# HKU-BAL/MegaGTA

Hardware: AMD Instinct MI355X
Metric: HMM-scored node expansions/sec + SdBG-build Gk-mer/s, k=45, 100Mx150bp (higher is better)
Workload: dtype u32

## Files before the change

### include/megagta_hip.h

```cpp
#ifndef MEGAGTA_HIP_H_
#define MEGAGTA_HIP_H_
#include <stdint.h>
#ifdef __cplusplus
extern "C" {
#endif

#define MGTA_OK 0
#define MGTA_EINVAL (-1)
#define MGTA_EHIP (-2)
#define MGTA_ENOMEM (-3)
#define MGTA_EUNSUPPORTED (-4)
#define MGTA_ESINK (-5)
#define MGTA_EOVERFLOW (-6)
#define MGTA_EINTERNAL (-7)

#define MGTA_NUM_BUCKETS 65536

typedef struct mgta_ctx mgta_ctx;
typedef struct mgta_reads mgta_reads;
typedef struct mgta_sdbg mgta_sdbg;
typedef struct mgta_hmm mgta_hmm;

const char *mgta_last_error(void);
const char *mgta_version(void);

mgta_ctx *mgta_ctx_create(int device_id);
void mgta_ctx_destroy(mgta_ctx *);
int mgta_ctx_set_mem_limit(mgta_ctx *, uint64_t bytes);
int mgta_ctx_device_memory(mgta_ctx *, uint64_t *free_bytes, uint64_t *total_bytes);
int mgta_ctx_keep_stream(mgta_ctx *, int on);
typedef struct mgta_stream mgta_stream;
int mgta_sdbg_stream_detach(mgta_ctx *, mgta_stream **out);
int mgta_stream_sizes(const mgta_stream *, uint64_t *n_recs, uint64_t *n_tip_words);
int mgta_stream_download(mgta_stream *, uint16_t *recs, uint32_t *tips);
void mgta_stream_free(mgta_stream *);
int mgta_ctx_release_scratch(mgta_ctx *);
int mgta_ctx_set_full_lsd(mgta_ctx *, int on);
int mgta_sort_plan(uint64_t n_items, int words_per_key, uint32_t bucket_begin, uint32_t bucket_end, int *n_passes, int *skip_bits);
int mgta_sort_plan_wide(uint64_t n_items, int words_per_key, uint32_t bucket_begin, uint32_t bucket_end, int *n_passes, int *skip_bits,
                        int *widths );
int mgta_ctx_set_search_cost_rate(mgta_ctx *, int expansions_per_seed);
int mgta_ctx_set_search_cost_curve(mgta_ctx *, int expansions_per_seed, uint64_t knee_expansions, int expansions_per_seed_beyond);
int mgta_ctx_set_search_arena(mgta_ctx *, int log2_base_nodes, uint64_t pool_bytes);
int mgta_ctx_set_search_page_limit(mgta_ctx *, int pages);
int mgta_ctx_keep_multiplicity(mgta_ctx *, int on);

int mgta_reads_pack_text(mgta_ctx *, const char *text, uint64_t n_bytes, const uint64_t *offsets , uint64_t n_reads,
                         uint32_t *bin_words, uint64_t capacity_words, uint64_t *n_words_out);


typedef int (*mgta_edge_sink)(void *user, int32_t bucket_begin, int32_t bucket_end,
                              const int64_t *bucket_counts ,
                              const uint16_t *recs, int64_t n_recs, const uint16_t *large, int64_t n_large,
                              const uint32_t *tips, int64_t n_tip_words);

typedef struct mgta_build_stats {
    int32_t k, words_per_key, words_per_tip, n_passes;
    int64_t n_reads, n_kmers;
    int64_t n_items;
    int64_t n_edges, n_tips, n_large;
    int64_t n_sort_launches;
    double ms_total;
    double ms_count, ms_gen, ms_sort, ms_emit, ms_d2h;
    double ms_sort_scatter;
    double ms_local_sort;
    int64_t n_big_segments;
    int64_t n_lsd_tiles;
    uint64_t bytes_peak;
    double ms_stage1;
    int64_t n_fused_passes;
    int64_t n_wide_passes;
    int64_t n_split_levels;
} mgta_build_stats;

int mgta_reads_upload(mgta_ctx *, const uint32_t *packed_seq, uint64_t n_words, const uint64_t *start_idx,
                      uint64_t n_reads, mgta_reads **out);
int mgta_reads_adopt_device(mgta_ctx *, const uint32_t *d_packed_seq, uint64_t n_words,
                            const uint64_t *d_start_idx, uint64_t n_reads, mgta_reads **out);
void mgta_reads_free(mgta_reads *);

int mgta_sdbg_build_resident(mgta_ctx *, const mgta_reads *, uint64_t n_short_reads, int k, int min_count,
                             int need_mercy, int32_t bucket_begin, int32_t bucket_end ,
                             mgta_edge_sink sink, void *user, mgta_build_stats *stats);
int mgta_sdbg_last_counting(mgta_ctx *, int64_t *hist );
int mgta_sdbg_export_records_device(mgta_ctx *, void *d_dst, uint64_t capacity_bytes, uint64_t *n_records);
int mgta_sdbg_build(mgta_ctx *, const uint32_t *packed_seq, uint64_t n_words, const uint64_t *start_idx,
                    uint64_t n_reads, uint64_t n_short_reads, int k, int min_count, int need_mercy,
                    mgta_edge_sink sink, void *user, mgta_build_stats *stats);

int mgta_sdbg_load(mgta_ctx *, int k, const uint16_t *recs, int64_t size, const int64_t *bucket_items,
                   const uint32_t *tips, int64_t n_tip_words, int words_per_tip, mgta_sdbg **out);
int mgta_sdbg_load_resident(mgta_ctx *, mgta_sdbg **out);
int mgta_sdbg_load_large(mgta_ctx *, int k, const uint16_t *recs, int64_t size, const int64_t *bucket_items, const uint32_t *tips,
                         int64_t n_tip_words, int words_per_tip, const uint16_t *large, int64_t n_large, mgta_sdbg **out);
int mgta_sdbg_load_files(mgta_ctx *, const char *prefix, mgta_sdbg **out);
void mgta_sdbg_free(mgta_sdbg *);
int64_t mgta_sdbg_size(const mgta_sdbg *);
int mgta_sdbg_k(const mgta_sdbg *);
int mgta_sdbg_outgoing(mgta_sdbg *, const int64_t *edges, int64_t n, int64_t *out4, int8_t *outdeg);
int mgta_sdbg_invalid_bits(mgta_sdbg *, uint64_t *words);
int mgta_sdbg_index_edges(mgta_sdbg *, const uint8_t *seqs , int64_t n, int64_t *edge_ids);

int mgta_sdbg_edge_multiplicity(mgta_sdbg *, const int64_t *edge_ids, int64_t n, uint16_t *mult);

typedef struct mgta_contig_cov {
    uint64_t sum;
    uint32_t len, n_windows;
    uint32_t n_covered;
    uint32_t min, max, median;
} mgta_contig_cov;
typedef struct mgta_coverage_stats {
    int64_t n_contigs, n_windows;
    int64_t n_walked;
    int64_t n_index_searches;
    int64_t n_batches;
    int64_t groups_per_cu;
    double ms_kernel;
    double ms_walk;
} mgta_coverage_stats;
int mgta_ctx_set_coverage_batch(mgta_ctx *, uint64_t windows);
int mgta_contig_coverage(mgta_sdbg *, const char *seqs, const uint64_t *offsets , int64_t n, mgta_contig_cov *per_contig,
                         uint16_t *per_window , int64_t *abundance , mgta_coverage_stats *stats );

typedef struct mgta_contig_share {
    uint64_t mass;
    uint32_t len, n_windows;
    uint32_t n_covered;
    uint32_t n_unique;
    uint32_t max_share;
    uint32_t reserved_;
} mgta_contig_share;
typedef struct mgta_share_stats {
    int64_t n_contigs, n_windows;
    int64_t n_walked, n_index_searches;
    int64_t n_batches;
    int64_t n_covered;
    int64_t n_distinct_edges;
    uint64_t total_mult;
    uint64_t total_mass;
    uint64_t table_slots;
    uint64_t table_bytes;
    uint64_t window_bytes;
    double ms_walk;
    double ms_count;
    double ms_share;
    double ms_total;
} mgta_share_stats;
int mgta_ctx_set_share_hash_bits(mgta_ctx *, int bits);
int mgta_contig_share_coverage(mgta_sdbg *, const char *seqs, const uint64_t *offsets , int64_t n, mgta_contig_share *per_contig,
                               uint32_t *per_window_share , uint16_t *per_window , mgta_share_stats *stats );

typedef struct mgta_match_stats {
    int64_t n_contigs, n_contig_windows;
    int64_t n_marked_edges;
    int64_t n_reads, n_read_windows;
    int64_t n_walked, n_index_searches;
    int64_t n_matched_reads;
    int64_t groups_per_cu;
    double ms_mark, ms_walk;
} mgta_match_stats;
int mgta_reads_match_contigs(mgta_sdbg *, const mgta_reads *reads, int reads_reversed, uint64_t n_short_reads,
                             const char *seqs, const uint64_t *offsets , int64_t n,
                             uint64_t *match_bits ,
                             uint32_t *hit_windows , mgta_match_stats *stats );

typedef struct mgta_sample_cov_stats {
    int64_t n_contigs, n_windows;
    int64_t n_walked, n_index_searches;
    int64_t n_batches;
    int64_t n_covered;
    int64_t n_keys;
    int64_t n_libs;
    int64_t n_reads, n_read_windows;
    int64_t n_read_walked, n_read_index_searches;
    int64_t n_hit_windows;
    int64_t groups_per_cu;
    uint64_t total_mass;
    uint64_t table_slots;
    uint64_t table_bytes;
    uint64_t window_bytes;
    uint64_t count_bytes;
    double ms_mark;
    double ms_scan;
    double ms_mass;
    double ms_total;
} mgta_sample_cov_stats;
int mgta_contig_sample_coverage(mgta_sdbg *, const mgta_reads *reads, int reads_reversed, const uint64_t *lib_end , int n_libs,
                                const char *seqs, const uint64_t *offsets , int64_t n, uint64_t *mass ,
                                mgta_contig_share *per_contig , uint64_t *per_window_count ,
                                uint32_t *per_window_share , uint64_t *lib_hit_windows ,
                                mgta_sample_cov_stats *stats );

typedef struct mgta_pileup_params { int32_t min_anchors, min_overlap, max_mismatch_permille; } mgta_pileup_params;
typedef struct mgta_contig_pileup { uint32_t len, n_covered, min_depth, max_depth; uint64_t n_placed, n_unique, depth_sum, mismatch_sum; } mgta_contig_pileup;
typedef struct mgta_read_place { int32_t score, contig, diag, orient; uint32_t n_placed, n_mismatch; } mgta_read_place;
typedef struct mgta_pileup_stats {
    int64_t n_contigs, n_contig_letters, n_contig_windows;
    int64_t n_keys;
    int64_t n_occurrences;
    int64_t n_reads, n_read_windows;
    int64_t n_hit_windows;
    int64_t n_read_walked, n_read_index_searches;
    int64_t n_reads_with_candidate, n_candidates;
    int64_t n_verified;
    int64_t n_reads_placed, n_reads_multi, n_placements;
    int64_t n_bases_piled;
    int64_t groups_per_cu;
    uint64_t peak_bytes;
    double ms_keys, ms_index, ms_scan, ms_records, ms_total;
} mgta_pileup_stats;
int mgta_reads_pileup(mgta_sdbg *, const mgta_reads *reads, int reads_reversed, uint64_t n_short_reads, const char *seqs,
                      const uint64_t *offsets , int64_t n, const mgta_pileup_params *params ,
                      uint32_t *counts , uint32_t *uniq ,
                      mgta_contig_pileup *per_contig , mgta_read_place *per_read ,
                      mgta_pileup_stats *stats );
int mgta_ctx_set_pileup_chunk(mgta_ctx *, uint32_t reads);

typedef struct mgta_derep_stats {
    int64_t n_seqs, n_letters;
    int64_t n_first;
    int64_t n_duplicates, n_contained, n_kept;
    int64_t n_windows;
    int64_t anchor_len;
    int64_t n_compares;
    double ms_dups, ms_table, ms_verify;
} mgta_derep_stats;
int mgta_seqs_derep(mgta_ctx *, const char *seqs, const uint64_t *offsets , int64_t n,
                    uint8_t *status, int64_t *rep, uint32_t *copies, mgta_derep_stats *stats );
int mgta_ctx_set_derep_hash_bits(mgta_ctx *, int bits);

typedef struct mgta_align_rec {
    double score;
    int32_t status;
    int32_t model_from, model_to;
    int32_t n_match, n_insert, n_delete;
} mgta_align_rec;
typedef struct mgta_align_stats {
// ... 202 lines not shown
```

### megagta_amd/_lib.py

```python
from __future__ import annotations

import ctypes as C
import os

_HERE = os.path.dirname(os.path.abspath(__file__))
LIB_PATH = os.environ.get("MEGAGTA_HIP_LIB") or os.path.join(_HERE, "libmegagta_hip.so")


class MegaGtaError(RuntimeError):
    pass


class DenovoStats(C.Structure):
    _fields_ = [("n_tips", C.c_int64), ("n_bubbles", C.c_int64), ("n_bubble_candidates", C.c_int64), ("n_bubble_rounds", C.c_int64),
                ("n_paths", C.c_int64), ("n_unitig_sweeps", C.c_int64), ("n_contigs", C.c_int64), ("total_len", C.c_int64),
                ("ms_tips", C.c_float), ("ms_bubbles", C.c_float), ("ms_unitigs", C.c_float)]

    def as_dict(self):
        return {n: getattr(self, n) for n, _ in self._fields_}


class BuildStats(C.Structure):
    _fields_ = [("k", C.c_int32), ("words_per_key", C.c_int32), ("words_per_tip", C.c_int32), ("n_passes", C.c_int32),
                ("n_reads", C.c_int64), ("n_kmers", C.c_int64), ("n_items", C.c_int64), ("n_edges", C.c_int64),
# ... 57 lines not shown
                ("table_slots", C.c_uint64), ("table_bytes", C.c_uint64), ("window_bytes", C.c_uint64), ("ms_walk", C.c_double), ("ms_count", C.c_double),
                ("ms_share", C.c_double), ("ms_total", C.c_double)]

    def as_dict(self):
        return {n: getattr(self, n) for n, _ in self._fields_}


class MatchStats(C.Structure):
    _fields_ = [("n_contigs", C.c_int64), ("n_contig_windows", C.c_int64), ("n_marked_edges", C.c_int64), ("n_reads", C.c_int64),
                ("n_read_windows", C.c_int64), ("n_walked", C.c_int64), ("n_index_searches", C.c_int64), ("n_matched_reads", C.c_int64),
                ("groups_per_cu", C.c_int64), ("ms_mark", C.c_double), ("ms_walk", C.c_double)]

    def as_dict(self):
        return {n: getattr(self, n) for n, _ in self._fields_}


class SampleCovStats(C.Structure):
    _fields_ = [("n_contigs", C.c_int64), ("n_windows", C.c_int64), ("n_walked", C.c_int64), ("n_index_searches", C.c_int64), ("n_batches", C.c_int64),
                ("n_covered", C.c_int64), ("n_keys", C.c_int64), ("n_libs", C.c_int64), ("n_reads", C.c_int64), ("n_read_windows", C.c_int64),
                ("n_read_walked", C.c_int64), ("n_read_index_searches", C.c_int64), ("n_hit_windows", C.c_int64), ("groups_per_cu", C.c_int64),
                ("total_mass", C.c_uint64), ("table_slots", C.c_uint64), ("table_bytes", C.c_uint64), ("window_bytes", C.c_uint64),
                ("count_bytes", C.c_uint64), ("ms_mark", C.c_double), ("ms_scan", C.c_double), ("ms_mass", C.c_double), ("ms_total", C.c_double)]

    def as_dict(self):
        return {n: getattr(self, n) for n, _ in self._fields_}


class DerepStats(C.Structure):
    _fields_ = [("n_seqs", C.c_int64), ("n_letters", C.c_int64), ("n_first", C.c_int64), ("n_duplicates", C.c_int64), ("n_contained", C.c_int64),
                ("n_kept", C.c_int64), ("n_windows", C.c_int64), ("anchor_len", C.c_int64), ("n_compares", C.c_int64), ("ms_dups", C.c_double),
                ("ms_table", C.c_double), ("ms_verify", C.c_double)]

    def as_dict(self):
        return {n: getattr(self, n) for n, _ in self._fields_}


class AlignRec(C.Structure):
    _fields_ = [("score", C.c_double), ("status", C.c_int32), ("model_from", C.c_int32), ("model_to", C.c_int32), ("n_match", C.c_int32),
                ("n_insert", C.c_int32), ("n_delete", C.c_int32)]


class AlignStats(C.Structure):
    _fields_ = [("n_seqs", C.c_int64), ("n_aligned", C.c_int64), ("n_unaligned", C.c_int64), ("n_cells", C.c_int64), ("n_batches", C.c_int64),
                ("blocks_per_cu", C.c_int64), ("waves_per_block", C.c_int64), ("grid_blocks", C.c_int64), ("lds_bytes", C.c_int64),
                ("msc_in_lds", C.c_int64), ("ms_fill", C.c_double), ("ms_trace", C.c_double)]

    def as_dict(self):
        return {n: getattr(self, n) for n, _ in self._fields_}


class PostRec(C.Structure):
    _fields_ = [("fwd", C.c_double), ("bwd", C.c_double), ("status", C.c_int32), ("pad", C.c_int32)]


class PostStats(C.Structure):
    _fields_ = [("n_seqs", C.c_int64), ("n_scored", C.c_int64), ("n_unaligned", C.c_int64), ("n_cells", C.c_int64), ("n_batches", C.c_int64),
                ("workgroups", C.c_int64), ("waves_per_block", C.c_int64), ("blocks_per_cu", C.c_int64), ("lds_bytes", C.c_int64),
                ("msc_in_lds", C.c_int64), ("peak_bytes", C.c_int64), ("ms_forward", C.c_double), ("ms_backward", C.c_double)]

    def as_dict(self):
        return {n: getattr(self, n) for n, _ in self._fields_}


class RowPair(C.Structure):
    _fields_ = [("i", C.c_int32), ("j", C.c_int32), ("n_diff", C.c_uint16), ("n_overlap", C.c_uint16)]


class ClusterStats(C.Structure):
    _fields_ = [("n_rows", C.c_int64), ("n_unaligned", C.c_int64), ("n_pairs_kept", C.c_int64), ("n_clusters", C.c_int64), ("n_singletons", C.c_int64),
                ("largest_cluster", C.c_int64), ("n_components", C.c_int64), ("n_tiles", C.c_int64), ("n_link_pops", C.c_int64),
                ("blocks_per_cu", C.c_int64), ("grid_blocks", C.c_int64), ("lds_bytes", C.c_int64), ("peak_bytes", C.c_int64),
                ("ms_pairs", C.c_double), ("ms_link", C.c_double)]

    def as_dict(self):
        return {n: getattr(self, n) for n, _ in self._fields_}


class TreeStats(C.Structure):
    _fields_ = [("n_rows", C.c_int64), ("n_pairs", C.c_int64), ("n_merges", C.c_int64), ("n_rounds", C.c_int64), ("n_entries_visited", C.c_int64),
                ("n_lists_rewritten", C.c_int64), ("n_cut_fallbacks", C.c_int64), ("n_unaligned", C.c_int64), ("n_clusters", C.c_int64),
                ("n_singletons", C.c_int64), ("largest_cluster", C.c_int64), ("peak_bytes", C.c_int64), ("ms_pairs", C.c_double), ("ms_build", C.c_double),
                ("ms_rounds", C.c_double), ("ms_cut", C.c_double)]

    def as_dict(self):
        return {n: getattr(self, n) for n, _ in self._fields_}


class NearestRec(C.Structure):
    _fields_ = [("status", C.c_int32), ("ref", C.c_int32), ("score", C.c_int32), ("ref_from", C.c_int32), ("ref_to", C.c_int32), ("n_match", C.c_int32),
                ("n_ident", C.c_int32), ("n_insert", C.c_int32), ("n_delete", C.c_int32)]


class NearestStats(C.Structure):
    _fields_ = [("n_seqs", C.c_int64), ("n_refs", C.c_int64), ("n_pairs", C.c_int64), ("n_unaligned", C.c_int64), ("n_cells", C.c_int64),
                ("n_trace_cells", C.c_int64), ("n_batches", C.c_int64), ("n_segments", C.c_int64), ("blocks_per_cu", C.c_int64),
                ("waves_per_block", C.c_int64), ("grid_blocks", C.c_int64), ("lds_bytes", C.c_int64), ("peak_bytes", C.c_int64),
                ("ms_score", C.c_double), ("ms_trace", C.c_double)]

    def as_dict(self):
        return {n: getattr(self, n) for n, _ in self._fields_}


class ChimeraRec(C.Structure):
    _fields_ = [("status", C.c_int32), ("ref", C.c_int32), ("score", C.c_int32), ("brk", C.c_int32), ("left_ref", C.c_int32), ("left_score", C.c_int32),
                ("right_ref", C.c_int32), ("right_score", C.c_int32), ("two", C.c_int32), ("one", C.c_int32), ("gain", C.c_int32)]


class ChimeraStats(C.Structure):
    _fields_ = [("n_seqs", C.c_int64), ("n_refs", C.c_int64), ("n_clean", C.c_int64), ("n_chimeric", C.c_int64), ("n_unchecked", C.c_int64),
                ("n_cells", C.c_int64), ("n_parent_cells", C.c_int64), ("n_items", C.c_int64), ("n_parent_items", C.c_int64), ("n_segments", C.c_int64),
                ("n_groups", C.c_int64), ("grid_blocks", C.c_int64), ("waves_per_block", C.c_int64), ("blocks_per_cu", C.c_int64), ("lds_bytes", C.c_int64),
                ("bound_bytes", C.c_int64), ("peak_bytes", C.c_int64), ("ms_top", C.c_double), ("ms_parents", C.c_double)]

    def as_dict(self):
        return {n: getattr(self, n) for n, _ in self._fields_}


class PileupParams(C.Structure):
    _fields_ = [("min_anchors", C.c_int32), ("min_overlap", C.c_int32), ("max_mismatch_permille", C.c_int32)]


class PileupStats(C.Structure):
    _fields_ = [("n_contigs", C.c_int64), ("n_contig_letters", C.c_int64), ("n_contig_windows", C.c_int64), ("n_keys", C.c_int64), ("n_occurrences", C.c_int64),
                ("n_reads", C.c_int64), ("n_read_windows", C.c_int64), ("n_hit_windows", C.c_int64), ("n_read_walked", C.c_int64),
                ("n_read_index_searches", C.c_int64), ("n_reads_with_candidate", C.c_int64), ("n_candidates", C.c_int64), ("n_verified", C.c_int64),
                ("n_reads_placed", C.c_int64), ("n_reads_multi", C.c_int64), ("n_placements", C.c_int64), ("n_bases_piled", C.c_int64),
                ("groups_per_cu", C.c_int64), ("peak_bytes", C.c_uint64), ("ms_keys", C.c_double), ("ms_index", C.c_double), ("ms_scan", C.c_double),
                ("ms_records", C.c_double), ("ms_total", C.c_double)]

    def as_dict(self):
        return {n: getattr(self, n) for n, _ in self._fields_}


EDGE_SINK = C.CFUNCTYPE(C.c_int, C.c_void_p, C.c_int32, C.c_int32, C.POINTER(C.c_int64), C.POINTER(C.c_uint16), C.c_int64,
                        C.POINTER(C.c_uint16), C.c_int64, C.POINTER(C.c_uint32), C.c_int64)
CONTIG_SINK = C.CFUNCTYPE(C.c_int, C.c_void_p, C.c_int64, C.c_void_p, C.c_int64, C.c_void_p, C.c_int64,
                          C.POINTER(AstarSide), C.POINTER(AstarSide))

SYMBOLS = {
    "mgta_last_error": (C.c_char_p, []),
    "mgta_version": (C.c_char_p, []),
    "mgta_ctx_create": (C.c_void_p, [C.c_int]),
    "mgta_ctx_destroy": (None, [C.c_void_p]),
    "mgta_ctx_set_mem_limit": (C.c_int, [C.c_void_p, C.c_uint64]),
    "mgta_ctx_set_full_lsd": (C.c_int, [C.c_void_p, C.c_int]),
    "mgta_sort_plan": (C.c_int, [C.c_uint64, C.c_int, C.c_uint32, C.c_uint32, C.POINTER(C.c_int), C.POINTER(C.c_int)]),
    "mgta_sort_plan_wide": (C.c_int, [C.c_uint64, C.c_int, C.c_uint32, C.c_uint32, C.POINTER(C.c_int), C.POINTER(C.c_int), C.POINTER(C.c_int)]),
    "mgta_reads_upload": (C.c_int, [C.c_void_p, C.c_void_p, C.c_uint64, C.c_void_p, C.c_uint64, C.POINTER(C.c_void_p)]),
    "mgta_reads_adopt_device": (C.c_int, [C.c_void_p, C.c_void_p, C.c_uint64, C.c_void_p, C.c_uint64, C.POINTER(C.c_void_p)]),
    "mgta_reads_free": (None, [C.c_void_p]),
    "mgta_sdbg_build_resident": (C.c_int, [C.c_void_p, C.c_void_p, C.c_uint64, C.c_int, C.c_int, C.c_int, C.c_int32, C.c_int32,
                                          EDGE_SINK, C.c_void_p, C.POINTER(BuildStats)]),
    "mgta_sdbg_last_counting": (C.c_int, [C.c_void_p, C.c_void_p]),
    "mgta_sdbg_export_records_device": (C.c_int, [C.c_void_p, C.c_void_p, C.c_uint64, C.POINTER(C.c_uint64)]),
    "mgta_sdbg_build": (C.c_int, [C.c_void_p, C.c_void_p, C.c_uint64, C.c_void_p, C.c_uint64, C.c_uint64, C.c_int, C.c_int,
                                 C.c_int, EDGE_SINK, C.c_void_p, C.POINTER(BuildStats)]),
    "mgta_findstart": (C.c_int, [C.c_void_p, C.c_void_p, C.c_int, C.c_int, C.c_void_p, C.c_int64, C.c_void_p, C.c_int64, C.c_void_p, C.c_void_p]),
    "mgta_sdbg_load_resident": (C.c_int, [C.c_void_p, C.c_void_p]),
    "mgta_sdbg_load_files": (C.c_int, [C.c_void_p, C.c_char_p, C.c_void_p]),
    "mgta_sdbg_invalid_bits": (C.c_int, [C.c_void_p, C.c_void_p]),
    "mgta_ctx_set_search_cost_rate": (C.c_int, [C.c_void_p, C.c_int]),
    "mgta_ctx_set_search_cost_curve": (C.c_int, [C.c_void_p, C.c_int, C.c_uint64, C.c_int]),
    "mgta_ctx_set_search_arena": (C.c_int, [C.c_void_p, C.c_int, C.c_uint64]),
    "mgta_ctx_set_search_page_limit": (C.c_int, [C.c_void_p, C.c_int]),
    "mgta_ctx_device_memory": (C.c_int, [C.c_void_p, C.POINTER(C.c_uint64), C.POINTER(C.c_uint64)]),
    "mgta_ctx_keep_stream": (C.c_int, [C.c_void_p, C.c_int]),
    "mgta_sdbg_stream_detach": (C.c_int, [C.c_void_p, C.POINTER(C.c_void_p)]),
    "mgta_stream_sizes": (C.c_int, [C.c_void_p, C.POINTER(C.c_uint64), C.POINTER(C.c_uint64)]),
    "mgta_stream_download": (C.c_int, [C.c_void_p, C.c_void_p, C.c_void_p]),
    "mgta_stream_free": (None, [C.c_void_p]),
    "mgta_sdbg_k": (C.c_int, [C.c_void_p]),
    "mgta_ctx_set_search_share": (C.c_int, [C.c_void_p, C.c_int, C.c_int]),
    "mgta_astar_batch_on": (C.c_int, [C.c_void_p, C.c_void_p, C.c_void_p, C.c_void_p, C.c_char_p, C.c_void_p, C.c_int64, C.c_int, C.c_double,
                                     C.c_int, CONTIG_SINK, C.c_void_p, C.POINTER(AstarStats)]),
    "mgta_astar_batch_packed": (C.c_int, [C.c_void_p, C.c_void_p, C.c_void_p, C.c_char_p, C.c_void_p, C.c_int64, C.c_int, C.c_double, C.c_int,
                                         C.POINTER(C.c_void_p), C.c_void_p, C.c_void_p, C.POINTER(AstarStats)]),
    "mgta_reads_pack_text": (C.c_int, [C.c_void_p, C.c_char_p, C.c_uint64, C.c_void_p, C.c_uint64, C.c_void_p, C.c_uint64, C.POINTER(C.c_uint64)]),
    "mgta_ctx_release_scratch": (C.c_int, [C.c_void_p]),
    "mgta_denovo": (C.c_int, [C.c_void_p, C.c_int, C.c_int, C.c_int, C.c_void_p, C.c_void_p, C.c_void_p]),
    "mgta_host_free": (None, [C.c_void_p]),
    "mgta_sdbg_load": (C.c_int, [C.c_void_p, C.c_int, C.c_void_p, C.c_int64, C.c_void_p, C.c_void_p, C.c_int64, C.c_int,
                                C.POINTER(C.c_void_p)]),
    "mgta_ctx_keep_multiplicity": (C.c_int, [C.c_void_p, C.c_int]),
    "mgta_ctx_set_coverage_batch": (C.c_int, [C.c_void_p, C.c_uint64]),
    "mgta_sdbg_load_large": (C.c_int, [C.c_void_p, C.c_int, C.c_void_p, C.c_int64, C.c_void_p, C.c_void_p, C.c_int64, C.c_int, C.c_void_p, C.c_int64,
                                      C.POINTER(C.c_void_p)]),
    "mgta_sdbg_edge_multiplicity": (C.c_int, [C.c_void_p, C.c_void_p, C.c_int64, C.c_void_p]),
    "mgta_contig_coverage": (C.c_int, [C.c_void_p, C.c_char_p, C.c_void_p, C.c_int64, C.c_void_p, C.c_void_p, C.c_void_p, C.c_void_p]),
    "mgta_contig_share_coverage": (C.c_int, [C.c_void_p, C.c_char_p, C.c_void_p, C.c_int64, C.c_void_p, C.c_void_p, C.c_void_p, C.c_void_p]),
    "mgta_ctx_set_share_hash_bits": (C.c_int, [C.c_void_p, C.c_int]),
    "mgta_reads_match_contigs": (C.c_int, [C.c_void_p, C.c_void_p, C.c_int, C.c_uint64, C.c_char_p, C.c_void_p, C.c_int64, C.c_void_p, C.c_void_p,
                                          C.c_void_p]),
    "mgta_contig_sample_coverage": (C.c_int, [C.c_void_p, C.c_void_p, C.c_int, C.c_void_p, C.c_int, C.c_char_p, C.c_void_p, C.c_int64, C.c_void_p, C.c_void_p,
                                             C.c_void_p, C.c_void_p, C.c_void_p, C.c_void_p]),
    "mgta_reads_pileup": (C.c_int, [C.c_void_p, C.c_void_p, C.c_int, C.c_uint64, C.c_char_p, C.c_void_p, C.c_int64, C.c_void_p, C.c_void_p, C.c_void_p, C.c_void_p,
                                   C.c_void_p, C.c_void_p]),
    "mgta_ctx_set_pileup_chunk": (C.c_int, [C.c_void_p, C.c_uint32]),
    "mgta_seqs_derep": (C.c_int, [C.c_void_p, C.c_char_p, C.c_void_p, C.c_int64, C.c_void_p, C.c_void_p, C.c_void_p, C.c_void_p]),
    "mgta_ctx_set_derep_hash_bits": (C.c_int, [C.c_void_p, C.c_int]),
    "mgta_seqs_align": (C.c_int, [C.c_void_p, C.c_void_p, C.c_char_p, C.c_void_p, C.c_int64, C.c_void_p, C.c_void_p, C.c_void_p, C.c_void_p, C.c_void_p]),
    "mgta_ctx_set_align_batch": (C.c_int, [C.c_void_p, C.c_int64]),
    "mgta_seqs_posterior": (C.c_int, [C.c_void_p, C.c_void_p, C.c_char_p, C.c_void_p, C.c_int64, C.c_void_p, C.c_void_p, C.c_void_p, C.c_void_p, C.c_void_p,
                                      C.c_void_p]),
    "mgta_ctx_set_posterior_batch": (C.c_int, [C.c_void_p, C.c_int64]),
    "mgta_rows_pairs": (C.c_int, [C.c_void_p, C.c_void_p, C.c_int64, C.c_int64, C.c_int64, C.c_double, C.c_void_p, C.c_int64, C.c_void_p, C.c_void_p]),
    "mgta_rows_cluster": (C.c_int, [C.c_void_p, C.c_void_p, C.c_void_p, C.c_int64, C.c_int64, C.c_int64, C.c_double, C.c_void_p, C.c_void_p, C.c_void_p,
                                    C.c_void_p, C.c_void_p]),
    "mgta_pairs_link": (C.c_int, [C.c_void_p, C.c_int64, C.c_void_p, C.c_void_p, C.c_int64, C.c_void_p, C.c_void_p, C.c_void_p, C.c_void_p, C.c_void_p]),
    "mgta_ctx_set_cluster_tile": (C.c_int, [C.c_void_p, C.c_int64]),
    "mgta_pairs_tree": (C.c_int, [C.c_void_p, C.c_void_p, C.c_int64, C.c_void_p, C.c_int64, C.c_void_p, C.c_int64, C.c_void_p, C.c_void_p]),
    "mgta_tree_cut": (C.c_int, [C.c_void_p, C.c_int64, C.c_void_p, C.c_int64, C.c_void_p, C.c_void_p, C.c_int64, C.c_double, C.c_void_p, C.c_void_p, C.c_void_p,
                                C.c_void_p, C.c_void_p]),
    "mgta_rows_clusters": (C.c_int, [C.c_void_p, C.c_void_p, C.c_void_p, C.c_int64, C.c_int64, C.c_int64, C.c_void_p, C.c_int64, C.c_void_p, C.c_void_p,
                                     C.c_void_p, C.c_void_p, C.c_void_p, C.c_void_p, C.c_void_p]),
    "mgta_seqs_nearest": (C.c_int, [C.c_void_p, C.c_char_p, C.c_void_p, C.c_int64, C.c_char_p, C.c_void_p, C.c_int64, C.c_void_p, C.c_int32, C.c_int32,
                                    C.c_void_p, C.c_void_p, C.c_void_p, C.c_void_p, C.c_void_p]),
    "mgta_ctx_set_nearest_batch": (C.c_int, [C.c_void_p, C.c_int64]),
    "mgta_seqs_chimera": (C.c_int, [C.c_void_p, C.c_char_p, C.c_void_p, C.c_int64, C.c_char_p, C.c_void_p, C.c_int64, C.c_void_p, C.c_int32, C.c_int32,
                                    C.c_int32, C.c_int32, C.c_void_p, C.c_void_p, C.c_void_p]),
    "mgta_ctx_set_chimera_segment": (C.c_int, [C.c_void_p, C.c_int64]),
    "mgta_ctx_set_chimera_groups": (C.c_int, [C.c_void_p, C.c_int64]),
    "mgta_sdbg_free": (None, [C.c_void_p]),
    "mgta_sdbg_size": (C.c_int64, [C.c_void_p]),
    "mgta_sdbg_outgoing": (C.c_int, [C.c_void_p, C.c_void_p, C.c_int64, C.c_void_p, C.c_void_p]),
    "mgta_sdbg_index_edges": (C.c_int, [C.c_void_p, C.c_void_p, C.c_int64, C.c_void_p]),
    "mgta_hmm_load": (C.c_int, [C.c_void_p, C.c_int, C.c_int, C.c_void_p, C.c_void_p, C.c_void_p, C.c_void_p, C.c_void_p,
                               C.POINTER(C.c_void_p)]),
    "mgta_hmm_free": (None, [C.c_void_p]),
    "mgta_probe_random_lines": (C.c_int, [C.c_void_p, C.c_uint64, C.POINTER(LineProbe), C.c_int]),
    "mgta_astar_batch": (C.c_int, [C.c_void_p, C.c_void_p, C.c_void_p, C.c_char_p, C.c_void_p, C.c_int64, C.c_int, C.c_double,
                                  C.c_int, CONTIG_SINK, C.c_void_p, C.POINTER(AstarStats)]),
}

_LIB = None


def load():
    global _LIB
    if _LIB is not None:
        return _LIB
    if not os.path.exists(LIB_PATH):
        raise MegaGtaError(f"{LIB_PATH} is missing: build it with `python -c 'import __graft_entry__ as g; g.build()'` "
                           "(make -C megagta_amd/csrc). There is no CPU fallback.")
    L = C.CDLL(LIB_PATH)
    for name, (res, args) in SYMBOLS.items():
        fn = getattr(L, name)
        fn.restype, fn.argtypes = res, args
    _LIB = L
    return L


def check(rc: int, what: str):
    if rc != 0:
        raise MegaGtaError(f"{what} failed ({rc}): {load().mgta_last_error().decode()}")
```

### megagta_amd/api.py

```python
from __future__ import annotations

import ctypes as C
import hashlib
import os
from dataclasses import dataclass, field

import numpy as np

from . import _lib
from .chimera import REC as _chimera_rec
from ._lib import MegaGtaError, check

NUM_BUCKETS = 65536


@dataclass
class EdgeStream:
    k: int
    words_per_tip: int
    bucket_items: np.ndarray
    records: np.ndarray
    large: np.ndarray
    tips: np.ndarray
    bucket_large: np.ndarray = None
# ... 170 lines not shown
                  "mgta_rows_pairs")
            if got.value != cnt.value:
                raise MegaGtaError(f"mgta_rows_pairs counted {cnt.value} pairs, then {got.value}")
        return dict(pairs=pairs[:cnt.value], stats=st.as_dict())

    def cluster(self, rows, lens, min_overlap: int, cutoff: float) -> dict:
        r = self._rows(rows)
        n, M = r.shape
        ln = np.ascontiguousarray(lens, dtype=np.int64)
        if ln.shape != (n,):
            raise ValueError("lens must hold one length per row")
        cl, rep = np.zeros(max(1, n), dtype=np.int32), np.zeros(max(1, n), dtype=np.int64)
        rd, ro = np.zeros(max(1, n), dtype=np.uint16), np.zeros(max(1, n), dtype=np.uint16)
        st = _lib.ClusterStats()
        check(self._L.mgta_rows_cluster(self.h, r.ctypes.data, ln.ctypes.data, n, M, int(min_overlap), float(cutoff), cl.ctypes.data, rep.ctypes.data,
                                        rd.ctypes.data, ro.ctypes.data, C.byref(st)), "mgta_rows_cluster")
        return dict(cluster=cl[:n], rep=rep[:n], rep_diff=rd[:n], rep_overlap=ro[:n], stats=st.as_dict())

    def pairs_tree(self, pairs, n_residues) -> dict:
        p = _pair_array(pairs)
        nr = np.ascontiguousarray(n_residues, dtype=np.int32)
        if nr.ndim != 1:
            raise ValueError("n_residues must hold one value per row")
        n = nr.size
        merges = np.zeros(max(1, n), dtype=TREE_MERGE)
        cnt, st = C.c_int64(0), _lib.TreeStats()
        check(self._L.mgta_pairs_tree(self.h, p.ctypes.data if p.size else None, p.size, nr.ctypes.data, n, merges.ctypes.data, n, C.byref(cnt), C.byref(st)),
              "mgta_pairs_tree")
        return dict(merges=merges[:cnt.value], stats=st.as_dict())

    def clusters(self, rows, lens, min_overlap: int, cutoffs) -> dict:
        r = self._rows(rows)
        n, M = r.shape
        ln = np.ascontiguousarray(lens, dtype=np.int64)
        if ln.shape != (n,):
            raise ValueError("lens must hold one length per row")
        cut = np.ascontiguousarray(cutoffs, dtype=np.float64)
        if cut.ndim != 1:
            raise ValueError("cutoffs must be a list of numbers")
        k = cut.size
        cl, rep = np.zeros((k, n), dtype=np.int32), np.zeros((k, n), dtype=np.int64)
        rd, ro = np.zeros((k, n), dtype=np.uint16), np.zeros((k, n), dtype=np.uint16)
        merges = np.zeros(max(1, n), dtype=TREE_MERGE)
        cnt, st = C.c_int64(0), _lib.TreeStats()
        check(self._L.mgta_rows_clusters(self.h, r.ctypes.data, ln.ctypes.data, n, M, int(min_overlap), cut.ctypes.data if k else None, k, cl.ctypes.data,
                                         rep.ctypes.data, rd.ctypes.data, ro.ctypes.data, merges.ctypes.data, C.byref(cnt), C.byref(st)), "mgta_rows_clusters")
        return dict(cluster=cl, rep=rep, rep_diff=rd, rep_overlap=ro, merges=merges[:cnt.value], stats=st.as_dict())

    def set_nearest_batch(self, cells: int = 0):
        check(self._L.mgta_ctx_set_nearest_batch(self.h, int(cells)), "mgta_ctx_set_nearest_batch")

    def nearest(self, seqs, refs, sub, gap_open: int, gap_extend: int, scores: bool = False, paths: bool = False) -> dict:
        raw = [s if isinstance(s, (bytes, bytearray)) else str(s).encode("latin-1") for s in seqs]
        rraw = [s if isinstance(s, (bytes, bytearray)) else str(s).encode("latin-1") for s in refs]
        n, n_ref = len(raw), len(rraw)
        table = np.ascontiguousarray(sub, dtype=np.int8)
        if table.shape != (27, 27):
            raise ValueError("sub must be int8[27, 27]")
        offsets, roffsets = np.zeros(n + 1, dtype=np.uint64), np.zeros(n_ref + 1, dtype=np.uint64)
        if n:
            np.cumsum([len(s) for s in raw], out=offsets[1:])
        if n_ref:
            np.cumsum([len(s) for s in rraw], out=roffsets[1:])
        recs = np.zeros(max(1, n), dtype=NEAREST_REC)
        sc = np.zeros((n, n_ref), dtype=np.int32) if scores else None
        p = np.zeros(int(offsets[n]) + n * 4096 + 1, dtype=np.uint8) if paths else None
        plen = np.zeros(max(1, n), dtype=np.int32) if paths else None
        st = _lib.NearestStats()
        check(self._L.mgta_seqs_nearest(self.h, b"".join(raw), offsets.ctypes.data, n, b"".join(rraw), roffsets.ctypes.data, n_ref, table.ctypes.data,
                                        int(gap_open), int(gap_extend), recs.ctypes.data, sc.ctypes.data if scores and sc.size else None,
                                        p.ctypes.data if paths else None, plen.ctypes.data if paths else None, C.byref(st)), "mgta_seqs_nearest")
        out = dict(recs=recs[:n], stats=st.as_dict())
        if scores:
            out["scores"] = sc
        if paths:
            out["paths"] = [p[int(offsets[i]) + i * 4096:int(offsets[i]) + i * 4096 + int(plen[i])].tobytes().decode() for i in range(n)]
        return out

    def set_chimera_segment(self, columns: int = 0):
        check(self._L.mgta_ctx_set_chimera_segment(self.h, int(columns)), "mgta_ctx_set_chimera_segment")

    def set_chimera_groups(self, groups: int = 0):
        check(self._L.mgta_ctx_set_chimera_groups(self.h, int(groups)), "mgta_ctx_set_chimera_groups")

    def chimera(self, seqs, refs, sub, gap_open: int, gap_extend: int, min_seg: int, min_gain: int, tops: bool = False) -> dict:
        raw = [s if isinstance(s, (bytes, bytearray)) else str(s).encode("latin-1") for s in seqs]
        rraw = [s if isinstance(s, (bytes, bytearray)) else str(s).encode("latin-1") for s in refs]
        n, n_ref = len(raw), len(rraw)
        table = np.ascontiguousarray(sub, dtype=np.int8)
        if table.shape != (27, 27):
            raise ValueError("sub must be int8[27, 27]")
        offsets, roffsets = np.zeros(n + 1, dtype=np.uint64), np.zeros(n_ref + 1, dtype=np.uint64)
        if n:
            np.cumsum([len(s) for s in raw], out=offsets[1:])
        if n_ref:
            np.cumsum([len(s) for s in rraw], out=roffsets[1:])
        recs = np.zeros(max(1, n), dtype=CHIMERA_REC)
        tp = np.zeros((int(offsets[n]) + 1, 8), dtype=np.int32) if tops else None
        st = _lib.ChimeraStats()
        check(self._L.mgta_seqs_chimera(self.h, b"".join(raw), offsets.ctypes.data, n, b"".join(rraw), roffsets.ctypes.data, n_ref, table.ctypes.data,
                                        int(gap_open), int(gap_extend), int(min_seg), int(min_gain), recs.ctypes.data, tp.ctypes.data if tops else None,
                                        C.byref(st)), "mgta_seqs_chimera")
        out = dict(recs=recs[:n], stats=st.as_dict())
        if tops:
            out["tops"] = [tp[int(offsets[i]):int(offsets[i + 1])] for i in range(n)]
        return out

    def release_scratch(self):
        check(self._L.mgta_ctx_release_scratch(self.h), "mgta_ctx_release_scratch")

    def set_search_arena(self, log2_base_nodes: int = 0, pool_bytes: int = 0):
        check(self._L.mgta_ctx_set_search_arena(self.h, int(log2_base_nodes), int(pool_bytes)), "mgta_ctx_set_search_arena")

    def set_search_page_limit(self, pages: int = 0):
        check(self._L.mgta_ctx_set_search_page_limit(self.h, int(pages)), "mgta_ctx_set_search_page_limit")

    def upload_reads(self, packed: np.ndarray, start_idx: np.ndarray) -> "Reads":
        packed = np.ascontiguousarray(packed, dtype=np.uint32)
        start_idx = np.ascontiguousarray(start_idx, dtype=np.uint64)
        out = C.c_void_p()
        check(self._L.mgta_reads_upload(self.h, packed.ctypes.data, packed.size, start_idx.ctypes.data, start_idx.size - 1,
                                        C.byref(out)), "mgta_reads_upload")
        return Reads(self, out, start_idx.size - 1)

    def adopt_reads(self, d_packed_ptr: int, n_words: int, d_start_ptr: int, n_reads: int, keepalive=None) -> "Reads":
        out = C.c_void_p()
        check(self._L.mgta_reads_adopt_device(self.h, d_packed_ptr, n_words, d_start_ptr, n_reads, C.byref(out)),
              "mgta_reads_adopt_device")
        r = Reads(self, out, n_reads)
        r._keep = keepalive
        return r

    def build_sdbg(self, reads: "Reads", k: int, min_count: int = 1, need_mercy: bool = False, collect: bool = True,
                   n_short_reads: int | None = None, bucket_range: tuple[int, int] = (0, NUM_BUCKETS)) -> EdgeStream:
        wpt = (2 * k + 31) // 32
        recs, large, tips = [], [], []
        counts = np.zeros((NUM_BUCKETS, 3), dtype=np.int64)

        def sink(user, b0, b1, bc, r, nr, lg, nl, tp, ntw):
            nb = b1 - b0
            counts[b0:b1] = np.ctypeslib.as_array(bc, shape=(nb * 3,)).reshape(nb, 3)
            recs.append(np.ctypeslib.as_array(r, shape=(nr,)).copy() if nr and r else np.zeros(0, np.uint16))
            large.append(np.ctypeslib.as_array(lg, shape=(nl,)).copy() if nl else np.zeros(0, np.uint16))
            tips.append(np.ctypeslib.as_array(tp, shape=(ntw,)).copy() if ntw and tp else np.zeros(0, np.uint32))
            return 0

        cb = _lib.EDGE_SINK(sink) if collect else C.cast(None, _lib.EDGE_SINK)
        st = _lib.BuildStats()
        ns = reads.n_reads if n_short_reads is None else n_short_reads
        check(self._L.mgta_sdbg_build_resident(self.h, reads.h, ns, k, min_count, int(need_mercy), bucket_range[0], bucket_range[1],
                                               cb, None, C.byref(st)),
              "mgta_sdbg_build_resident")
        cat = lambda xs, dt: np.concatenate(xs) if xs else np.zeros(0, dt)
        return EdgeStream(k=k, words_per_tip=wpt, bucket_items=counts[:, 0].copy(), records=cat(recs, np.uint16),
                          large=cat(large, np.uint16), tips=cat(tips, np.uint32), bucket_large=counts[:, 1].copy(),
                          bucket_tips=counts[:, 2].copy(), stats=st.as_dict())


def export_records_to_torch(ctx: "Context"):
    import torch
    n = C.c_uint64()
    check(ctx._L.mgta_sdbg_export_records_device(ctx.h, None, 0, C.byref(n)), "mgta_sdbg_export_records_device")
    t = torch.empty(max(1, n.value * 2), dtype=torch.uint8, device="cuda")
    check(ctx._L.mgta_sdbg_export_records_device(ctx.h, t.data_ptr(), t.numel(), C.byref(n)), "mgta_sdbg_export_records_device")
    return t[: n.value * 2]


SHARE_DTYPE = np.dtype([("mass", "<u8"), ("len", "<u4"), ("n_windows", "<u4"), ("n_covered", "<u4"), ("n_unique", "<u4"), ("max_share", "<u4"),
                        ("reserved_", "<u4")])
COV_DTYPE = np.dtype([("sum", "<u8"), ("len", "<u4"), ("n_windows", "<u4"), ("n_covered", "<u4"), ("min", "<u4"), ("max", "<u4"), ("median", "<u4")])


class _multiplicity:

    def __init__(self, ctx: "Context", on: bool):
        self.ctx, self.was = ctx, getattr(ctx, "_keep_multiplicity", False)
        self.on = bool(on) or self.was

    def __enter__(self):
        if self.on != self.was:
            self.ctx.keep_multiplicity(self.on)
        return self

    def __exit__(self, *exc):
        if self.on != self.was:
            self.ctx.keep_multiplicity(self.was)
        return False


class Graph:

    def __init__(self, ctx: Context, stream: "EdgeStream | None", k: int = 0, keep_multiplicity: bool = False):
        if stream is None:
            self.ctx, self.k = ctx, k
            out = C.c_void_p()
            with _multiplicity(ctx, keep_multiplicity) as sw:
                self.keep_multiplicity = sw.on
                check(ctx._L.mgta_sdbg_load_resident(ctx.h, C.byref(out)), "mgta_sdbg_load_resident")
            self.h = out
            self.size = ctx._L.mgta_sdbg_size(self.h)
            self.k = ctx._L.mgta_sdbg_k(self.h)
            return
        self.ctx, self.k = ctx, stream.k
        recs = np.ascontiguousarray(stream.records, dtype=np.uint16)
        bi = np.ascontiguousarray(stream.bucket_items, dtype=np.int64)
        tips = np.ascontiguousarray(stream.tips, dtype=np.uint32)
        out = C.c_void_p()
        with _multiplicity(ctx, keep_multiplicity) as sw:
            self.keep_multiplicity = sw.on
            if sw.on:
                large = np.ascontiguousarray(stream.large, dtype=np.uint16)
                check(ctx._L.mgta_sdbg_load_large(ctx.h, stream.k, recs.ctypes.data, recs.size, bi.ctypes.data, tips.ctypes.data, tips.size,
                                                  stream.words_per_tip, large.ctypes.data, large.size, C.byref(out)), "mgta_sdbg_load_large")
            else:
                check(ctx._L.mgta_sdbg_load(ctx.h, stream.k, recs.ctypes.data, recs.size, bi.ctypes.data, tips.ctypes.data, tips.size,
                                            stream.words_per_tip, C.byref(out)), "mgta_sdbg_load")
        self.h = out
        self.size = ctx._L.mgta_sdbg_size(self.h)

    @classmethod
    def from_files(cls, ctx: Context, prefix: str, keep_multiplicity: bool = False) -> "Graph":
        self = cls.__new__(cls)
        self.ctx = ctx
        out = C.c_void_p()
        with _multiplicity(ctx, keep_multiplicity) as sw:
            self.keep_multiplicity = sw.on
            check(ctx._L.mgta_sdbg_load_files(ctx.h, os.fsencode(prefix), C.byref(out)), "mgta_sdbg_load_files")
        self.h = out
        self.size = ctx._L.mgta_sdbg_size(self.h)
        self.k = ctx._L.mgta_sdbg_k(self.h)
        return self

    def outgoing(self, edges) -> tuple[np.ndarray, np.ndarray]:
        e = np.ascontiguousarray(edges, dtype=np.int64)
        out = np.empty((e.size, 4), dtype=np.int64)
        deg = np.empty(e.size, dtype=np.int8)
        check(self.ctx._L.mgta_sdbg_outgoing(self.h, e.ctypes.data, e.size, out.ctypes.data, deg.ctypes.data), "mgta_sdbg_outgoing")
        return deg, out

    def index_edges(self, kmers: list[str]) -> np.ndarray:
        m = {"A": 1, "C": 2, "G": 3, "T": 4, "N": 3}
        seqs = np.array([[m.get(c, 0) for c in s.upper()[: self.k + 1]] for s in kmers], dtype=np.uint8).reshape(len(kmers), self.k + 1)
        ids = np.empty(len(kmers), dtype=np.int64)
        check(self.ctx._L.mgta_sdbg_index_edges(self.h, seqs.ctypes.data, len(kmers), ids.ctypes.data), "mgta_sdbg_index_edges")
        return ids

    def invalid_bits(self) -> np.ndarray:
        out = np.zeros((self.size + 63) // 64, dtype=np.uint64)
        check(self.ctx._L.mgta_sdbg_invalid_bits(self.h, out.ctypes.data), "mgta_sdbg_invalid_bits")
        return out

    def edge_multiplicity(self, ids) -> np.ndarray:
        e = np.ascontiguousarray(ids, dtype=np.int64)
        out = np.empty(e.size, dtype=np.uint16)
        check(self.ctx._L.mgta_sdbg_edge_multiplicity(self.h, e.ctypes.data, e.size, out.ctypes.data), "mgta_sdbg_edge_multiplicity")
        return out

    def contig_coverage(self, seqs, per_window: bool = False, abundance: bool = True) -> dict:
        raw = [s if isinstance(s, (bytes, bytearray)) else str(s).encode() for s in seqs]
        n = len(raw)
        offsets = np.zeros(n + 1, dtype=np.uint64)
        if n:
            np.cumsum([len(s) for s in raw], out=offsets[1:])
        buf = b"".join(raw)
        cov = np.zeros(n, dtype=COV_DTYPE)
        nw = np.maximum(0, np.diff(offsets.astype(np.int64)) - self.ctx._L.mgta_sdbg_k(self.h))
        woff = np.zeros(n + 1, dtype=np.int64)
        np.cumsum(nw, out=woff[1:])
        pw = np.zeros(int(woff[-1]), dtype=np.uint16) if per_window else None
        ab = np.zeros(65536, dtype=np.int64) if abundance else None
        st = _lib.CoverageStats()
        check(self.ctx._L.mgta_contig_coverage(self.h, buf, offsets.ctypes.data, n, cov.ctypes.data if n else None,
                                               pw.ctypes.data if per_window and pw.size else None, ab.ctypes.data if abundance else None,
                                               C.byref(st)), "mgta_contig_coverage")
        out = dict(contigs=cov, abundance=ab, stats=st.as_dict())
        if per_window:
            out["per_window"], out["window_offsets"] = pw, woff
        return out

    def contig_share_coverage(self, seqs, per_window: bool = False) -> dict:
        raw = [s if isinstance(s, (bytes, bytearray)) else str(s).encode() for s in seqs]
        n = len(raw)
        offsets = np.zeros(n + 1, dtype=np.uint64)
        if n:
            np.cumsum([len(s) for s in raw], out=offsets[1:])
        rec = np.zeros(n, dtype=SHARE_DTYPE)
        nw = np.maximum(0, np.diff(offsets.astype(np.int64)) - self.ctx._L.mgta_sdbg_k(self.h))
        woff = np.zeros(n + 1, dtype=np.int64)
        np.cumsum(nw, out=woff[1:])
        pws = np.zeros(int(woff[-1]), dtype=np.uint32) if per_window else None
        pw = np.zeros(int(woff[-1]), dtype=np.uint16) if per_window else None
        st = _lib.ShareStats()
        check(self.ctx._L.mgta_contig_share_coverage(self.h, b"".join(raw), offsets.ctypes.data, n, rec.ctypes.data if n else None,
                                                     pws.ctypes.data if per_window and pws.size else None, pw.ctypes.data if per_window and pw.size else None,
                                                     C.byref(st)), "mgta_contig_share_coverage")
        out = dict(contigs=rec, stats=st.as_dict(), per_window_share=pws, per_window=pw)
        if per_window:
            out["window_offsets"] = woff
        return out

    def match_reads(self, reads: "Reads", seqs, n_short_reads: int | None = None, counts: bool = False, reads_reversed: bool = True) -> dict:
        raw = [s if isinstance(s, (bytes, bytearray)) else str(s).encode() for s in seqs]
        n = len(raw)
        offsets = np.zeros(n + 1, dtype=np.uint64)
        if n:
            np.cumsum([len(s) for s in raw], out=offsets[1:])
        ns = reads.n_reads if n_short_reads is None else int(n_short_reads)
        words = np.zeros(max(1, (ns + 63) // 64), dtype=np.uint64)
        hits = np.zeros(ns, dtype=np.uint32) if counts else None
# ... 335 lines not shown
```

### megagta_amd/csrc/common.hpp

```cpp
#pragma once
#include <hip/hip_runtime.h>

#include <cstdarg>
#include <cstdint>
#include <cstdio>
#include <cstring>
#include <exception>
#include <new>
#include <string>
#include <vector>

#include "../../include/megagta_hip.h"

namespace mgta {

void set_error(const char *fmt, ...);

struct HipError {
    int code;
};

#define MGTA_HIP_CHECK(expr)                                                                        \
    do {                                                                                            \
        hipError_t e_ = (expr);                                                                     \
        if (e_ != hipSuccess) {                                                                     \
            ::mgta::set_error("%s failed: %s (%s:%d)", #expr, hipGetErrorString(e_), __FILE__, __LINE__); \
            throw ::mgta::HipError{e_ == hipErrorOutOfMemory ? MGTA_ENOMEM : MGTA_EHIP};           \
        }                                                                                           \
    } while (0)

struct DevBuf {
    void *p = nullptr;
    size_t bytes = 0;
    uint64_t *live = nullptr, *peak = nullptr;
    DevBuf() = default;
    DevBuf(const DevBuf &) = delete;
    DevBuf &operator=(const DevBuf &) = delete;
    DevBuf(DevBuf &&o) noexcept { *this = std::move(o); }
    DevBuf &operator=(DevBuf &&o) noexcept {
        if (this != &o) { release(); p = o.p; bytes = o.bytes; live = o.live; peak = o.peak; o.p = nullptr; o.bytes = 0; }
        return *this;
    }
    ~DevBuf() { release(); }
    void alloc(size_t n, uint64_t *live_ = nullptr, uint64_t *peak_ = nullptr) {
        release();
        if (n == 0) n = 16;
        MGTA_HIP_CHECK(hipMalloc(&p, n));
        bytes = n; live = live_; peak = peak_;
        if (live) { *live += n; if (peak && *live > *peak) *peak = *live; }
    }
    void release() {
        if (p) { (void)hipFree(p); if (live) *live -= bytes; }
        p = nullptr; bytes = 0;
    }
    template <class T> T *as() const { return reinterpret_cast<T *>(p); }
};

template <class F> int guarded(const char *who, F &&f) {
    try { return f(); }
    catch (const HipError &e) { return e.code; }
    catch (const std::bad_alloc &) { set_error("%s: out of host memory", who); return MGTA_ENOMEM; }
    catch (const std::exception &e) { set_error("%s: %s", who, e.what()); return MGTA_EHIP; }
}

struct Timer {
    hipEvent_t a = nullptr, b = nullptr;
    hipStream_t st;
    explicit Timer(hipStream_t s) : st(s) { MGTA_HIP_CHECK(hipEventCreate(&a)); MGTA_HIP_CHECK(hipEventCreate(&b)); }
    Timer(Timer &&o) noexcept : a(o.a), b(o.b), st(o.st) { o.a = o.b = nullptr; }
    ~Timer() { if (a) (void)hipEventDestroy(a); if (b) (void)hipEventDestroy(b); }
    void start() { MGTA_HIP_CHECK(hipEventRecord(a, st)); }
    void end() { MGTA_HIP_CHECK(hipEventRecord(b, st)); }
    float ms() const { float t = 0; MGTA_HIP_CHECK(hipEventElapsedTime(&t, a, b)); return t; }
    double stop() {
        MGTA_HIP_CHECK(hipGetLastError());
        end();
        MGTA_HIP_CHECK(hipEventSynchronize(b));
        MGTA_HIP_CHECK(hipGetLastError());
        return ms();
    }
};

enum Slot { S_BLOCK_COUNT, S_BLOCK_BASE, S_SCAN_TMP, S_SMALL, S_KEYS_A, S_KEYS_B, S_HIST, S_TILE_HEADS, S_TILE_BASE, S_CNT, S_BASE,
            S_FIRST, S_OUT_REC, S_OUT_LARGE, S_OUT_TIPS, S_PLAN, S_BIG, S_LSD, S_MULTI_COUNT, S_POS2ID, S_SOLID, S_MERCY, S_EDGE_COUNT, S_SIDE, S_FUSED_HIST,
            S_DIGIT_TOTALS ,
            S_SPLIT , S_NUM };

}

namespace mgta {
struct AstarArenas {
    DevBuf pool, meta;
};
}

struct mgta_ctx {
    int refs = 1;
    int device = 0;
    hipStream_t stream = nullptr;
    uint64_t mem_limit = 0;
    int force_full_lsd = 0;
    int lsd_skip_left = 0;
    int split_levels = 0;
    int astar_log_b0 = 0;
    uint64_t astar_pool_bytes = 0;
    int search_page_limit = 0;
    int search_share_num = 1, search_share_den = 1;
    int search_cost_rate = 0;
    uint64_t search_cost_knee = 0;
    int search_cost_rate2 = 0;
    int force_lsd_tiles = 0;
    uint64_t live_bytes = 0, peak_bytes = 0;
    int num_cus = 256;
    hipDeviceProp_t prop;
    std::vector<mgta::DevBuf> pool;
    mgta::AstarArenas astar;
    std::vector<int64_t> edge_counting;
    const void *last_rec = nullptr;
    uint64_t last_n_rec = 0;
    uint32_t last_bucket_lo = 0, last_bucket_hi = 0;
    const void *last_tips = nullptr;
    const void *last_first = nullptr;
    uint64_t last_n_tips = 0;
    int last_k = 0, last_words_per_tip = 0;
    int keep_stream = 0;
    bool acc_valid = false;
    mgta::DevBuf acc_rec, acc_tips;
    uint64_t acc_n_rec = 0, acc_n_tips = 0;
    std::vector<int64_t> acc_items;
    int keep_multiplicity = 0;
    uint64_t coverage_batch_windows = 0;
    uint64_t align_batch_cells = 0;
    uint64_t posterior_batch_cells = 0;
    uint64_t nearest_batch_cells = 0;
    uint64_t chimera_segment_cols = 0;
    uint64_t chimera_groups = 0;
    uint64_t cluster_tile_rows = 0;
    int derep_hash_bits = 64;
    int share_hash_bits = 64;
    uint32_t pileup_chunk = 0;
    const void *last_large = nullptr;
    uint64_t last_n_large = 0;
    mgta::DevBuf acc_large;
    uint64_t acc_n_large = 0;
    bool acc_has_large = false;
};

namespace mgta {
inline void ctx_retain(mgta_ctx *c) { __atomic_add_fetch(&c->refs, 1, __ATOMIC_RELAXED); }
void ctx_release(mgta_ctx *c);
inline void forget_last_build(mgta_ctx *c) {
    c->last_rec = nullptr; c->last_tips = nullptr; c->last_first = nullptr; c->last_n_rec = 0; c->last_n_tips = 0; c->last_k = 0;
    c->last_large = nullptr; c->last_n_large = 0;
}
}

struct mgta_hmm {
    mgta_ctx *ctx = nullptr;
    int M = 0, A = 0;
    mgta::DevBuf tab;
    int8_t col[2][64];
    mgta::DevBuf d_col;
    int8_t alpha[128];
    mgta::DevBuf d_alpha;
    size_t n_doubles = 0;
};

struct mgta_reads {
    mgta_ctx *ctx = nullptr;
    const uint32_t *d_packed = nullptr;
    const uint64_t *d_start = nullptr;
    uint64_t n_words = 0, n_reads = 0;
    mgta::DevBuf own_packed, own_start;
};
```

### megagta_amd/csrc/sdbg_build.hip

```cpp
#include <algorithm>
#include <cmath>
#include <cstdlib>
#include <memory>
#include <type_traits>

#include "common.hpp"
#include "device_utils.hpp"
#include "scan.hpp"
#include "segment_split.hpp"

namespace mgta {

constexpr int kDollar = 4;

template <int W>
struct Key {
    uint32_t w[W];
};

template <int W>
__device__ __forceinline__ void shl_bits(uint32_t (&x)[W], int s) {
    if (s == 0) return;
    if (s == 32) {
#pragma unroll
// ... 987 lines not shown
            ss.toff[tid] = (uint32_t)place;
            ss.gtile[tid] = ex + my_off - place;
            if (tid == kVals - 1) ss.toff[kVals] = (uint32_t)(place + c);
        }
        __syncthreads();
        if (tile_base >= n) return;
        const uint64_t cnt = (n - tile_base) < (uint64_t)kBlockTile ? (n - tile_base) : (uint64_t)kBlockTile;
        scatter_subtiles<W, BIASED, true, STABLE, BITS, NEXT_BITS>(sh, in + tile_base, out, cnt, d, &ss, d_next);
        __syncthreads();
        const int lane = lane_id(), wv = wave_id();
        for (int v = wv * (kVals / kSortWaves); v < (wv + 1) * (kVals / kSortWaves); ++v) {
            const uint32_t from = ss.toff[v], len = ss.toff[v + 1] - from;
            SideEntry<NEXT_BITS> *to = side + ss.gtile[v] + from;
            for (uint32_t i = lane; i < len; i += 64) to[i] = ss.bytes[from + i];
        }
    } else {
        __syncthreads();
        if (tile_base >= n) return;
        const uint64_t cnt = (n - tile_base) < (uint64_t)kBlockTile ? (n - tile_base) : (uint64_t)kBlockTile;
        scatter_subtiles<W, BIASED, false, STABLE, BITS>(sh, in + tile_base, out, cnt, d);
    }
}

constexpr uint64_t kSegInOther = 1ull << 63;
struct SegList {
    uint64_t *first, *end;
    uint32_t *count;
    uint32_t cap;
};
struct SplitLists {
    SegList small, mid, next;
    uint32_t *n_split;
};

template <int W>
__global__ __launch_bounds__(kSortThreads) void segment_split_kernel(Key<W> *buf0, Key<W> *buf1, const uint64_t *seg_first, const uint64_t *seg_end,
                                                                      Digit d, uint32_t local_tile, uint32_t lds_cap, SplitLists out) {
    __shared__ ScatterShared<W> sh;
    __shared__ uint64_t s64[kSortThreads / 64 + 1];
    __shared__ uint32_t s_cnt[256];
    __shared__ uint32_t e_meta[256];
    __shared__ uint32_t s_one;
    const int tid = threadIdx.x, lane = lane_id(), wv = wave_id();
    const uint64_t f = wave_uniform(seg_first[blockIdx.x]), s0 = f & ~kSegInOther, cnt = wave_uniform(seg_end[blockIdx.x]) - s0;
    if (cnt <= (uint64_t)lds_cap) return;
    const bool in_other = (f & kSegInOther) != 0;
    const Key<W> *x = (in_other ? buf1 : buf0) + s0;
    Key<W> *y = (in_other ? buf0 : buf1) + s0;
    if (tid < 256) s_cnt[tid] = 0;
    if (tid == 0) { s_one = 0; atomicAdd(out.n_split, 1u); }
    __syncthreads();
    for (uint64_t base = (uint64_t)wv * 64; base < cnt; base += kSortThreads) {
        const uint64_t i = base + (uint64_t)lane;
        const bool valid = i < cnt;
        const uint32_t dg = valid ? get_digit<W>(x[i], d) : 0u;
        const uint32_t dg0 = wave_uniform(dg);
        const uint64_t vm = __ballot(valid);
        if (__ballot(valid && dg == dg0) == vm) {
            if (lane == 0) atomicAdd(&s_cnt[dg0], (uint32_t)__popcll(vm));
        } else if (valid)
            atomicAdd(&s_cnt[dg], 1u);
    }
    __syncthreads();
    const uint64_t c = tid < 256 ? s_cnt[tid] : 0;
    if (c == cnt) s_one = 1;
    const uint64_t ex = block_excl_scan64<kSortThreads>(c, s64, nullptr);
    if (tid < 256) sh.gbase[tid] = ex;
    __syncthreads();
    auto append = [&](const SegList &l, uint32_t q, uint64_t first, uint64_t end) {
        if (q < l.cap) { l.first[q] = first; l.end[q] = end; }
    };
    if (s_one) {
        if (tid == 0) append(out.next, atomicAdd(out.next.count, 1u), f, s0 + cnt);
        return;
    }
    scatter_subtiles<W>(sh, x, y, cnt, d);
    __syncthreads();
    if (wv != 0) return;
    uint64_t *const e_first = sh.gbase, *const e_end = sh.gdelta;
    uint32_t cv[4], n_cls[kSplitClasses] = {0, 0, 0}, n_ent = 0;
#pragma unroll
    for (int q = 0; q < 4; ++q) cv[q] = s_cnt[q * 64 + lane];
    SplitPacker pk(s0, local_tile, lds_cap);
    auto emit = [&](uint32_t cls, uint64_t first, uint64_t end) {
        const uint32_t idx = cls == kSplitSmall ? n_cls[0]++ : (cls == kSplitMid ? n_cls[1]++ : n_cls[2]++);
        if (lane == 0) { e_first[n_ent] = first; e_end[n_ent] = end; e_meta[n_ent] = cls | (idx << 2); }
        ++n_ent;
    };
#pragma unroll
    for (int q = 0; q < 4; ++q)
        for (int i = 0; i < 64; ++i) pk.step((uint32_t)__builtin_amdgcn_readlane((int)cv[q], i), emit);
    pk.finish(emit);
    uint32_t base[kSplitClasses] = {0, 0, 0};
    if (lane == 0) {
        if (n_cls[0]) base[0] = atomicAdd(out.small.count, n_cls[0]);
        if (n_cls[1]) base[1] = atomicAdd(out.mid.count, n_cls[1]);
        if (n_cls[2]) base[2] = atomicAdd(out.next.count, n_cls[2]);
    }
#pragma unroll
    for (int q = 0; q < kSplitClasses; ++q) base[q] = wave_uniform(base[q]);
    wave_lds_fence();
    const uint64_t where = in_other ? 0ull : kSegInOther;
    for (uint32_t e = lane; e < n_ent; e += 64) {
        const uint32_t cls = e_meta[e] & 3u, idx = e_meta[e] >> 2;
        const uint64_t first = e_first[e] | where, end = e_end[e];
        if (cls == kSplitSmall) append(out.small, base[0] + idx, first, end);
        else if (cls == kSplitMid) append(out.mid, base[1] + idx, first, end);
        else append(out.next, base[2] + idx, first, end);
    }
}

template <int W>
__global__ __launch_bounds__(kSortThreads) void segment_copy_kernel(Key<W> *res, const Key<W> *other, const uint64_t *seg_first, const uint64_t *seg_end) {
    const uint64_t f = seg_first[blockIdx.x], s0 = f & ~kSegInOther, cnt = seg_end[blockIdx.x] - s0;
    if (!(f & kSegInOther)) return;
    for (uint64_t i = threadIdx.x; i < cnt; i += kSortThreads) res[s0 + i] = other[s0 + i];
}

template <int W> struct LocalCfg {
    static constexpr int kTile = W <= 4 ? 4096 : 2048;
    static constexpr int kIpt = kTile / kSortThreads;
    static constexpr int kChunk = kTile / kSortWaves;
};

template <int W> struct BigCfg {
    static constexpr int kTile = W <= 4 ? 8192 : (W <= 8 ? 4096 : 0);
};

template <int W, int TILE = LocalCfg<W>::kTile>
struct LocalShared {
    Key<W> keys[TILE];
    uint16_t seg[TILE];
    uint16_t whist[kSortWaves][256];
    uint32_t start[256];
    uint32_t scratch[kSortThreads / 64 + 1];
    uint32_t wheads[kSortWaves + 1];
};

template <int W>
struct CompareShared {
    static constexpr int kRoom = (80 * 1024 - 1024 - LocalCfg<W>::kTile * 4 * W) / 2;
    static constexpr int kBins = kRoom >= 2048 ? (kRoom / 2048 * 2048 < 16384 ? kRoom / 2048 * 2048 : 16384) : 16384;
    static_assert(kBins >= LocalCfg<W>::kTile || kBins == 16384, "a bin per segment at least");
    Key<W> keys[LocalCfg<W>::kTile];
    uint32_t hist[kBins / 2];
    uint32_t scratch[kSortThreads / 64 + 1];
    uint32_t flags[2];
    uint64_t masks[LocalCfg<W>::kTile / 64];
};

template <int W>
__device__ __forceinline__ uint32_t key_prefix(const Key<W> &key, int T) { return T == 0 ? 0u : (key.w[0] >> (32 - T)); }

struct LocalPlan {
    const Digit *low_plan;
    int n_low;
    int T;
    Digit upper;
    uint32_t mask_last2;
    uint32_t mask_last;
    uint32_t stride;
    uint64_t *lsd_list;
    uint32_t *lsd_count;
    uint32_t lsd_cap;
    int debug;
};

constexpr uint32_t kMaxAvgRun = 40;
constexpr uint32_t kMaxRun = 256;

template <int W, int FIRST, bool MASKED>
__device__ __forceinline__ bool key_less(const Key<W> &a, const Key<W> &b, uint32_t m2, uint32_t m1) {
    bool lt = false;
    auto word = [&](const Key<W> &k, int j) {
        uint32_t x = k.w[j];
        if (MASKED && j == W - 1) x &= m1;
        if (MASKED && j == W - 2) x &= m2;
        return x;
    };
#pragma unroll
    for (int j = W - 1; j >= FIRST; j -= 2) {
        if (j - 1 >= FIRST) {
            const uint64_t x = ((uint64_t)word(a, j - 1) << 32) | word(a, j), y = ((uint64_t)word(b, j - 1) << 32) | word(b, j);
            lt = x < y || (x == y && lt);
        } else {
            const uint32_t x = word(a, j), y = word(b, j);
            lt = x < y || (x == y && lt);
        }
    }
    return lt;
}

template <int W>
__device__ __forceinline__ int tile_load(LocalShared<W> &sh, const Key<W> *keys, uint64_t first, uint32_t nt, int T, Key<W> (&key)[LocalCfg<W>::kIpt],
                                         uint32_t (&seg)[LocalCfg<W>::kIpt]) {
    constexpr int kIpt = LocalCfg<W>::kIpt, kChunk = LocalCfg<W>::kChunk;
    const int lane = lane_id(), wv = wave_id();
    const uint64_t le_mask = lanemask_lt() | (1ull << lane);
    uint32_t running = 0;
#pragma unroll
    for (int it = 0; it < kIpt; ++it) {
        uint32_t j = (uint32_t)wv * kChunk + (uint32_t)it * 64 + (uint32_t)lane;
        bool valid = j < nt, head = false;
        if (valid) {
            key[it] = keys[first + j];
            head = j == 0 || key_prefix<W>(key[it], T) != key_prefix<W>(keys[first + j - 1], T);
        }
        uint64_t bal = __ballot(head);
        seg[it] = running + (uint32_t)__popcll(bal & le_mask);
        running += (uint32_t)__popcll(bal);
    }
    if (lane == 0) sh.wheads[wv] = running;
    __syncthreads();
    uint32_t before = 0, nseg = 0;
    for (int w = 0; w < kSortWaves; ++w) { uint32_t c = sh.wheads[w]; if (w < wv) before += c; nseg += c; }
    before = wave_uniform(before);
    nseg = wave_uniform(nseg);
#pragma unroll
    for (int it = 0; it < kIpt; ++it) seg[it] = seg[it] + before - 1;
    return nseg <= 1 ? 0 : (nseg <= 256 ? 1 : 2);
}

template <int W, int TILE = LocalCfg<W>::kTile>
__device__ __forceinline__ void tile_zero_counts(LocalShared<W, TILE> &sh) {
    uint16_t *whist = sh.whist[wave_id()];
    for (int i = lane_id(); i < 256; i += 64) whist[i] = 0;
}

template <int W, int TILE = LocalCfg<W>::kTile>
__device__ __forceinline__ void lds_pass(LocalShared<W, TILE> &sh, Key<W> (&key)[TILE / kSortThreads], uint32_t (&seg)[TILE / kSortThreads], uint32_t nt,
                                         Digit d, bool by_seg, int seg_shift, bool reload, uint32_t off = 0) {
    constexpr int kIpt = TILE / kSortThreads, kChunk = TILE / kSortWaves;
    const int tid = threadIdx.x, lane = lane_id(), wv = wave_id();
    uint16_t *whist = sh.whist[wv];
    uint32_t dr[kIpt], cnt[kIpt];
    if (by_seg) {
#pragma unroll
        for (int it = 0; it < kIpt; ++it) dr[it] = (seg[it] >> seg_shift) & 255u;
    } else {
        get_digits<W, kIpt>(key, d, dr);
    }
#pragma unroll
    for (int it = 0; it < kIpt; ++it) {
        uint32_t j = (uint32_t)wv * kChunk + (uint32_t)it * 64 + (uint32_t)lane;
        bool valid = j - off < nt;
        uint32_t dg = valid ? dr[it] : 0u, rank;
        wave_match(dg, by_seg ? 8 : d.bits, valid, rank, cnt[it]);
        dr[it] = dg | (rank << 8) | ((uint32_t)valid << 31);
    }
#pragma unroll
    for (int it = 0; it < kIpt; ++it) {
        if (dr[it] >> 31) {
            const uint32_t dg = dr[it] & 255u, rank = (dr[it] >> 8) & 0xFFu, prev = whist[dg];
            if (rank == cnt[it] - 1) whist[dg] = (uint16_t)(prev + cnt[it]);
            dr[it] += prev << 8;
        }
        wave_lds_fence();
    }
    __syncthreads();
    uint32_t tot = 0, inc = 0;
    if (wv < 4) {
#pragma unroll
        for (int w = 0; w < kSortWaves; ++w) tot += sh.whist[w][tid];
        inc = wave_incl_scan(tot);
        if (lane == 63) sh.scratch[wv] = inc;
    }
    __syncthreads();
    if (wv < 4) {
        uint32_t running = inc - tot;
        for (int w = 0; w < wv; ++w) running += sh.scratch[w];
#pragma unroll
        for (int w = 0; w < kSortWaves; ++w) { uint32_t c = sh.whist[w][tid]; sh.whist[w][tid] = (uint16_t)running; running += c; }
    }
    __syncthreads();
#pragma unroll
    for (int it = 0; it < kIpt; ++it) {
        if (dr[it] >> 31) {
            uint32_t pos = whist[dr[it] & 255u] + ((dr[it] >> 8) & 0x7FFFFFu);
            sh.keys[pos] = key[it];
            sh.seg[pos] = (uint16_t)seg[it];
        }
    }
    __syncthreads();
    tile_zero_counts<W, TILE>(sh);
    if (reload) {
#pragma unroll
        for (int it = 0; it < kIpt; ++it) {
            uint32_t j = (uint32_t)wv * kChunk + (uint32_t)it * 64 + (uint32_t)lane;
            if (j < nt) { key[it] = sh.keys[j]; seg[it] = sh.seg[j]; }
        }
    }
}

template <int W, int PW>
__device__ __forceinline__ uint64_t key_top(const Key<W> &k) {
    return PW == 1 ? (uint64_t)k.w[0] : (((uint64_t)k.w[0] << 32) | (uint64_t)k.w[W > 1 ? 1 : 0]);
}

template <int W, int FIRST, bool MASKED, int PW>
__device__ __forceinline__ bool finish_by_comparison(CompareShared<W> &sh, Key<W> *keys, uint64_t first, uint32_t nt, int run_bits, uint32_t m2,
                                                     uint32_t m1, bool skip_compare) {
    const int run_shift = 32 * PW - run_bits;
    constexpr int kIpt = LocalCfg<W>::kIpt, kWindows = LocalCfg<W>::kTile / 64;
    const int lane = lane_id(), wv = wave_id();
    const uint64_t le_mask = lanemask_lt() | (1ull << lane);
    uint32_t heads = 0;
#pragma unroll
    for (int it = 0; it < kIpt; ++it) {
        const uint32_t win = (uint32_t)it * kSortWaves + (uint32_t)wv, j = win * 64 + (uint32_t)lane;
        const bool head = j < nt && (j == 0 || ((key_top<W, PW>(sh.keys[j - 1]) ^ key_top<W, PW>(sh.keys[j])) >> run_shift) != 0);
        const uint64_t hm = __ballot(head);
        if (lane == 0) sh.masks[win] = hm;
        heads += (uint32_t)__popcll(hm);
    }
    if (lane == 0 && heads) atomicAdd(&sh.flags[0], heads);
    __syncthreads();
    if (nt > wave_uniform(sh.flags[0]) * kMaxAvgRun) return false;
    uint32_t run[kIpt];
    bool over = false;
#pragma unroll
    for (int it = 0; it < kIpt; ++it) {
        const uint32_t win = (uint32_t)it * kSortWaves + (uint32_t)wv, j = win * 64 + (uint32_t)lane;
        run[it] = 0;
        if (j < nt) {
            const uint64_t hm = sh.masks[win];
            uint64_t m = hm & le_mask;
            uint32_t w = win;
            while (m == 0 && win - w <= kMaxRun / 64) m = sh.masks[--w];
            const uint32_t rs = m ? w * 64 + 63u - (uint32_t)__clzll((long long)m) : j;
            over = over || m == 0;
            m = hm & ~le_mask;
            w = win;
            while (m == 0 && w + 1 < (uint32_t)kWindows && w - win <= kMaxRun / 64) m = sh.masks[++w];
            const uint32_t re = m ? w * 64 + (uint32_t)__ffsll((long long)m) - 1u : nt;
            over = over || re - rs > kMaxRun;
            run[it] = rs | ((re - rs) << 16);
        }
    }
    if (__ballot(over) && lane == 0) sh.flags[1] = 1;
    __syncthreads();
    if (wave_uniform(sh.flags[1])) return false;
#pragma unroll
    for (int it = 0; it < kIpt; ++it) {
        const uint32_t j = ((uint32_t)it * kSortWaves + (uint32_t)wv) * 64 + (uint32_t)lane;
        if (j < nt) {
            const Key<W> mine = sh.keys[j];
            const uint32_t rs = run[it] & 0xFFFFu, re = rs + (run[it] >> 16);
            uint32_t r = j - rs;
            if (!skip_compare) {
                r = 0;
#pragma unroll 2
                for (uint32_t t = rs; t < j; ++t) r += key_less<W, FIRST, MASKED>(mine, sh.keys[t], m2, m1) ? 0u : 1u;
#pragma unroll 2
                for (uint32_t t = j + 1; t < re; ++t) r += key_less<W, FIRST, MASKED>(sh.keys[t], mine, m2, m1) ? 1u : 0u;
            }
            keys[first + rs + r] = mine;
        }
    }
    return true;
}

template <int W, bool WANT_KEYS>
__global__ __launch_bounds__(kSortThreads, 8) void local_sort_kernel(Key<W> *keys, uint64_t n, LocalPlan lp, uint64_t *big, uint32_t *big_count,
                                                                     uint32_t big_cap) {
    constexpr int kTile = LocalCfg<W>::kTile, kIpt = LocalCfg<W>::kIpt, kChunk = LocalCfg<W>::kChunk, kWindows = kTile / 64;
    constexpr uint32_t NONE = ~0u;
    static_assert(kWindows <= 64, "tile bounds are read off one 64-bit head mask per lane");
    const uint32_t kLocalStride = lp.stride;
    __shared__ CompareShared<W> sh;
    const int tid = threadIdx.x, lane = lane_id(), wv = wave_id(), T = lp.T;
    const uint64_t lo = (uint64_t)blockIdx.x * kLocalStride;
    const uint32_t loaded = (uint32_t)(n - lo < (uint64_t)kTile ? n - lo : (uint64_t)kTile);
    constexpr bool want_keys = WANT_KEYS;
    if (tid == 0) { sh.flags[0] = 0; sh.flags[1] = 0; }
    Key<W> key[kIpt];
    uint32_t seg[kIpt];
    uint32_t carry = 0;
#pragma unroll
    for (int it = 0; it < kIpt; ++it) {
        const uint32_t j = (uint32_t)wv * kChunk + (uint32_t)it * 64 + (uint32_t)lane;
        const bool inw = j < loaded;
        uint32_t p = 0;
        if (inw) {
            if (want_keys) key[it] = keys[lo + j];
            else key[it].w[0] = keys[lo + j].w[0];
            p = key_prefix<W>(key[it], T);
        }
        uint32_t pp = __shfl_up(p, 1, 64);
        if (lane == 0) pp = it == 0 ? ((inw && lo + j > 0) ? key_prefix<W>(keys[lo + j - 1], T) : 0u) : carry;
        carry = __shfl(p, 63, 64);
        const uint64_t hm = __ballot(inw && (lo + j == 0 || p != pp));
        if (lane == 0) sh.masks[wv * kIpt + it] = hm;
    }
    __syncthreads();
    const uint64_t hmask = lane < kWindows ? sh.masks[lane] : 0ull;
    const bool in_stride = (uint32_t)lane < kLocalStride / 64;
    const uint32_t first_off = wave_uniform(wave_min(in_stride && hmask ? (uint32_t)lane * 64 + (uint32_t)__ffsll((long long)hmask) - 1u : NONE));
    if (first_off == NONE) return;
    uint32_t end_off = wave_uniform(wave_min(!in_stride && hmask ? (uint32_t)lane * 64 + (uint32_t)__ffsll((long long)hmask) - 1u : NONE));
    if (end_off == NONE) {
        if (lo + loaded == n) end_off = loaded;
        else {
            end_off = wave_uniform(wave_max(in_stride && hmask ? (uint32_t)lane * 64 + 63u - (uint32_t)__clzll((long long)hmask) : 0u));
            if (tid == 0) {
                uint32_t q = atomicAdd(big_count, 1u);
                if (q < big_cap) big[q] = lo + end_off;
            }
        }
    }
    const uint32_t nt = end_off - first_off;
    if (nt == 0) return;
    const uint64_t first = lo + first_off;
    auto leave_to_lsd = [&]() {
        if (tid == 0) {
            uint32_t q = atomicAdd(lp.lsd_count, 1u);
            if (q < lp.lsd_cap) { lp.lsd_list[2 * q] = first; lp.lsd_list[2 * q + 1] = lo + end_off; }
        }
    };
    if (!want_keys) { leave_to_lsd(); return; }
    uint32_t nseg;
    {
        uint64_t in_tile = hmask;
        const uint32_t w0 = (uint32_t)lane * 64;
        if (w0 + 64 <= first_off || w0 >= end_off) in_tile = 0;
        else {
            if (first_off > w0) in_tile &= ~0ull << (first_off - w0);
            if (end_off < w0 + 64) in_tile &= ~0ull >> (w0 + 64 - end_off);
        }
        const uint32_t c = (uint32_t)__popcll(in_tile), inc = wave_incl_scan(c);
        nseg = wave_uniform((uint32_t)__shfl(inc, 63, 64));
        const uint64_t le_mask = lanemask_lt() | (1ull << lane);
#pragma unroll
        for (int it = 0; it < kIpt; ++it) {
            const int m = wv * kIpt + it;
            const uint32_t before = (uint32_t)__shfl(inc - c, m, 64);
            const uint64_t mm = (uint64_t)__shfl((unsigned long long)in_tile, m, 64);
            seg[it] = before + (uint32_t)__popcll(mm & le_mask) - 1u;
        }
    }
    if (lp.debug & 2) return;
    constexpr int kBins = CompareShared<W>::kBins, kWordsPerThread = kBins / 2 / kSortThreads;
    int ub = 31 - __clz((int)((uint32_t)kBins / nseg));
    if (ub > lp.upper.bits) ub = lp.upper.bits;
    const uint32_t n_words = ((nseg << ub) + 1u) >> 1;
    for (uint32_t i = tid; i < n_words; i += kSortThreads) sh.hist[i] = 0;
    __syncthreads();
    const int run_bits = T + ub;
    uint32_t br[kIpt];
#pragma unroll
    for (int it = 0; it < kIpt; ++it) {
        const uint32_t j = (uint32_t)wv * kChunk + (uint32_t)it * 64 + (uint32_t)lane;
        br[it] = ~0u;
        if (j - first_off < nt) {
            const uint32_t dg = ub ? (uint32_t)((key_top<W, 2>(key[it]) << T) >> (64 - ub)) : 0u;
            const uint32_t bin = (seg[it] << ub) | dg, sh16 = (bin & 1u) * 16u;
            const uint32_t old = atomicAdd(&sh.hist[bin >> 1], 1u << sh16);
            br[it] = bin | (((old >> sh16) & 0xFFFFu) << 16);
        }
    }
    __syncthreads();
    {
        uint32_t wds[kWordsPerThread], run = 0;
#pragma unroll
        for (int i = 0; i < kWordsPerThread; ++i) {
            const uint32_t wi = (uint32_t)tid * kWordsPerThread + i;
            const uint32_t x = wi < n_words ? sh.hist[wi] : 0u;
            wds[i] = run | ((run + (x & 0xFFFFu)) << 16);
            run += (x & 0xFFFFu) + (x >> 16);
        }
        const uint32_t base = block_excl_scan<kSortThreads>(run, sh.scratch, nullptr);
#pragma unroll
        for (int i = 0; i < kWordsPerThread; ++i) {
            const uint32_t wi = (uint32_t)tid * kWordsPerThread + i;
            if (wi < n_words) sh.hist[wi] = wds[i] + base * 0x00010001u;
        }
    }
    __syncthreads();
#pragma unroll
    for (int it = 0; it < kIpt; ++it) {
        if (br[it] != ~0u) {
            const uint32_t bin = br[it] & 0xFFFFu;
            const uint32_t pos = ((sh.hist[bin >> 1] >> ((bin & 1u) * 16u)) & 0xFFFFu) + (br[it] >> 16);
#pragma unroll
            for (int w = 0; w < W; ++w) sh.keys[pos].w[w] = key[it].w[w];
        }
    }
    __syncthreads();
    if (lp.debug & 4) return;
    const bool skip = (lp.debug & 1) != 0;
    const bool masked = (lp.mask_last2 & lp.mask_last) != ~0u;
    bool done;
    if (run_bits > 32 && W > 1)
        done = masked ? finish_by_comparison<W, (W > 1 ? 1 : 0), true, 2>(sh, keys, first, nt, run_bits, lp.mask_last2, lp.mask_last, skip)
                      : finish_by_comparison<W, (W > 1 ? 1 : 0), false, 2>(sh, keys, first, nt, run_bits, lp.mask_last2, lp.mask_last, skip);
    else if (run_bits == 32 && W > 1)
        done = masked ? finish_by_comparison<W, (W > 1 ? 1 : 0), true, 1>(sh, keys, first, nt, run_bits, lp.mask_last2, lp.mask_last, skip)
                      : finish_by_comparison<W, (W > 1 ? 1 : 0), false, 1>(sh, keys, first, nt, run_bits, lp.mask_last2, lp.mask_last, skip);
    else
        done = masked ? finish_by_comparison<W, 0, true, 1>(sh, keys, first, nt, run_bits, lp.mask_last2, lp.mask_last, skip)
                      : finish_by_comparison<W, 0, false, 1>(sh, keys, first, nt, run_bits, lp.mask_last2, lp.mask_last, skip);
    if (!done) leave_to_lsd();
}

template <int W>
__global__ __launch_bounds__(kSortThreads, 8) void local_lsd_kernel(Key<W> *keys, const Key<W> *other, const uint64_t *start, const uint64_t *end,
                                                                    int stride, LocalPlan lp) {
    constexpr int kIpt = LocalCfg<W>::kIpt;
    __shared__ LocalShared<W> sh;
    const int tid = threadIdx.x;
    const uint64_t f = wave_uniform(start[(uint64_t)blockIdx.x * stride]), first = f & ~kSegInOther;
    const uint64_t cnt = wave_uniform(end[(uint64_t)blockIdx.x * stride]) - first;
    if (cnt > (uint64_t)LocalCfg<W>::kTile || cnt == 0) return;
    const uint32_t nt = (uint32_t)cnt;
    const Key<W> *in = (f & kSegInOther) ? other : keys;
    Key<W> key[kIpt];
    uint32_t seg[kIpt];
    const int n_seg_pass = tile_load<W>(sh, in, first, nt, lp.T, key, seg);
    const int n_pass = lp.n_low + n_seg_pass;
    tile_zero_counts<W>(sh);
    for (int pass = 0; pass < n_pass; ++pass) {
        const bool by_seg = pass >= lp.n_low;
        Digit d;
        d.pos = 0; d.bits = 8; d.bias = 0;
        if (!by_seg) d = lp.low_plan[pass];
        lds_pass<W>(sh, key, seg, nt, d, by_seg, by_seg ? 8 * (pass - lp.n_low) : 0, pass + 1 < n_pass);
    }
#pragma unroll
    for (int it = 0; it < kIpt; ++it) {
        uint32_t j = (uint32_t)it * kSortThreads + (uint32_t)tid;
        if (j < nt) keys[first + j] = sh.keys[j];
    }
}

template <int W>
__global__ __launch_bounds__(kSortThreads) void segment_lds_kernel(Key<W> *keys, const Key<W> *other, const uint64_t *start, const uint64_t *end,
                                                                    LocalPlan lp) {
    constexpr int TILE = BigCfg<W>::kTile > 0 ? BigCfg<W>::kTile : LocalCfg<W>::kTile, kIpt = TILE / kSortThreads, kChunk = TILE / kSortWaves;
    __shared__ LocalShared<W, TILE> sh;
    const int tid = threadIdx.x, lane = lane_id(), wv = wave_id();
    const uint64_t f = wave_uniform(start[blockIdx.x]), first = f & ~kSegInOther, cnt = wave_uniform(end[blockIdx.x]) - first;
    if (cnt <= (uint64_t)LocalCfg<W>::kTile || cnt > (uint64_t)BigCfg<W>::kTile) return;
    const uint32_t nt = (uint32_t)cnt;
    const Key<W> *in = (f & kSegInOther) ? other : keys;
    Key<W> key[kIpt];
    uint32_t seg[kIpt];
#pragma unroll
    for (int it = 0; it < kIpt; ++it) {
        const uint32_t j = (uint32_t)wv * kChunk + (uint32_t)it * 64 + (uint32_t)lane;
        seg[it] = 0;
        if (j < nt) key[it] = in[first + j];
    }
    tile_zero_counts<W, TILE>(sh);
    for (int pass = 0; pass < lp.n_low; ++pass) lds_pass<W, TILE>(sh, key, seg, nt, lp.low_plan[pass], false, 0, pass + 1 < lp.n_low);
#pragma unroll
    for (int it = 0; it < kIpt; ++it) {
        const uint32_t j = (uint32_t)it * kSortThreads + (uint32_t)tid;
        if (j < nt) keys[first + j] = sh.keys[j];
    }
}

template <int W>
__global__ __launch_bounds__(256) void segment_end_kernel(const Key<W> *keys, uint64_t n, int T, const uint64_t *big, uint64_t *big_end) {
    __shared__ unsigned long long s_end;
    const uint64_t start = big[blockIdx.x];
    const uint32_t pre = key_prefix<W>(keys[start], T);
    if (threadIdx.x == 0) s_end = ~0ull;
    __syncthreads();
    for (uint64_t base = start + 1; base < n; base += 256 * 16) {
        unsigned long long found = ~0ull;
        for (int i = 0; i < 16; ++i) {
            uint64_t idx = base + (uint64_t)i * 256 + threadIdx.x;
            if (idx < n && key_prefix<W>(keys[idx], T) != pre && (unsigned long long)idx < found) found = idx;
        }
        if (found != ~0ull) atomicMin(&s_end, found);
        __syncthreads();
        if (s_end != ~0ull) break;
    }
    __syncthreads();
    if (threadIdx.x == 0) big_end[blockIdx.x] = s_end == ~0ull ? n : s_end;
}

constexpr int kEmitThreads = 256;
constexpr int kEmitPerThread = 16;
constexpr int kEmitTile = kEmitThreads * kEmitPerThread;

template <int W>
__device__ __forceinline__ bool keys_equal(const Key<W> &x, const Key<W> &y) {
    bool eq = true;
#pragma unroll
    for (int j = 0; j < W; ++j) eq = eq && (x.w[j] == y.w[j]);
    return eq;
}
template <int W>
__device__ __forceinline__ bool same_km1(const Key<W> &x, const Key<W> &y, int k) {
    int full = (k - 1) >> 4, rem = (k - 1) & 15;
    bool eq = true;
#pragma unroll
    for (int j = 0; j < W; ++j) {
        if (j < full) eq = eq && (x.w[j] == y.w[j]);
        else if (j == full && rem > 0) eq = eq && ((x.w[j] >> (16 - rem) * 2) == (y.w[j] >> (16 - rem) * 2));
    }
    return eq;
}
template <int W>
__device__ __forceinline__ int key_a(const Key<W> &x, int k) {
    if ((x.w[W - 1] >> 3) & 1u) {
        int wi = (k - 1) >> 4, ci = (k - 1) & 15;
        uint32_t word = 0;
#pragma unroll
        for (int j = 0; j < W; ++j) if (j == wi) word = x.w[j];
        return (word >> (15 - ci) * 2) & 3;
    }
    return kDollar;
}
template <int W>
__device__ __forceinline__ int key_b(const Key<W> &x) { return x.w[W - 1] & 7u; }

constexpr int kRunBaseStepLog = 10;
struct RunStarts {
    uint32_t *lo;
    uint64_t *base;
};
__device__ __forceinline__ uint64_t run_full_start(const RunStarts &r, uint64_t s) {
    const uint64_t b = r.base[s >> kRunBaseStepLog];
    return b + (uint32_t)(r.lo[s] - (uint32_t)b);
}
__device__ __forceinline__ uint64_t run_length(const RunStarts &r, uint64_t s, uint64_t m, uint64_t n_items) {
    return s + 1 < m ? (uint64_t)(uint32_t)(r.lo[s + 1] - r.lo[s]) : n_items - run_full_start(r, s);
}

struct EmitChain {
    unsigned long long *state;
    uint32_t *ticket;
    uint32_t *error;
    unsigned long long *total;
};

template <int W, bool TICKET>
__global__ __launch_bounds__(kEmitThreads) void emit_compact_kernel(const Key<W> *keys, uint64_t n, int k, EmitChain chain, uint32_t n_tiles,
                                                                     RunStarts sub_start, uint8_t *sub_info) {
    __shared__ uint32_t s_cnt[kEmitPerThread * (kEmitThreads / 64)];
    __shared__ uint32_t s_scr[kEmitThreads / 64 + 1];
    __shared__ uint32_t s_tile;
    __shared__ unsigned long long s_base;
    const uint32_t tile = TICKET ? chain_ticket(chain.ticket, &s_tile) : blockIdx.x;
    uint64_t base = (uint64_t)tile * kEmitTile;
    const int lane = lane_id(), wv = wave_id();
    uint32_t headbits = 0;
    uint32_t rank_in_wave[kEmitPerThread];
    uint8_t info[kEmitPerThread];
#pragma unroll
    for (int it = 0; it < kEmitPerThread; ++it) {
        uint64_t idx = base + (uint64_t)it * kEmitThreads + threadIdx.x;
        bool head = false;
        info[it] = 0;
        if (idx < n) {
            Key<W> cur = keys[idx];
            bool ghead = true, bhead = true;
            if (idx == 0) head = true;
            else {
                Key<W> prv = keys[idx - 1];
                head = !keys_equal<W>(cur, prv);
                ghead = !same_km1<W>(cur, prv, k);
                bhead = (cur.w[0] >> 16) != (prv.w[0] >> 16);
            }
            info[it] = (uint8_t)(key_a<W>(cur, k) | (key_b<W>(cur) << 3) | ((int)ghead << 6) | ((int)bhead << 7));
        }
        uint64_t bal = __ballot(head);
        rank_in_wave[it] = (uint32_t)__popcll(bal & lanemask_lt());
        headbits |= (uint32_t)head << it;
        if (lane == 0) s_cnt[it * (kEmitThreads / 64) + wv] = (uint32_t)__popcll(bal);
    }
    __syncthreads();
    uint32_t v = threadIdx.x < kEmitPerThread * (kEmitThreads / 64) ? s_cnt[threadIdx.x] : 0, tile_total = 0;
    uint32_t ex = block_excl_scan<kEmitThreads>(v, s_scr, &tile_total);
    __syncthreads();
    if (threadIdx.x < kEmitPerThread * (kEmitThreads / 64)) s_cnt[threadIdx.x] = ex;
    if (wv == 0) {
        const uint64_t before = chain_exclusive(chain.state, tile, tile_total, chain.error);
        if (lane == 0) {
            s_base = before;
            if (tile + 1 == n_tiles) *chain.total = before + tile_total;
        }
    }
    __syncthreads();
    uint64_t tb = s_base;
#pragma unroll
    for (int it = 0; it < kEmitPerThread; ++it) {
        if ((headbits >> it) & 1u) {
            uint64_t idx = base + (uint64_t)it * kEmitThreads + threadIdx.x;
            uint64_t s = tb + s_cnt[it * (kEmitThreads / 64) + wv] + rank_in_wave[it];
            sub_start.lo[s] = (uint32_t)idx;
            if ((s & ((1u << kRunBaseStepLog) - 1)) == 0) sub_start.base[s >> kRunBaseStepLog] = idx;
            sub_info[s] = info[it];
        }
    }
}

constexpr int kDecideThreads = 256;
constexpr int kDecidePerThread = 4;
constexpr int kDecideTile = kDecideThreads * kDecidePerThread;
constexpr int kDecideHalo = 32;

__device__ __forceinline__ bool run_suppressed(int a, int b, int has_a, int has_b) {
    return (a == kDollar && ((has_b >> b) & 1)) || (b == kDollar && ((has_a >> a) & 1));
}

__global__ __launch_bounds__(kDecideThreads) void emit_decide_kernel(RunStarts sub_start, const uint8_t *sub_info, uint64_t m,
                                                                      uint64_t n_items, uint16_t *rec, uint32_t *cnt_e,
                                                                      uint32_t *cnt_l, uint32_t *cnt_t) {
    __shared__ uint32_t s_e[kDecideThreads / 64], s_l[kDecideThreads / 64], s_t[kDecideThreads / 64];
    __shared__ uint8_t s_info[kDecideTile + 2 * kDecideHalo];
    const uint64_t t0 = (uint64_t)blockIdx.x * kDecideTile;
    const uint64_t w_lo = t0 >= (uint64_t)kDecideHalo ? t0 - kDecideHalo : 0;
    const uint64_t w_hi = t0 + kDecideTile + kDecideHalo < m ? t0 + kDecideTile + kDecideHalo : m;
    for (uint64_t x = w_lo + threadIdx.x; x < w_hi; x += kDecideThreads) s_info[x - w_lo] = sub_info[x];
    __syncthreads();
    auto info_at = [&](uint64_t x) -> int { return (x >= w_lo && x < w_hi) ? (int)s_info[x - w_lo] : (int)sub_info[x]; };
    uint32_t ne = 0, nl = 0, nt = 0;
    for (int q = 0; q < kDecidePerThread; ++q) {
        uint64_t s = t0 + (uint64_t)q * kDecideThreads + threadIdx.x;
        if (s >= m) break;
        int inf = info_at(s);
        int a = inf & 7, b = (inf >> 3) & 7;
        int has_a = 0, has_b = 0;
        auto collect = [&](int xi) {
            const int xa = xi & 7, xb = (xi >> 3) & 7;
            if (xa != kDollar && xb != kDollar) { has_a |= 1 << xa; has_b |= 1 << xb; }
        };
        collect(inf);
        bool front_b_solid = false, front_b_dollar = false;
        uint64_t gs = s;
        for (int gi = inf; !(gi & 64);) {
            --gs; gi = info_at(gs); collect(gi);
            if (((gi >> 3) & 7) == b) { if ((gi & 7) != kDollar) front_b_solid = true; else front_b_dollar = true; }
        }
        uint64_t ge = s + 1;
        while (ge < m) {
            const int xi = info_at(ge);
            if (xi & 64) break;
            collect(xi);
            ++ge;
        }
        uint16_t r = 0xFFFF;
        if (!run_suppressed(a, b, has_a, has_b)) {
            const bool seen_b = front_b_solid || (front_b_dollar && !((has_b >> b) & 1));
            int w = (b == kDollar) ? 0 : (seen_b ? b + 5 : b + 1);
            int last = 0;
            if (a != kDollar) {
                bool later = false;
                for (uint64_t x = s + 1; x < ge; ++x) {
                    int xi = info_at(x), xa = xi & 7, xb = (xi >> 3) & 7;
                    if (xa == a && (xb != kDollar || !((has_a >> a) & 1))) later = true;
                }
                last = later ? 0 : 1;
            }
            uint64_t run = run_length(sub_start, s, m, n_items);
            uint32_t count = run > 65535 ? 65535u : (uint32_t)run;
            int tip = a == kDollar;
            r = (uint16_t)(w | (last << 4) | (tip << 5) | ((count > 255 ? 255u : count) << 8));
            ne++;
            nl += count > 254;
            nt += tip;
        }
        rec[s] = r;
    }
    ne = wave_sum(ne); nl = wave_sum(nl); nt = wave_sum(nt);
    if (lane_id() == 0) { s_e[wave_id()] = ne; s_l[wave_id()] = nl; s_t[wave_id()] = nt; }
    __syncthreads();
    if (threadIdx.x == 0) {
        uint32_t e = 0, l = 0, t = 0;
        for (int w = 0; w < kDecideThreads / 64; ++w) { e += s_e[w]; l += s_l[w]; t += s_t[w]; }
        cnt_e[blockIdx.x] = e; cnt_l[blockIdx.x] = l; cnt_t[blockIdx.x] = t;
    }
}

template <int W>
__global__ __launch_bounds__(kDecideThreads) void emit_write_kernel(const Key<W> *keys, RunStarts sub_start, const uint8_t *sub_info, const uint16_t *rec,
                                                                     uint64_t m, uint64_t n_items, const uint64_t *base_e,
                                                                     const uint64_t *base_l, const uint64_t *base_t, int words_per_tip,
                                                                     uint32_t b_lo, uint16_t *out_rec, uint16_t *out_large,
                                                                     uint32_t *out_tips, int64_t *bucket_first ) {
    __shared__ uint64_t s_scr[kDecideThreads / 64 + 1];
    uint64_t s0 = (uint64_t)blockIdx.x * kDecideTile + (uint64_t)threadIdx.x * kDecidePerThread;
    uint16_t r[kDecidePerThread];
    uint64_t packed = 0;
    uint32_t cnts[kDecidePerThread];
    for (int q = 0; q < kDecidePerThread; ++q) {
        uint64_t s = s0 + q;
        r[q] = 0xFFFF; cnts[q] = 0;
        if (s < m) {
            r[q] = rec[s];
            if (r[q] != 0xFFFF) {
                uint64_t run = run_length(sub_start, s, m, n_items);
                cnts[q] = run > 65535 ? 65535u : (uint32_t)run;
                packed += 1ull + ((uint64_t)(cnts[q] > 254) << 20) + ((uint64_t)((r[q] >> 5) & 1) << 40);
            }
        }
    }
    uint64_t ex = block_excl_scan64<kDecideThreads>(packed, s_scr, nullptr);
    uint64_t ie = base_e[blockIdx.x] + (ex & 0xFFFFF), il = base_l[blockIdx.x] + ((ex >> 20) & 0xFFFFF),
             it = base_t[blockIdx.x] + (ex >> 40);
    for (int q = 0; q < kDecidePerThread; ++q) {
        uint64_t s = s0 + q;
        if (s >= m) break;
        const bool is_tip = r[q] != 0xFFFF && ((r[q] >> 5) & 1);
        const bool bucket_head = (sub_info[s] & 128) != 0;
        const uint64_t first_item = (is_tip || bucket_head) ? run_full_start(sub_start, s) : 0;
        if (bucket_head) {
            uint32_t bucket = keys[first_item].w[0] >> 16;
            int64_t *bf = bucket_first + (uint64_t)(bucket - b_lo) * 3;
            bf[0] = (int64_t)ie; bf[1] = (int64_t)il; bf[2] = (int64_t)it;
        }
        if (r[q] != 0xFFFF) {
            out_rec[ie++] = r[q];
            if (cnts[q] > 254) out_large[il++] = (uint16_t)cnts[q];
            if ((r[q] >> 5) & 1) {
                for (int j = 0; j < words_per_tip; ++j) out_tips[it * words_per_tip + j] = keys[first_item].w[j];
                it++;
            }
        }
    }
}

}
#include "sdbg_solid.hpp"
namespace mgta {

static std::vector<Digit> low_digit_plan(int k, int W, int T) {
    std::vector<Digit> plan;
    int pad = 32 * W - 2 * k - 4, top = 32 * W - T;
    if (top > 0) plan.push_back(Digit{0, std::min(4, top)});
    for (int pos = 4 + pad; pos < top; pos += 8) plan.push_back(Digit{pos, std::min(8, top - pos)});
    return plan;
}

template <class T>
static T *pool_get(mgta_ctx *ctx, int slot, uint64_t bytes) {
    if ((int)ctx->pool.size() < S_NUM) ctx->pool.resize(S_NUM);
    DevBuf &b = ctx->pool[slot];
    if (b.bytes < bytes || !b.p) {
        b.release();
        b.alloc(bytes + bytes / 8, &ctx->live_bytes, &ctx->peak_bytes);
    }
    return b.as<T>();
}
static uint64_t pool_bytes(const mgta_ctx *ctx) {
    uint64_t t = 0;
    for (const DevBuf &b : ctx->pool) t += b.bytes;
    return t;
}

struct SortModes {
    int bias = 1, side = 1, fused = 1, wide = 1;
    static SortModes from_env() {
        const char *bias = getenv("MGTA_SORT_BIAS"), *side = getenv("MGTA_SORT_SIDE"), *fused = getenv("MGTA_SORT_FUSED"), *wide = getenv("MGTA_SORT_WIDE");
        return SortModes{bias ? atoi(bias) : 1, side ? atoi(side) : 1, fused ? atoi(fused) : 1, wide ? atoi(wide) : 1};
    }
};

static double avg_segment_len(uint64_t n_items, int p, double prefix_frac) { return (double)n_items / std::max(1.0, std::pow(256.0, p) * prefix_frac); }
static double avg_segment_len_bits(uint64_t n_items, int bits, double prefix_frac) { return (double)n_items / std::max(1.0, std::pow(2.0, bits) * prefix_frac); }
constexpr int kMaxTop = 4;
struct TopPlan {
    int P = 0, skip = 0;
    uint32_t bias = 0;
    double frac = 1.0;
    int width[kMaxTop] = {8, 8, 8, 8};
    int key_bits() const { int t = 0; for (int i = 0; i < P; ++i) t += width[i]; return t; }
    int T() const { return key_bits() + skip; }
    int n_wide() const { int c = 0; for (int i = 0; i < P; ++i) c += width[i] > 8; return c; }
    int max_width() const { int m = 8; for (int i = 0; i < P; ++i) m = std::max(m, width[i]); return m; }
    bool same_digits(const TopPlan &o) const {
        bool same = P == o.P && skip == o.skip && bias == o.bias;
        for (int i = 0; same && i < P; ++i) same = width[i] == o.width[i];
        return same;
    }
    Digit pass_digit(int W, int i) const {
        int below = skip;
        for (int j = 0; j <= i; ++j) below += width[j];
        return Digit{32 * W - below, width[i], bias};
    }
    double avg_segment(uint64_t n_items) const { return avg_segment_len_bits(n_items, key_bits(), frac); }
};
static TopPlan choose_top_plan(const mgta_ctx *ctx, uint64_t n_items, int max_top, double prefix_frac, uint32_t b_lo = 0, uint32_t b_hi = 0,
                               int mode = 0) {
    TopPlan plain;
    plain.frac = prefix_frac;
    if (ctx && ctx->force_full_lsd) return plain;
    while (plain.P < max_top && avg_segment_len(n_items, plain.P, prefix_frac) > (plain.P >= 3 ? 700.0 : 256.0)) ++plain.P;
    if (mode == 0 || b_hi <= b_lo || (b_lo == 0 && b_hi >= (uint32_t)MGTA_NUM_BUCKETS)) return plain;
    const uint32_t span = ((b_hi - b_lo) << 16) - 1u;
    const int skip_full = __builtin_clz(span | 1u);
    for (int P = 1; P <= max_top; ++P) {
        const int skip = std::min(skip_full, 32 - 8 * P);
        if (skip <= 0 || 8 * P + skip < 16) continue;
        const double frac = std::min(1.0, prefix_frac * std::pow(2.0, skip));
        const double limit = mode >= 2 ? (P >= 3 ? 700.0 : 256.0) : (P >= 3 ? 400.0 : 256.0);
        if (P < max_top && avg_segment_len(n_items, P, frac) > limit) continue;
        if (P < plain.P || (mode >= 2 && P <= plain.P)) return TopPlan{P, skip, b_lo << 16, frac};
        break;
    }
    return plain;
}

static TopPlan widen_top_plan(const TopPlan &base, uint64_t n_items, int max_top, double prefix_frac, uint32_t b_lo, uint32_t b_hi, int bias_mode,
                              int wide) {
    const int max_bits = 8 * std::min(max_top, kMaxTop);
    if (wide <= 0 || base.P < 2) return base;
    if (wide >= 2) {
        TopPlan tp = base;
        for (int i = 0; i < tp.P - 1 && tp.key_bits() < max_bits; ++i) tp.width[i] = 9;
        if (tp.key_bits() + tp.skip > max_bits) {
            tp.skip = max_bits - tp.key_bits();
            if (tp.skip < 0 || (tp.skip > 0 && tp.T() < 16)) return base;
            if (tp.skip == 0) tp.bias = 0;
            tp.frac = std::min(1.0, prefix_frac * std::pow(2.0, tp.skip));
        }
        return tp;
    }
    if (base.P < 3) return base;
    TopPlan tp;
    tp.P = base.P - 1;
    for (int i = 0; i < tp.P - 1; ++i) tp.width[i] = 9;
    const bool sub_range = bias_mode != 0 && b_hi > b_lo && !(b_lo == 0 && b_hi >= (uint32_t)MGTA_NUM_BUCKETS);
    const int skip_full = sub_range ? __builtin_clz((((b_hi - b_lo) << 16) - 1u) | 1u) : 0;
    tp.skip = std::max(0, std::min(skip_full, max_bits - tp.key_bits()));
    if (tp.skip > 0 && tp.T() < 16) tp.skip = 0;
    tp.bias = tp.skip > 0 ? b_lo << 16 : 0u;
    tp.frac = std::min(1.0, prefix_frac * std::pow(2.0, tp.skip));
    if (tp.key_bits() > max_bits || tp.avg_segment(n_items) > 256.0) return base;
    return tp;
}

template <int WT>
struct SortJob {
    Key<WT> *a = nullptr, *b = nullptr;
    uint64_t n = 0;
    TopPlan top;
    std::vector<Digit> low;
    uint32_t mask_last2 = ~0u, mask_last = ~0u;
    int side_mode = 1;
    bool census_done = false;
    bool side_done = false;
    bool first_pass_done = false;
    bool uses_side() const { return side_mode > 0 && top.P >= 2 && kSideFits<WT>; }
    uint64_t side_bytes() const { return n * (top.max_width() > 8 ? 2u : 1u) + 64; }
    uint64_t hist_bytes() const { return std::max<uint64_t>(1, (n + kBlockTile - 1) / kBlockTile) * ((uint64_t)8 << top.max_width()); }
};
static uint64_t *digit_totals(mgta_ctx *ctx) { return pool_get<uint64_t>(ctx, S_DIGIT_TOTALS, 1024 * 8); }
struct SortLog {
    mgta_build_stats *S = nullptr;
    std::vector<Timer> scatter;
};

template <int WT, int BITS, int NEXT_BITS>
static bool global_pass(mgta_ctx *ctx, const SortJob<WT> &job, SortLog *log, const Key<WT> *src, Key<WT> *dst, Digit dg, Digit dn, bool first,
                        bool side_valid, bool write_side, void *d_side, uint64_t *d_hist, uint64_t *d_totals) {
    hipStream_t stream = ctx->stream;
    const uint64_t n = job.n, tiles = (n + kBlockTile - 1) / kBlockTile;
    constexpr uint64_t kVals = 1ull << BITS;
    const dim3 grid((unsigned)tiles), block(kSortThreads);
    if (!(first && job.census_done)) {
        if (side_valid) {
            hipLaunchKernelGGL((radix_census_side_kernel<BITS>), grid, block, 0, stream, static_cast<const SideEntry<BITS> *>(d_side), n, tiles, d_hist);
            if (job.side_mode >= 2) {
                std::vector<uint64_t> h_side(tiles * kVals), h_keys(tiles * kVals);
                MGTA_HIP_CHECK(hipStreamSynchronize(stream));
                MGTA_HIP_CHECK(hipMemcpy(h_side.data(), d_hist, tiles * kVals * 8, hipMemcpyDeviceToHost));
                hipLaunchKernelGGL((radix_census_kernel<WT, BITS>), grid, block, 0, stream, src, n, dg, tiles, d_hist);
                MGTA_HIP_CHECK(hipStreamSynchronize(stream));
                MGTA_HIP_CHECK(hipMemcpy(h_keys.data(), d_hist, tiles * kVals * 8, hipMemcpyDeviceToHost));
                if (h_side != h_keys) { set_error("internal: side-digit census differs from the census of the keys"); return false; }
            }
        } else
            hipLaunchKernelGGL((radix_census_kernel<WT, BITS>), grid, block, 0, stream, src, n, dg, tiles, d_hist);
    }
    hipLaunchKernelGGL(radix_rowscan_kernel, dim3((unsigned)kVals), dim3(1024), 0, stream, d_hist, tiles, d_totals);
    if (log) log->scatter.emplace_back(stream).start();
    auto launch = [&](auto biased, auto side, auto stable) {
        constexpr bool kSide = decltype(side)::value;
        hipLaunchKernelGGL((radix_scatter_kernel<WT, decltype(biased)::value, kSide, decltype(stable)::value, BITS, kSide ? NEXT_BITS : 8>), grid, block, 0, stream,
                           src, dst, n, dg, tiles, d_hist, d_totals, kSide ? static_cast<SideEntry<kSide ? NEXT_BITS : 8> *>(d_side) : nullptr, dn);
    };
    auto pick_stable = [&](auto biased, auto side) {
        if constexpr (BITS == 8) {
            if (first) { launch(biased, side, std::false_type{}); return; }
        }
        launch(biased, side, std::true_type{});
    };
    auto pick_side = [&](auto biased) {
        if constexpr (kScatterFits<WT, BITS, NEXT_BITS>) {
            if (write_side) { pick_stable(biased, std::true_type{}); return; }
        }
        pick_stable(biased, std::false_type{});
    };
    dg.bias ? pick_side(std::true_type{}) : pick_side(std::false_type{});
    if (log) {
        log->scatter.back().end();
        log->S->n_sort_launches++;
        if (BITS > 8) log->S->n_wide_passes++;
    }
    return true;
}

template <int WT>
static Key<WT> *global_passes(mgta_ctx *ctx, const SortJob<WT> &job, SortLog *log) {
    uint64_t *d_hist = pool_get<uint64_t>(ctx, S_HIST, job.hist_bytes());
    uint64_t *d_totals = digit_totals(ctx);
    void *d_side = job.uses_side() ? pool_get<uint8_t>(ctx, S_SIDE, job.side_bytes()) : nullptr;
    bool side_valid = job.side_done && d_side;
    Key<WT> *src = job.a, *dst = job.b;
    for (int i = job.top.P - 1 - (job.first_pass_done ? 1 : 0); i >= 0; --i) {
        const bool first = i == job.top.P - 1;
        const Digit dg = job.top.pass_digit(WT, i), dn = i > 0 ? job.top.pass_digit(WT, i - 1) : Digit{0, 0, 0};
        const bool write_side = d_side && i > 0;
        const int bits = dg.bits, next = i > 0 ? dn.bits : 8;
        bool ok = false, known = true;
        auto run = [&](auto b, auto nb) {
            ok = global_pass<WT, decltype(b)::value, decltype(nb)::value>(ctx, job, log, src, dst, dg, dn, first, side_valid, write_side, d_side, d_hist, d_totals);
        };
        using std::integral_constant;
        if (bits == 8 && next == 8) run(integral_constant<int, 8>{}, integral_constant<int, 8>{});
        else if constexpr (kWideFits<WT>) {
            if (bits == 8 && next == 9) run(integral_constant<int, 8>{}, integral_constant<int, 9>{});
            else if (bits == 9 && (next == 9 || i == 0)) run(integral_constant<int, 9>{}, integral_constant<int, 9>{});
            else known = false;
        } else
            known = false;
        if (!known) { set_error("internal: no scatter kernel for a %d-bit digit before a %d-bit one at %d key words", bits, next, WT); return nullptr; }
        if (!ok) return nullptr;
        side_valid = write_side;
        std::swap(src, dst);
    }
    return src;
}

template <int WT> constexpr uint32_t kLdsCap = BigCfg<WT>::kTile > 0 ? BigCfg<WT>::kTile : LocalCfg<WT>::kTile;
template <int WT>
static uint64_t split_list_bytes(uint64_t n_items) { return split_list_caps(n_items, LocalCfg<WT>::kTile, kLdsCap<WT>).bytes(); }

template <int WT>
static int split_oversized(mgta_ctx *ctx, const SortJob<WT> &job, Key<WT> *src, Key<WT> *dst, const uint64_t *seg_first, const uint64_t *seg_end,
                           uint32_t n_seg, const LocalPlan &lp) {
    hipStream_t stream = ctx->stream;
    const SplitCaps caps = split_list_caps(job.n, LocalCfg<WT>::kTile, kLdsCap<WT>);
    if (caps.n_small > 0xFFFFFFFFull) { set_error("too many keys for the lists of the oversized segments"); return -1; }
    uint64_t *d_lists = pool_get<uint64_t>(ctx, S_SPLIT, caps.bytes());
    uint64_t *at = d_lists;
    auto take = [&](uint64_t entries) { SegList l{at, at + entries, nullptr, (uint32_t)entries}; at += 2 * entries; return l; };
    SegList small = take(caps.n_small), mid = take(caps.n_mid), next[2] = {take(caps.n_next), take(caps.n_next)};
    uint32_t *d_counts = reinterpret_cast<uint32_t *>(at);
    small.count = d_counts; mid.count = d_counts + 1; next[0].count = next[1].count = d_counts + 2;
    int levels = 0;
    const int n_low = (int)job.low.size();
    for (int level = 0; level < n_low && n_seg > 0; ++level) {
        MGTA_HIP_CHECK(hipMemsetAsync(d_counts, 0, 16, stream));
        const SplitLists out{small, mid, next[level & 1], d_counts + 3};
        hipLaunchKernelGGL((segment_split_kernel<WT>), dim3(n_seg), dim3(kSortThreads), 0, stream, src, dst, seg_first, seg_end, job.low[n_low - 1 - level],
                           (uint32_t)LocalCfg<WT>::kTile, kLdsCap<WT>, out);
        uint32_t h[4] = {0, 0, 0, 0};
        MGTA_HIP_CHECK(hipMemcpyAsync(h, d_counts, 16, hipMemcpyDeviceToHost, stream));
        MGTA_HIP_CHECK(hipStreamSynchronize(stream));
        if (h[0] > small.cap || h[1] > mid.cap || h[2] > out.next.cap) {
            set_error("internal: list overflow of the oversized segments at level %d (%u / %u / %u entries)", level, h[0], h[1], h[2]);
            return -1;
        }
        if (h[3] > 0) ++levels;
        if (h[0] > 0) hipLaunchKernelGGL((local_lsd_kernel<WT>), dim3(h[0]), dim3(kSortThreads), 0, stream, src, dst, small.first, small.end, 1, lp);
        if (h[1] > 0) hipLaunchKernelGGL((segment_lds_kernel<WT>), dim3(h[1]), dim3(kSortThreads), 0, stream, src, dst, mid.first, mid.end, lp);
        seg_first = out.next.first; seg_end = out.next.end; n_seg = h[2];
    }
    if (n_seg > 0) hipLaunchKernelGGL((segment_copy_kernel<WT>), dim3(n_seg), dim3(kSortThreads), 0, stream, src, dst, seg_first, seg_end);
    return levels;
}

template <int WT>
static Key<WT> *lds_finish(mgta_ctx *ctx, const SortJob<WT> &job, Key<WT> *src, Key<WT> *dst, SortLog *log) {
    hipStream_t stream = ctx->stream;
    const uint64_t n_items = job.n;
    const int T = job.top.T();
    const std::vector<Digit> &low = job.low;
    if (low.size() > 64) { set_error("too many sort digits"); return nullptr; }
    Digit *d_plan = pool_get<Digit>(ctx, S_PLAN, 64 * sizeof(Digit));
    MGTA_HIP_CHECK(hipMemcpyAsync(d_plan, low.data(), low.size() * sizeof(Digit), hipMemcpyHostToDevice, stream));
    const double avg_seg = job.top.avg_segment(n_items);
    uint32_t margin = (uint32_t)std::min<double>(LocalCfg<WT>::kTile / 2, std::max<double>(LocalCfg<WT>::kTile / 8, 2.5 * avg_seg));
    margin = (margin + 63u) & ~63u;
    const uint32_t stride = (uint32_t)LocalCfg<WT>::kTile - margin;
    const uint64_t l_blocks = (n_items + stride - 1) / stride;
    if (l_blocks > 0x7FFFFFFFull) { set_error("too many sort tiles"); return nullptr; }
    const uint32_t big_cap = (uint32_t)l_blocks + 1;
    uint64_t *d_big = pool_get<uint64_t>(ctx, S_BIG, (2 * (uint64_t)big_cap + 2) * 8);
    uint32_t *d_big_count = reinterpret_cast<uint32_t *>(d_big + 2 * (uint64_t)big_cap);
    MGTA_HIP_CHECK(hipMemsetAsync(d_big_count, 0, 8, stream));
    uint64_t *d_lsd = pool_get<uint64_t>(ctx, S_LSD, 2 * l_blocks * 8);
    Timer t(stream);
    t.start();
    const bool skip_a = ctx->lsd_skip_left > 0;
    if (skip_a) --ctx->lsd_skip_left;
    const int ub = ((ctx->force_lsd_tiles & 1) || skip_a) ? 0 : std::max(0, std::min(8, (WT > 1 ? 40 : 32) - T));
    LocalPlan lp;
    lp.low_plan = d_plan; lp.n_low = (int)low.size(); lp.T = T;
    lp.upper = Digit{32 * WT - T - ub, ub};
    lp.mask_last2 = job.mask_last2; lp.mask_last = job.mask_last; lp.stride = stride;
    lp.lsd_list = d_lsd; lp.lsd_count = d_big_count + 1; lp.lsd_cap = (uint32_t)l_blocks;
    lp.debug = ctx->force_lsd_tiles >> 1;
    if (ub > 0)
        hipLaunchKernelGGL((local_sort_kernel<WT, true>), dim3((unsigned)l_blocks), dim3(kSortThreads), 0, stream, src, n_items, lp, d_big, d_big_count,
                           big_cap);
    else
        hipLaunchKernelGGL((local_sort_kernel<WT, false>), dim3((unsigned)l_blocks), dim3(kSortThreads), 0, stream, src, n_items, lp, d_big, d_big_count,
                           big_cap);
    t.end();
    uint32_t n_big = 0, n_lsd_tiles = 0;
    MGTA_HIP_CHECK(hipMemcpyAsync(&n_lsd_tiles, d_big_count + 1, 4, hipMemcpyDeviceToHost, stream));
    MGTA_HIP_CHECK(hipMemcpyAsync(&n_big, d_big_count, 4, hipMemcpyDeviceToHost, stream));
    MGTA_HIP_CHECK(hipStreamSynchronize(stream));
    const float ms_local = t.ms();
    if (n_big > big_cap) { set_error("more than %u oversized key segments in one pass", big_cap); return nullptr; }
    if (n_lsd_tiles > lp.lsd_cap) { set_error("internal: tile list overflow"); return nullptr; }
    if (ub > 0 && l_blocks >= 64 && 2 * (uint64_t)n_lsd_tiles > l_blocks) ctx->lsd_skip_left = 7;
    t.start();
    if (n_lsd_tiles > 0 && !(lp.debug & 2))
        hipLaunchKernelGGL((local_lsd_kernel<WT>), dim3(n_lsd_tiles), dim3(kSortThreads), 0, stream, src, dst, d_lsd, d_lsd + 1, 2, lp);
    if (n_big > 0) {
        hipLaunchKernelGGL((segment_end_kernel<WT>), dim3(n_big), dim3(256), 0, stream, src, n_items, T, d_big, d_big + big_cap);
        hipLaunchKernelGGL((local_lsd_kernel<WT>), dim3(n_big), dim3(kSortThreads), 0, stream, src, dst, d_big, d_big + big_cap, 1, lp);
        const bool use_big = BigCfg<WT>::kTile > 0 && !low.empty();
        if (use_big) hipLaunchKernelGGL((segment_lds_kernel<WT>), dim3(n_big), dim3(kSortThreads), 0, stream, src, dst, d_big, d_big + big_cap, lp);
        if (!low.empty()) {
            const int levels = split_oversized<WT>(ctx, job, src, dst, d_big, d_big + big_cap, n_big, lp);
            if (levels < 0) return nullptr;
            ctx->split_levels = std::max(ctx->split_levels, levels);
        }
    }
    t.end();
    MGTA_HIP_CHECK(hipEventSynchronize(t.b));
    const float ms = t.ms();
    if (log) { log->S->ms_local_sort += ms_local + ms; log->S->n_lsd_tiles += n_lsd_tiles; log->S->n_big_segments += n_big; }
    return src;
}

template <int WT>
static Key<WT> *device_sort(mgta_ctx *ctx, const SortJob<WT> &job, SortLog *log = nullptr) {
    Key<WT> *src = global_passes(ctx, job, log);
    return src ? lds_finish(ctx, job, src, src == job.a ? job.b : job.a, log) : nullptr;
}

template <int W>
static int run_stage1(mgta_ctx *ctx, const mgta_reads *rd, uint64_t n_short, int k, int min_count, int need_mercy, uint64_t budget,
                      int side_mode, unsigned long long **is_solid_out, int *num_k1_out) {
    constexpr int WT = W + 2;
    hipStream_t stream = ctx->stream;
    const uint64_t n_reads = rd->n_reads;
    const uint64_t n_blocks = (n_reads + kReadsPerBlock - 1) / kReadsPerBlock;
    uint64_t *d_small = pool_get<uint64_t>(ctx, S_SMALL, 4096);
    uint64_t *d_total = d_small;
    unsigned int *d_maxlen = reinterpret_cast<unsigned int *>(d_small + 300);
    unsigned long long *d_mercy_count = reinterpret_cast<unsigned long long *>(d_small + 302), *d_num_mercy = d_mercy_count + 1;
    MGTA_HIP_CHECK(hipMemsetAsync(d_small + 300, 0, 64, stream));
    if (n_short > n_reads) n_short = n_reads;
    if (n_short) hipLaunchKernelGGL(max_len_kernel, dim3((unsigned)((n_short + 255) / 256)), dim3(256), 0, stream, rd->d_start, n_short, d_maxlen);
    unsigned int max_len = 0;
    MGTA_HIP_CHECK(hipMemcpyAsync(&max_len, d_maxlen, 4, hipMemcpyDeviceToHost, stream));
    MGTA_HIP_CHECK(hipStreamSynchronize(stream));
    if (n_reads >= 0xFFFFFFFFull) { set_error("stage 1: more than 2^32 reads"); return MGTA_EUNSUPPORTED; }
    const uint64_t bases_bound = rd->n_words * 16 + 16;
    const uint64_t n_pos_entries = (bases_bound >> kPosStepLog) + 2;
    uint32_t *d_pos2id = pool_get<uint32_t>(ctx, S_POS2ID, n_pos_entries * 4);
    hipLaunchKernelGGL(pos_to_id_kernel, dim3((unsigned)((n_pos_entries + 255) / 256)), dim3(256), 0, stream, rd->d_start, n_reads, n_pos_entries, d_pos2id);
    int cand_shift = 0;
    while (cand_shift < 40 && (((bases_bound << 2) | 3ull) << (cand_shift + 1)) >> (cand_shift + 1) == ((bases_bound << 2) | 3ull)) ++cand_shift;
    const int num_k1 = std::max<int>(0, (int)max_len - k);
    const uint64_t n_bits = (uint64_t)num_k1 * n_short;
    unsigned long long *d_solid = pool_get<unsigned long long>(ctx, S_SOLID, (n_bits / 64 + 2) * 8);
    MGTA_HIP_CHECK(hipMemsetAsync(d_solid, 0, (n_bits / 64 + 2) * 8, stream));
    unsigned long long *d_edge_count = pool_get<unsigned long long>(ctx, S_EDGE_COUNT, 65536 * 8);
    MGTA_HIP_CHECK(hipMemsetAsync(d_edge_count, 0, 65536 * 8, stream));
    uint32_t *d_block_count = pool_get<uint32_t>(ctx, S_BLOCK_COUNT, std::max<uint64_t>(1, n_blocks) * 4);
    uint64_t *d_block_base = pool_get<uint64_t>(ctx, S_BLOCK_BASE, std::max<uint64_t>(1, n_blocks) * 8);

    S1Args sa;
    sa.packed = rd->d_packed; sa.n_words = rd->n_words; sa.start = rd->d_start; sa.n_reads = n_reads; sa.k = k;
    sa.block_count = d_block_count; sa.block_base = d_block_base; sa.out = nullptr;
    Key<2> *d_mercy = nullptr;
    uint64_t mercy_cap = 0;
    int n_pass = 1;
    uint32_t b_lo = 0;
    while (b_lo < MGTA_NUM_BUCKETS) {
        uint32_t width = (MGTA_NUM_BUCKETS + n_pass - 1) / n_pass;
        uint32_t b_hi = std::min<uint32_t>(MGTA_NUM_BUCKETS, b_lo + width);
        sa.b_lo = b_lo; sa.b_hi = b_hi;
        uint64_t *d_scan_tmp = pool_get<uint64_t>(ctx, S_SCAN_TMP, scan_tmp_elems(std::max<uint64_t>(n_blocks, 1024)) * 8);
        if (n_blocks) hipLaunchKernelGGL((s1_scan_kernel<W, false>), dim3((unsigned)n_blocks), dim3(kScanBlock), 0, stream, sa);
        exclusive_scan_u32(stream, d_block_count, n_blocks, d_block_base, d_scan_tmp, d_total);
        uint64_t n_items = 0;
        MGTA_HIP_CHECK(hipMemcpyAsync(&n_items, d_total, 8, hipMemcpyDeviceToHost, stream));
        MGTA_HIP_CHECK(hipStreamSynchronize(stream));
        uint64_t n_tiles = (n_items + kBlockTile - 1) / kBlockTile;
        uint64_t need = 2 * n_items * sizeof(Key<WT>) + n_tiles * 256 * 8 + (need_mercy ? n_items * 8 : 0) + (8u << 20);
        uint64_t other = ctx->live_bytes - pool_bytes(ctx);
        if (need + need / 8 > budget - std::min<uint64_t>(budget, other) && width > 1) { n_pass *= 2; continue; }
        if (n_items > 0) {
            Key<WT> *d_a = pool_get<Key<WT>>(ctx, S_KEYS_A, n_items * sizeof(Key<WT>));
            Key<WT> *d_b = pool_get<Key<WT>>(ctx, S_KEYS_B, n_items * sizeof(Key<WT>));
            if (need_mercy && (!d_mercy || mercy_cap < 2 * n_items)) {
                uint64_t have = 0;
                MGTA_HIP_CHECK(hipMemcpy(&have, d_mercy_count, 8, hipMemcpyDeviceToHost));
                uint64_t new_cap = have + 2 * n_items;
                DevBuf keep;
                if (have) { keep.alloc(have * 8); MGTA_HIP_CHECK(hipMemcpy(keep.p, d_mercy, have * 8, hipMemcpyDeviceToDevice)); }
                d_mercy = pool_get<Key<2>>(ctx, S_MERCY, new_cap * 8);
                if (have) MGTA_HIP_CHECK(hipMemcpy(d_mercy, keep.p, have * 8, hipMemcpyDeviceToDevice));
                mercy_cap = new_cap;
            }
            sa.out = d_a;
            hipLaunchKernelGGL((s1_scan_kernel<W, true>), dim3((unsigned)n_blocks), dim3(kScanBlock), 0, stream, sa);
            const int pad1 = 32 * W - 2 * (k - 1) - 6;
            auto low_plan = [&](int T) {
                std::vector<Digit> plan;
                int top = 32 * WT - T;
                plan.push_back(Digit{0, 6});
                if (top > 64) plan.push_back(Digit{64, std::min(6, top - 64)});
                for (int pos = 64 + 6 + pad1; pos < top; pos += 8) plan.push_back(Digit{pos, std::min(8, top - pos)});
                return plan;
            };
            const int max_top = std::min(4, std::max(0, (2 * (k - 1)) / 8));
            SortJob<WT> job{d_a, d_b, n_items, choose_top_plan(ctx, n_items, max_top, (double)(b_hi - b_lo) / MGTA_NUM_BUCKETS)};
            job.low = low_plan(job.top.T()); job.mask_last2 = 0u; job.mask_last = 0x3Fu; job.side_mode = side_mode;
            Key<WT> *sorted = device_sort(ctx, job);
            if (!sorted) return MGTA_EUNSUPPORTED;
            char *scratch = reinterpret_cast<char *>(sorted == d_a ? d_b : d_a);
            uint64_t e_tiles = (n_items + kEmitTile - 1) / kEmitTile;
            uint32_t *d_tile_heads = pool_get<uint32_t>(ctx, S_TILE_HEADS, e_tiles * 4);
            uint64_t *d_tile_base = pool_get<uint64_t>(ctx, S_TILE_BASE, e_tiles * 8);
            d_scan_tmp = pool_get<uint64_t>(ctx, S_SCAN_TMP, scan_tmp_elems(std::max<uint64_t>(n_blocks, e_tiles)) * 8);
            hipLaunchKernelGGL((s1_mark_kernel<W>), dim3((unsigned)e_tiles), dim3(kEmitThreads), 0, stream, sorted, n_items, d_tile_heads);
            exclusive_scan_u32(stream, d_tile_heads, e_tiles, d_tile_base, d_scan_tmp, d_total);
            uint64_t m = 0;
            MGTA_HIP_CHECK(hipMemcpyAsync(&m, d_total, 8, hipMemcpyDeviceToHost, stream));
            MGTA_HIP_CHECK(hipStreamSynchronize(stream));
            uint64_t *run_start = reinterpret_cast<uint64_t *>(scratch);
            uint16_t *run_info = reinterpret_cast<uint16_t *>(scratch + m * 8);
            uint16_t *group_mask = reinterpret_cast<uint16_t *>(scratch + m * 10);
            hipLaunchKernelGGL((s1_compact_kernel<W>), dim3((unsigned)e_tiles), dim3(kEmitThreads), 0, stream, sorted, n_items, k, d_tile_base,
                               run_start, run_info);
            unsigned rb = (unsigned)((m + 255) / 256);
            hipLaunchKernelGGL(s1_group_kernel, dim3(rb), dim3(256), 0, stream, run_start, run_info, m, n_items, min_count, group_mask);
            hipLaunchKernelGGL((s1_apply_kernel<W>), dim3(std::min(rb, 8192u)), dim3(256), 0, stream, sorted, run_start, run_info, group_mask, m, n_items, min_count,
                               k, rd->d_start, n_reads, n_short, num_k1, d_solid, d_edge_count, d_mercy, d_mercy_count, mercy_cap, need_mercy,
                               d_pos2id, cand_shift);
        }
        b_lo = b_hi;
    }
    ctx->edge_counting.assign(65536, 0);
    MGTA_HIP_CHECK(hipMemcpyAsync(ctx->edge_counting.data(), d_edge_count, 65536 * 8, hipMemcpyDeviceToHost, stream));
    MGTA_HIP_CHECK(hipStreamSynchronize(stream));
    if (need_mercy) {
        uint64_t n_cand = 0;
        MGTA_HIP_CHECK(hipMemcpy(&n_cand, d_mercy_count, 8, hipMemcpyDeviceToHost));
        if (n_cand > mercy_cap) { set_error("mercy candidate list overflow"); return MGTA_ENOMEM; }
        if (n_cand > 0) {
            Key<2> *d_tmp = pool_get<Key<2>>(ctx, S_KEYS_A, n_cand * 8);
            auto low64 = [&](int T) {
                std::vector<Digit> plan;
                for (int pos = 0; pos < 64 - T; pos += 8) plan.push_back(Digit{pos, std::min(8, 64 - T - pos)});
                return plan;
            };
            SortJob<2> job{d_mercy, d_tmp, n_cand, choose_top_plan(ctx, n_cand, 4, 1.0)};
            job.low = low64(job.top.T()); job.side_mode = side_mode;
            Key<2> *cs = device_sort(ctx, job);
            if (!cs) return MGTA_EUNSUPPORTED;
            if ((int)max_len <= kMercyMaxLen) {
                hipLaunchKernelGGL(mercy_kernel<false>, dim3((unsigned)((n_cand + 255) / 256)), dim3(256), 0, stream, cs, n_cand, rd->d_start, n_reads, k,
                                   num_k1, d_solid, d_num_mercy, d_pos2id, cand_shift, (uint8_t *)nullptr, (uint64_t)0);
                MGTA_HIP_CHECK(hipGetLastError());
                MGTA_HIP_CHECK(hipStreamSynchronize(stream));
            } else {
                const uint64_t stride = ((uint64_t)max_len + 64 + 63) & ~63ull;
                const unsigned grid = (unsigned)std::min<uint64_t>((n_cand + 255) / 256, (uint64_t)ctx->num_cus * 8);
                DevBuf d_flags;
                d_flags.alloc((uint64_t)grid * 4 * 3 * stride, &ctx->live_bytes, &ctx->peak_bytes);
                hipLaunchKernelGGL(mercy_kernel<true>, dim3(grid), dim3(256), 0, stream, cs, n_cand, rd->d_start, n_reads, k, num_k1, d_solid,
                                   d_num_mercy, d_pos2id, cand_shift, d_flags.as<uint8_t>(), stride);
                MGTA_HIP_CHECK(hipGetLastError());
                MGTA_HIP_CHECK(hipStreamSynchronize(stream));
            }
        }
    }
    *is_solid_out = d_solid;
    *num_k1_out = num_k1;
    return MGTA_OK;
}

struct Pass {
    uint32_t b_lo = 0, b_hi = 0, width = 0;
    bool closed_form = false;
    uint64_t n_items = 0, n_tiles = 0, key_b = 0;
    uint64_t n_edges = 0, n_large = 0, n_tips = 0;
    uint16_t *rec = nullptr, *large = nullptr;
    uint32_t *tips = nullptr;
    int64_t *first = nullptr;
    uint32_t nb() const { return b_hi - b_lo; }
};

template <int W>
struct Build {
    mgta_ctx *ctx;
    hipStream_t stream = ctx->stream;
    const mgta_reads *rd = nullptr;
    uint64_t n_short = 0, n_blocks = 0;
    int k = 0, words_per_tip = 0, min_count = 1, need_mercy = 0;
    uint32_t bucket_begin = 0, bucket_end = 0;
    mgta_edge_sink sink = nullptr; void *user = nullptr;
    SortModes modes;
    uint64_t budget = 0;
    bool acc = false;
    ScanArgs sa{};
    uint64_t *d_block_base = nullptr, *d_total = nullptr, *d_kmers = nullptr, *d_tot3 = nullptr, *d_sentinel = nullptr;
    uint32_t multi_n = 0, multi_width = 0, multi_lo = 0;
    uint32_t *d_multi_count = nullptr;
    struct FusedAhead { bool on = false; TopPlan top; };
    FusedAhead fz_plan[kMaxFusedRanges];
    uint64_t *fz_table = nullptr;
    uint64_t wide_items = 0;
    uint32_t wide_nb = 0;
    bool fz_check_failed = false;
    mgta_build_stats S{};
    Timer t_all{stream}, t_ph{stream};
    SortLog log{&S, {}};
    std::vector<int64_t> h_first, h_items;
    std::vector<uint16_t> h_rec, h_large;
    std::vector<uint32_t> h_tips;
    explicit Build(mgta_ctx *c) : ctx(c) {}

    int run() {
        int rc = start();
        if (rc == MGTA_OK) rc = solid_from_stage1();
        if (rc != MGTA_OK) return rc;
        t_all.start();
        int n_pass = 1;
        for (uint32_t b_lo = bucket_begin; b_lo < bucket_end;) {
            Pass p;
            p.width = (bucket_end - bucket_begin + n_pass - 1) / n_pass;
            p.b_lo = b_lo; p.b_hi = std::min<uint32_t>(bucket_end, b_lo + p.width);
            count_pass(p);
            if (const int more = admit_pass(p, n_pass)) { n_pass = more; wide_items = p.n_items; wide_nb = p.nb(); continue; }
            S.n_items += (int64_t)p.n_items;
            S.n_passes++;
            if (p.n_items > 0) {
                Key<W> *a = pool_get<Key<W>>(ctx, S_KEYS_A, p.key_b), *b = pool_get<Key<W>>(ctx, S_KEYS_B, p.key_b);
                const SortJob<W> job = plan_sort(p, a, b);
                write_keys(p, job);
                if (fz_check_failed) { set_error("internal: the fused key writer left keys outside the slice of their first sort digit"); return MGTA_EINTERNAL; }
                Key<W> *sorted = sort_keys(job);
                if (!sorted) return MGTA_EUNSUPPORTED;
                if ((rc = drop_sentinels(p)) != MGTA_OK || (rc = emit(p, sorted, sorted == a ? b : a)) != MGTA_OK) return rc;
            }
            publish_last(p.b_lo, p.b_hi, p.rec, p.n_edges, p.tips, p.n_tips, p.first, p.large, p.n_large);
            if (acc && p.n_items > 0) append_to_stream(p);
            S.n_edges += (int64_t)p.n_edges; S.n_large += (int64_t)p.n_large; S.n_tips += (int64_t)p.n_tips;
            if ((rc = deliver_pass(p)) != MGTA_OK) return rc;
            b_lo = p.b_hi;
        }
        if (acc) publish_last(bucket_begin, bucket_end, ctx->acc_rec.p, ctx->acc_n_rec, ctx->acc_tips.p, ctx->acc_n_tips, nullptr,
                              ctx->acc_has_large ? ctx->acc_large.p : nullptr, ctx->acc_n_large);
        ctx->acc_valid = acc;
        S.ms_total = t_all.stop();
        for (const Timer &t : log.scatter) S.ms_sort_scatter += t.ms();
        S.bytes_peak = ctx->peak_bytes;
        S.n_split_levels = ctx->split_levels;
        return MGTA_OK;
    }

    int start() {
        words_per_tip = (2 * k + 31) / 32;
        n_blocks = (rd->n_reads + kReadsPerBlock - 1) / kReadsPerBlock;
        if (n_blocks * (uint64_t)kScanBlock >= (1ull << 32)) { set_error("too many reads for one launch (%llu)", (unsigned long long)rd->n_reads); return MGTA_EUNSUPPORTED; }
        S.k = k; S.words_per_key = W; S.words_per_tip = words_per_tip; S.n_reads = (int64_t)rd->n_reads;
        ctx->peak_bytes = ctx->live_bytes;
        ctx->split_levels = 0;
        size_t free_b = 0, total_b = 0;
        MGTA_HIP_CHECK(hipMemGetInfo(&free_b, &total_b));
        const uint64_t avail = (uint64_t)free_b + pool_bytes(ctx);
        budget = ctx->mem_limit ? std::min<uint64_t>(ctx->mem_limit, avail) : (uint64_t)(avail * 0.9);
        acc = ctx->keep_stream != 0;
        ctx->acc_valid = false; ctx->acc_n_rec = 0; ctx->acc_n_tips = 0;
        ctx->acc_n_large = 0; ctx->acc_has_large = acc && ctx->keep_multiplicity;
        if (acc) ctx->acc_items.assign(MGTA_NUM_BUCKETS, 0);
        point_scans_at_pool();
        uint64_t *d_small = pool_get<uint64_t>(ctx, S_SMALL, 4096);
        d_total = d_small; d_kmers = d_small + 1; d_tot3 = d_small + 2; d_sentinel = d_small + 5;
        sa.packed = rd->d_packed; sa.n_words = rd->n_words; sa.start = rd->d_start; sa.n_reads = rd->n_reads; sa.k = k; sa.n_short = n_short;
        sa.n_kmers = (unsigned long long *)d_kmers; sa.n_sentinel = (unsigned long long *)d_sentinel;
        return MGTA_OK;
    }
    void point_scans_at_pool() {
        sa.block_count = pool_get<uint32_t>(ctx, S_BLOCK_COUNT, std::max<uint64_t>(1, n_blocks) * 4);
        sa.block_base = d_block_base = pool_get<uint64_t>(ctx, S_BLOCK_BASE, std::max<uint64_t>(1, n_blocks) * 8);
    }

    int solid_from_stage1() {
        if (min_count <= 1) return MGTA_OK;
        unsigned long long *sol = nullptr;
        int nk1 = 0;
        t_ph.start();
        const int rc = run_stage1<W>(ctx, rd, n_short, k, min_count, need_mercy, budget, modes.side, &sol, &nk1);
        if (rc != MGTA_OK) return rc;
        S.ms_stage1 = t_ph.stop();
        sa.is_solid = sol; sa.num_k1_per_read = nk1;
        point_scans_at_pool();
        return MGTA_OK;
    }

    void count_pass(Pass &p) {
        const bool first_pass = S.n_passes == 0;
        t_ph.start();
        sa.b_lo = p.b_lo; sa.b_hi = p.b_hi;
        sa.n_kmers = first_pass ? (unsigned long long *)d_kmers : nullptr;
        if (first_pass) MGTA_HIP_CHECK(hipMemsetAsync(d_kmers, 0, 8, stream));
        uint64_t *d_scan_tmp = pool_get<uint64_t>(ctx, S_SCAN_TMP, scan_tmp_elems(std::max<uint64_t>(n_blocks, 1024)) * 8);
        static_assert(kReadsPerBlock == 64, "item_count_closed_kernel: one lane per read of a workgroup");
        p.closed_form = !sa.is_solid && p.b_lo == 0 && p.b_hi == (uint32_t)MGTA_NUM_BUCKETS && !ctx->force_full_lsd;
        const uint32_t *counts = sa.block_count;
        sa.multi_n = 0; sa.multi_width = 0; sa.multi_magic = 0;
        if (n_blocks && (p.closed_form || sa.n_kmers))
            hipLaunchKernelGGL(item_count_closed_kernel, dim3((unsigned)((n_blocks + 63) / 64)), dim3(256), 0, stream, sa.start, sa.n_reads, n_blocks, k,
                               p.closed_form ? sa.block_count : nullptr, sa.n_kmers);
        if (n_blocks && !p.closed_form) {
            sa.n_kmers = nullptr;
            const uint32_t width = p.width, b_lo = p.b_lo, ranges_left = (bucket_end - b_lo + width - 1) / width;
            if (multi_n && (width != multi_width || b_lo < multi_lo || (b_lo - multi_lo) % width != 0 || (b_lo - multi_lo) / width >= multi_n)) multi_n = 0;
            if (!multi_n && ranges_left > 1 && ranges_left <= (uint32_t)kMaxCountRanges) {
                d_multi_count = pool_get<uint32_t>(ctx, S_MULTI_COUNT, (uint64_t)ranges_left * n_blocks * 4);
                ScanArgs sm = sa;
                sm.block_count = d_multi_count; sm.b_hi = bucket_end; sm.multi_width = width; sm.multi_n = ranges_left; sm.multi_magic = ((1ull << 32) + width - 1) / width;
                fz_table = nullptr;
                if (plan_ahead(sm, b_lo, width, ranges_left)) {
                    fz_table = sm.fz_hist = pool_get<uint64_t>(ctx, S_FUSED_HIST, fused_table_bytes(ranges_left));
                    if constexpr (W >= 2)
                        hipLaunchKernelGGL((item_scan_kernel<W, false, true>), dim3((unsigned)n_blocks), dim3(kScanBlock), 0, stream, sm);
                } else
                    hipLaunchKernelGGL((item_scan_kernel<W, false>), dim3((unsigned)n_blocks), dim3(kScanBlock), 0, stream, sm);
                multi_n = ranges_left; multi_width = width; multi_lo = b_lo;
            }
            if (multi_n) counts = d_multi_count + (uint64_t)((b_lo - multi_lo) / width) * n_blocks;
            else hipLaunchKernelGGL((item_scan_kernel<W, false>), dim3((unsigned)n_blocks), dim3(kScanBlock), 0, stream, sa);
        }
        exclusive_scan_u32(stream, counts, n_blocks, d_block_base, d_scan_tmp, d_total);
        MGTA_HIP_CHECK(hipMemcpyAsync(&p.n_items, d_total, 8, hipMemcpyDeviceToHost, stream));
        S.ms_count += t_ph.stop();
        if (first_pass) {
            unsigned long long km = 0;
            MGTA_HIP_CHECK(hipMemcpy(&km, d_kmers, 8, hipMemcpyDeviceToHost));
            S.n_kmers = (int64_t)km;
        }
    }

    int max_top() const { return (2 * k + 4 + 7) / 8 > 1 ? std::min(4, (32 * W - 8) / 8) : 0; }
    TopPlan top_plan(uint64_t n_items, uint32_t b_lo, uint32_t b_hi) const {
        const double frac = (double)(b_hi - b_lo) / MGTA_NUM_BUCKETS;
        const TopPlan tp = choose_top_plan(ctx, n_items, max_top(), frac, b_lo, b_hi, modes.bias);
        if (!kWideFits<W> || ctx->force_full_lsd) return tp;
        return widen_top_plan(tp, n_items, max_top(), frac, b_lo, b_hi, modes.bias, modes.wide);
    }
    uint64_t fused_table_bytes(uint32_t ranges) const { return (uint64_t)ranges * 256 * std::max<uint64_t>(1, n_blocks) * 8; }

    bool plan_ahead(ScanArgs &sm, uint32_t b_lo, uint32_t width, uint32_t ranges) {
        for (FusedAhead &f : fz_plan) f = FusedAhead{};
        if (modes.fused <= 0 || W < 2 || !wide_nb || ranges > (uint32_t)kMaxFusedRanges) return false;
        bool any = false;
        int max_width = 8;
        uint64_t est_max = 0;
        for (uint32_t g = 0; g < ranges; ++g) {
            const uint32_t lo = b_lo + g * width, hi = std::min<uint32_t>(bucket_end, lo + width);
            const uint64_t est = (uint64_t)((double)wide_items * (double)(hi - lo) / (double)wide_nb);
            const TopPlan tp = top_plan(est, lo, hi);
            est_max = std::max(est_max, est);
            max_width = std::max(max_width, tp.max_width());
            sm.fz_bias[g] = 0; sm.fz_shift[g] = 0;
            if (tp.P < 1 || tp.T() > 32) continue;
            fz_plan[g] = FusedAhead{true, tp};
            sm.fz_bias[g] = tp.bias; sm.fz_shift[g] = (uint32_t)(32 - tp.T());
            any = true;
        }
        if (!any) return false;
        uint64_t key_b = 0;
        const uint64_t need = pass_need(est_max, &key_b, max_width) + fused_table_bytes(ranges);
        return need + need / 8 <= avail_bytes();
    }

    uint64_t pass_need(uint64_t n_items, uint64_t *key_b, int max_width) const {
        const uint64_t n_tiles = (n_items + kBlockTile - 1) / kBlockTile;
        *key_b = std::max<uint64_t>(n_items * sizeof(Key<W>), n_items * 12) + 4096;
        return 2 * *key_b + n_tiles * ((uint64_t)8 << max_width) + n_items * 2 + n_items * (max_width > 8 ? 2 : 1)  + split_list_bytes<W>(n_items) +
               (8u << 20);
    }
    uint64_t avail_bytes() const {
        uint64_t other = ctx->live_bytes - pool_bytes(ctx);
        if (acc) {
            const double range_frac = (double)(bucket_end - bucket_begin) / (double)MGTA_NUM_BUCKETS;
            const uint64_t est = (uint64_t)((double)S.n_kmers * 1.5 * range_frac) + (64ull << 20);
            const uint64_t have = ctx->acc_rec.bytes + ctx->acc_tips.bytes;
            other += est > have ? est - have : 0;
        }
        return budget - std::min<uint64_t>(budget, other);
    }

    int admit_pass(Pass &p, int n_pass) {
        p.n_tiles = (p.n_items + kBlockTile - 1) / kBlockTile;
        uint64_t need = pass_need(p.n_items, &p.key_b, top_plan(p.n_items, p.b_lo, p.b_hi).max_width());
        const uint64_t avail = avail_bytes();
        if ((int)ctx->pool.size() > S_FUSED_HIST && ctx->pool[S_FUSED_HIST].bytes) {
            const uint64_t with = need + ctx->pool[S_FUSED_HIST].bytes;
            if (with + with / 8 <= avail) need = with;
            else if (need + need / 8 <= avail) { ctx->pool[S_FUSED_HIST].release(); fz_table = nullptr; }
        }
        if (need + need / 8 <= avail || p.width <= 1) return 0;
        const double ratio = (double)(need + need / 8) / (double)std::max<uint64_t>(avail, 1) * 1.03;
        return std::max(n_pass + 1, (int)std::ceil((double)n_pass * ratio));
    }

    SortJob<W> plan_sort(const Pass &p, Key<W> *a, Key<W> *b) const {
        SortJob<W> job{a, b, p.n_items, top_plan(p.n_items, p.b_lo, p.b_hi)};
        job.low = low_digit_plan(k, W, job.top.T());
        job.side_mode = modes.side;
        job.census_done = p.closed_form && job.top.P >= 1 && p.n_tiles <= 0x7FFFFFFFull;
        job.side_done = !p.closed_form && job.uses_side();
        if (!p.closed_form && fz_table && multi_n && p.width == multi_width && p.b_lo >= multi_lo && (p.b_lo - multi_lo) % p.width == 0) {
            const uint32_t g = (p.b_lo - multi_lo) / p.width;
            if (g < multi_n && g < (uint32_t)kMaxFusedRanges) {
                const FusedAhead &f = fz_plan[g];
                job.first_pass_done = f.on && job.top.P >= 1 && f.top.same_digits(job.top);
            }
        }
        return job;
    }

    void write_keys(const Pass &p, const SortJob<W> &job) {
        t_ph.start();
        sa.out = job.a;
        if (p.closed_form) MGTA_HIP_CHECK(hipMemsetAsync(d_sentinel, 0, 8, stream));
        const int shift = 32 - job.top.T();
        if (job.census_done) {
            uint64_t *d_hist = pool_get<uint64_t>(ctx, S_HIST, job.hist_bytes());
            hipLaunchKernelGGL((item_write_tiled_kernel<W>), dim3((unsigned)p.n_tiles), dim3(kScanBlock), 0, stream, sa, n_blocks, p.n_items,
                               shift, p.n_tiles, d_hist);
        } else if (p.closed_form)
            hipLaunchKernelGGL((item_write_closed_kernel<W>), dim3((unsigned)n_blocks), dim3(kScanBlock), 0, stream, sa);
        else if (job.first_pass_done) {
            uint64_t *tab = fz_table + (uint64_t)((p.b_lo - multi_lo) / p.width) * 256 * n_blocks;
            uint64_t *d_totals = digit_totals(ctx);
            hipLaunchKernelGGL(radix_rowscan_kernel, dim3(256), dim3(1024), 0, stream, tab, n_blocks, d_totals);
            sa.fz_hist = tab; sa.fz_totals = d_totals; sa.fz_n = p.n_items;
            sa.fz_bias[0] = job.top.bias; sa.fz_shift[0] = (uint32_t)shift;
            if (job.side_done) {
                sa.side = pool_get<uint8_t>(ctx, S_SIDE, job.side_bytes());
                sa.side_shift = shift + 8;
                sa.side_bias = job.top.bias;
                sa.side_bits = job.top.P >= 2 ? job.top.width[job.top.P - 2] : 8;
            }
            if constexpr (W >= 2)
                hipLaunchKernelGGL((item_write_fused_kernel<W>), dim3((unsigned)n_blocks), dim3(kScanBlock), 0, stream, sa);
            sa.side = nullptr; sa.fz_hist = nullptr; sa.fz_totals = nullptr;
            S.n_fused_passes++;
            if (modes.fused >= 2) {
                uint32_t *d_bad = reinterpret_cast<uint32_t *>(pool_get<uint64_t>(ctx, S_SMALL, 4096) + 320);
                uint32_t bad[2] = {0, 0};
                MGTA_HIP_CHECK(hipMemsetAsync(d_bad, 0, 8, stream));
                const unsigned grid = (unsigned)std::min<uint64_t>((p.n_items + kScanBlock - 1) / kScanBlock, (uint64_t)ctx->num_cus * 16);
                hipLaunchKernelGGL((fused_check_kernel<W>), dim3(grid), dim3(kScanBlock), 0, stream, job.a, p.n_items, d_totals, job.top.bias, (uint32_t)shift, d_bad);
                MGTA_HIP_CHECK(hipMemcpyAsync(bad, d_bad, 8, hipMemcpyDeviceToHost, stream));
                MGTA_HIP_CHECK(hipStreamSynchronize(stream));
                if (bad[0] || bad[1]) fz_check_failed = true;
            }
        } else {
            if (job.side_done) {
                sa.side = pool_get<uint8_t>(ctx, S_SIDE, job.side_bytes());
                sa.side_shift = shift;
                sa.side_bias = job.top.bias;
                sa.side_bits = 8;
            }
            hipLaunchKernelGGL((item_scan_kernel<W, true>), dim3((unsigned)n_blocks), dim3(kScanBlock), 0, stream, sa);
            sa.side = nullptr;
        }
        S.ms_gen += t_ph.stop();
    }

    Key<W> *sort_keys(const SortJob<W> &job) {
        t_ph.start();
        Key<W> *sorted = device_sort(ctx, job, &log);
        if (sorted) S.ms_sort += t_ph.stop();
        return sorted;
    }

    int drop_sentinels(Pass &p) {
        if (!p.closed_form || ((k + 1) & 1)) return MGTA_OK;
        unsigned long long n_sent = 0;
        MGTA_HIP_CHECK(hipMemcpy(&n_sent, d_sentinel, 8, hipMemcpyDeviceToHost));
        if (n_sent >= p.n_items) { set_error("internal: %llu sentinel keys among %llu items", n_sent, (unsigned long long)p.n_items); return MGTA_EINTERNAL; }
        p.n_items -= n_sent;
        S.n_items -= (int64_t)n_sent;
        return MGTA_OK;
    }

    int emit(Pass &p, const Key<W> *sorted, Key<W> *scratch_keys) {
        const uint64_t n_items = p.n_items;
        t_ph.start();
        char *scratch = reinterpret_cast<char *>(scratch_keys);
        uint64_t e_tiles = (n_items + kEmitTile - 1) / kEmitTile;
        uint64_t *d_scan_tmp = pool_get<uint64_t>(ctx, S_SCAN_TMP, scan_tmp_elems(std::max<uint64_t>(std::max(n_blocks, e_tiles), n_items / kDecideTile + 1)) * 8);
        if (e_tiles > 0xFFFFFFFFull) { set_error("too many emit tiles"); return MGTA_EUNSUPPORTED; }
        unsigned long long *d_chain = pool_get<unsigned long long>(ctx, S_TILE_BASE, (e_tiles + 4) * 8);
        EmitChain chain;
        chain.state = d_chain; chain.total = d_chain + e_tiles;
        chain.ticket = reinterpret_cast<uint32_t *>(d_chain + e_tiles + 1); chain.error = reinterpret_cast<uint32_t *>(d_chain + e_tiles + 2);
        RunStarts sub_start;
        sub_start.lo = reinterpret_cast<uint32_t *>(scratch);
        uint16_t *rec = reinterpret_cast<uint16_t *>(scratch + n_items * 4);
        uint8_t *info = reinterpret_cast<uint8_t *>(scratch + n_items * 6);
        sub_start.base = reinterpret_cast<uint64_t *>(scratch + ((n_items * 7 + 7) & ~7ull));
        unsigned long long chain_out[3] = {0, 0, 0};
        for (int attempt = 0; attempt < 2; ++attempt) {
            MGTA_HIP_CHECK(hipMemsetAsync(d_chain, 0, (e_tiles + 4) * 8, stream));
            if (attempt == 0 && !ctx->force_full_lsd)
                hipLaunchKernelGGL((emit_compact_kernel<W, false>), dim3((unsigned)e_tiles), dim3(kEmitThreads), 0, stream, sorted, n_items, k, chain,
                                   (uint32_t)e_tiles, sub_start, info);
            else
                hipLaunchKernelGGL((emit_compact_kernel<W, true>), dim3((unsigned)e_tiles), dim3(kEmitThreads), 0, stream, sorted, n_items, k, chain,
                                   (uint32_t)e_tiles, sub_start, info);
            MGTA_HIP_CHECK(hipMemcpyAsync(chain_out, d_chain + e_tiles, 24, hipMemcpyDeviceToHost, stream));
            MGTA_HIP_CHECK(hipStreamSynchronize(stream));
            if ((uint32_t)chain_out[2] == 0) break;
        }
        if ((uint32_t)chain_out[2] != 0) { set_error("internal: chained scan of the emitter timed out"); return MGTA_EINTERNAL; }
        const uint64_t m = chain_out[0];
        uint64_t d_tiles = (m + kDecideTile - 1) / kDecideTile;
        uint32_t *ce = pool_get<uint32_t>(ctx, S_CNT, d_tiles * 4 * 3), *cl = ce + d_tiles, *ct = cl + d_tiles;
        uint64_t *be = pool_get<uint64_t>(ctx, S_BASE, d_tiles * 8 * 3), *bl = be + d_tiles, *bt = bl + d_tiles;
        p.first = pool_get<int64_t>(ctx, S_FIRST, (uint64_t)MGTA_NUM_BUCKETS * 3 * 8);
        MGTA_HIP_CHECK(hipMemsetAsync(p.first, 0xFF, (uint64_t)p.nb() * 3 * 8, stream));
        hipLaunchKernelGGL(emit_decide_kernel, dim3((unsigned)d_tiles), dim3(kDecideThreads), 0, stream, sub_start, info, m, n_items,
                           rec, ce, cl, ct);
        exclusive_scan_u32(stream, ce, d_tiles, be, d_scan_tmp, d_tot3);
        exclusive_scan_u32(stream, cl, d_tiles, bl, d_scan_tmp, d_tot3 + 1);
        exclusive_scan_u32(stream, ct, d_tiles, bt, d_scan_tmp, d_tot3 + 2);
        uint64_t tot3[3];
        MGTA_HIP_CHECK(hipMemcpyAsync(tot3, d_tot3, 24, hipMemcpyDeviceToHost, stream));
        MGTA_HIP_CHECK(hipStreamSynchronize(stream));
        p.n_edges = tot3[0]; p.n_large = tot3[1]; p.n_tips = tot3[2];
        p.rec = pool_get<uint16_t>(ctx, S_OUT_REC, p.n_edges * 2);
        p.large = pool_get<uint16_t>(ctx, S_OUT_LARGE, p.n_large * 2);
        p.tips = pool_get<uint32_t>(ctx, S_OUT_TIPS, p.n_tips * words_per_tip * 4);
        hipLaunchKernelGGL((emit_write_kernel<W>), dim3((unsigned)d_tiles), dim3(kDecideThreads), 0, stream, sorted, sub_start, info, rec, m,
                           n_items, be, bl, bt, words_per_tip, p.b_lo, p.rec, p.large, p.tips, p.first);
        S.ms_emit += t_ph.stop();
        return MGTA_OK;
    }

    void publish_last(uint32_t lo, uint32_t hi, const void *rec, uint64_t n_rec, const void *tips, uint64_t n_tips, const void *first,
                      const void *large, uint64_t n_large) {
        ctx->last_large = large; ctx->last_n_large = n_large;
        ctx->last_rec = rec; ctx->last_n_rec = n_rec; ctx->last_bucket_lo = lo; ctx->last_bucket_hi = hi;
        ctx->last_tips = tips; ctx->last_n_tips = n_tips; ctx->last_first = first; ctx->last_k = k; ctx->last_words_per_tip = words_per_tip;
    }

    void append_to_stream(const Pass &p) {
        const uint64_t tip_b = words_per_tip * 4;
        auto ensure = [&](DevBuf &buf, uint64_t used, uint64_t add) {
            if (used + add <= buf.bytes) return;
            const double done = (double)(p.b_hi - bucket_begin) / (double)(bucket_end - bucket_begin);
            uint64_t want = (uint64_t)((double)(used + add) / std::max(done, 1e-3) * 1.1) + (1u << 20);
            want = std::max<uint64_t>(want, used + add);
            DevBuf bigger;
            bigger.alloc(want, &ctx->live_bytes, &ctx->peak_bytes);
            if (used) MGTA_HIP_CHECK(hipMemcpyAsync(bigger.p, buf.p, used, hipMemcpyDeviceToDevice, stream));
            MGTA_HIP_CHECK(hipStreamSynchronize(stream));
            buf = std::move(bigger);
        };
        ensure(ctx->acc_rec, ctx->acc_n_rec * 2, p.n_edges * 2);
        ensure(ctx->acc_tips, ctx->acc_n_tips * tip_b, p.n_tips * tip_b);
        if (ctx->acc_has_large) {
            ensure(ctx->acc_large, ctx->acc_n_large * 2, p.n_large * 2);
            if (p.n_large) MGTA_HIP_CHECK(hipMemcpyAsync(ctx->acc_large.as<char>() + ctx->acc_n_large * 2, p.large, p.n_large * 2, hipMemcpyDeviceToDevice, stream));
        }
        if (p.n_edges) MGTA_HIP_CHECK(hipMemcpyAsync(ctx->acc_rec.as<char>() + ctx->acc_n_rec * 2, p.rec, p.n_edges * 2, hipMemcpyDeviceToDevice, stream));
        if (p.n_tips) MGTA_HIP_CHECK(hipMemcpyAsync(ctx->acc_tips.as<char>() + ctx->acc_n_tips * tip_b, p.tips, p.n_tips * tip_b, hipMemcpyDeviceToDevice, stream));
        h_first.resize((size_t)p.nb() * 3);
        MGTA_HIP_CHECK(hipMemcpyAsync(h_first.data(), p.first, (size_t)p.nb() * 3 * 8, hipMemcpyDeviceToHost, stream));
        MGTA_HIP_CHECK(hipStreamSynchronize(stream));
        int64_t nxt = (int64_t)p.n_edges;
        for (int64_t b = (int64_t)p.nb() - 1; b >= 0; --b) {
            int64_t f = h_first[(size_t)b * 3];
            if (f < 0) f = nxt;
            ctx->acc_items[(size_t)p.b_lo + (size_t)b] = nxt - f;
            nxt = f;
        }
        ctx->acc_n_rec += p.n_edges; ctx->acc_n_tips += p.n_tips; ctx->acc_n_large += p.n_large;
    }

    int deliver_pass(const Pass &p) {
        if (!sink) return MGTA_OK;
        const bool to_host = ctx->keep_stream != 2;
        const uint64_t n_tip_words = p.n_tips * words_per_tip;
        h_items.assign((size_t)p.nb() * 3, 0);
        if (p.n_items > 0) {
            t_ph.start();
            h_rec.resize(to_host ? p.n_edges : 0); h_large.resize(p.n_large); h_tips.resize(to_host ? n_tip_words : 0);
            h_first.resize((size_t)p.nb() * 3);
            if (p.n_edges && to_host) MGTA_HIP_CHECK(hipMemcpyAsync(h_rec.data(), p.rec, p.n_edges * 2, hipMemcpyDeviceToHost, stream));
            if (p.n_large) MGTA_HIP_CHECK(hipMemcpyAsync(h_large.data(), p.large, p.n_large * 2, hipMemcpyDeviceToHost, stream));
            if (p.n_tips && to_host) MGTA_HIP_CHECK(hipMemcpyAsync(h_tips.data(), p.tips, n_tip_words * 4, hipMemcpyDeviceToHost, stream));
            MGTA_HIP_CHECK(hipMemcpyAsync(h_first.data(), p.first, (size_t)p.nb() * 3 * 8, hipMemcpyDeviceToHost, stream));
            S.ms_d2h += t_ph.stop();
            int64_t nxt[3] = {(int64_t)p.n_edges, (int64_t)p.n_large, (int64_t)p.n_tips};
            for (int64_t b = (int64_t)p.nb() - 1; b >= 0; --b)
                for (int c = 0; c < 3; ++c) {
                    int64_t f = h_first[(size_t)b * 3 + c];
                    if (f < 0) f = nxt[c];
                    h_items[(size_t)b * 3 + c] = nxt[c] - f;
                    nxt[c] = f;
                }
        } else { h_rec.clear(); h_large.clear(); h_tips.clear(); }
        const int rc = sink(user, (int32_t)p.b_lo, (int32_t)p.b_hi, h_items.data(), to_host ? h_rec.data() : nullptr, (int64_t)p.n_edges,
                            h_large.data(), (int64_t)p.n_large, to_host ? h_tips.data() : nullptr, (int64_t)n_tip_words);
        if (rc != 0) { set_error("edge sink returned %d", rc); return MGTA_ESINK; }
        return MGTA_OK;
    }
};

template <int W = 1, class F>
static int with_key_words(int words, F &&f) {
    if constexpr (W < 9) {
        if (words == W) return f(std::integral_constant<int, W>{});
        return with_key_words<W + 1>(words, f);
    } else
        return f(std::integral_constant<int, W>{});
}

}

using namespace mgta;

extern "C" {

int mgta_reads_upload(mgta_ctx *ctx, const uint32_t *packed, uint64_t n_words, const uint64_t *start_idx, uint64_t n_reads,
                      mgta_reads **out) {
    if (!ctx || !packed || !start_idx || !out) { set_error("mgta_reads_upload: null argument"); return MGTA_EINVAL; }
    return guarded("mgta_reads_upload", [&] {
        MGTA_HIP_CHECK(hipSetDevice(ctx->device));
        auto r = std::make_unique<mgta_reads>();
        r->ctx = ctx; r->n_words = n_words; r->n_reads = n_reads;
        r->own_packed.alloc((n_words + 16) * 4, &ctx->live_bytes, &ctx->peak_bytes);
        r->own_start.alloc((n_reads + 1) * 8, &ctx->live_bytes, &ctx->peak_bytes);
        MGTA_HIP_CHECK(hipMemsetAsync((char *)r->own_packed.p + n_words * 4, 0, 64, ctx->stream));
        MGTA_HIP_CHECK(hipMemcpyAsync(r->own_packed.p, packed, n_words * 4, hipMemcpyHostToDevice, ctx->stream));
        MGTA_HIP_CHECK(hipMemcpyAsync(r->own_start.p, start_idx, (n_reads + 1) * 8, hipMemcpyHostToDevice, ctx->stream));
        MGTA_HIP_CHECK(hipStreamSynchronize(ctx->stream));
        r->d_packed = r->own_packed.as<uint32_t>();
        r->d_start = r->own_start.as<uint64_t>();
        ctx_retain(ctx);
        *out = r.release();
        return MGTA_OK;
    });
}

int mgta_reads_adopt_device(mgta_ctx *ctx, const uint32_t *d_packed, uint64_t n_words, const uint64_t *d_start, uint64_t n_reads,
                            mgta_reads **out) {
    if (!ctx || !d_packed || !d_start || !out) { set_error("mgta_reads_adopt_device: null argument"); return MGTA_EINVAL; }
    return guarded("mgta_reads_adopt_device", [&] {
        auto *r = new mgta_reads;
        r->ctx = ctx; r->d_packed = d_packed; r->d_start = d_start; r->n_words = n_words; r->n_reads = n_reads;
        ctx_retain(ctx);
        *out = r;
        return MGTA_OK;
    });
}

void mgta_reads_free(mgta_reads *r) {
    if (!r) return;
    mgta_ctx *c = r->ctx;
    delete r;
    ctx_release(c);
}

int mgta_sdbg_build_resident(mgta_ctx *ctx, const mgta_reads *rd, uint64_t n_short_reads, int k, int min_count, int need_mercy,
                             int32_t bucket_begin, int32_t bucket_end, mgta_edge_sink sink, void *user, mgta_build_stats *stats) {
    if (!ctx || !rd) { set_error("mgta_sdbg_build: null argument"); return MGTA_EINVAL; }
    if (k < 9 || k > 127) { set_error("k=%d out of range [9,127] (kMaxK, definitions.h:56)", k); return MGTA_EINVAL; }
    if (bucket_begin < 0 || bucket_end > MGTA_NUM_BUCKETS || bucket_begin >= bucket_end) {
        set_error("bucket range [%d,%d) invalid", bucket_begin, bucket_end);
        return MGTA_EINVAL;
    }
    if (min_count < 1) { set_error("min_count must be >= 1"); return MGTA_EINVAL; }
    return guarded("mgta_sdbg_build", [&] {
        MGTA_HIP_CHECK(hipSetDevice(ctx->device));
        return with_key_words((2 * k + 4 + 31) / 32, [&](auto w) {
            Build<decltype(w)::value> B(ctx);
            B.rd = rd; B.n_short = n_short_reads; B.k = k; B.min_count = min_count; B.need_mercy = need_mercy;
            B.bucket_begin = (uint32_t)bucket_begin; B.bucket_end = (uint32_t)bucket_end; B.sink = sink; B.user = user;
            B.modes = SortModes::from_env();
            const int rc = B.run();
            if (rc == MGTA_OK && stats) *stats = B.S;
            return rc;
        });
    });
}

int mgta_sdbg_last_counting(mgta_ctx *ctx, int64_t *hist) {
    if (!ctx || !hist) { set_error("mgta_sdbg_last_counting: null argument"); return MGTA_EINVAL; }
    if (ctx->edge_counting.size() != 65536) { set_error("no stage-1 run (min_count > 1) on this context yet"); return MGTA_EINVAL; }
    std::copy(ctx->edge_counting.begin(), ctx->edge_counting.end(), hist);
    return MGTA_OK;
}

int mgta_sort_plan(uint64_t n_items, int words_per_key, uint32_t bucket_begin, uint32_t bucket_end, int *n_passes, int *skip_bits) {
    if (!n_passes || !skip_bits || words_per_key < 2 || bucket_end > (uint32_t)MGTA_NUM_BUCKETS || bucket_begin >= bucket_end) {
        set_error("mgta_sort_plan: bad argument");
        return MGTA_EINVAL;
    }
    const TopPlan tp = choose_top_plan(nullptr, n_items, std::min(4, (32 * words_per_key - 8) / 8), (double)(bucket_end - bucket_begin) / MGTA_NUM_BUCKETS,
                                       bucket_begin, bucket_end, SortModes::from_env().bias);
    *n_passes = tp.P;
    *skip_bits = tp.skip;
    return MGTA_OK;
}

int mgta_sort_plan_wide(uint64_t n_items, int words_per_key, uint32_t bucket_begin, uint32_t bucket_end, int *n_passes, int *skip_bits, int *widths) {
    if (!n_passes || !skip_bits || !widths || words_per_key < 2 || bucket_end > (uint32_t)MGTA_NUM_BUCKETS || bucket_begin >= bucket_end) {
        set_error("mgta_sort_plan_wide: bad argument");
        return MGTA_EINVAL;
    }
    const SortModes modes = SortModes::from_env();
    const int max_top = std::min(4, (32 * words_per_key - 8) / 8);
    const double frac = (double)(bucket_end - bucket_begin) / MGTA_NUM_BUCKETS;
    TopPlan tp = choose_top_plan(nullptr, n_items, max_top, frac, bucket_begin, bucket_end, modes.bias);
    const bool fits = with_key_words(words_per_key, [&](auto w) { return (int)kWideFits<decltype(w)::value>; }) > 0;
    if (fits) tp = widen_top_plan(tp, n_items, max_top, frac, bucket_begin, bucket_end, modes.bias, modes.wide);
    *n_passes = tp.P;
    *skip_bits = tp.skip;
    for (int i = 0; i < kMaxTop; ++i) widths[i] = i < tp.P ? tp.width[tp.P - 1 - i] : 0;
    return MGTA_OK;
}

int mgta_sdbg_export_records_device(mgta_ctx *ctx, void *d_dst, uint64_t capacity_bytes, uint64_t *n_records) {
    if (!ctx || !n_records) { set_error("mgta_sdbg_export_records_device: null argument"); return MGTA_EINVAL; }
    *n_records = ctx->last_n_rec;
    if (ctx->last_k == 0 || (!ctx->last_rec && ctx->last_n_rec)) { set_error("no device-resident build output"); return MGTA_EINVAL; }
    if (!d_dst) return MGTA_OK;
    if (capacity_bytes < ctx->last_n_rec * 2) { set_error("destination too small"); return MGTA_EINVAL; }
    return guarded("mgta_sdbg_export_records_device", [&] {
        MGTA_HIP_CHECK(hipSetDevice(ctx->device));
        if (ctx->last_n_rec) MGTA_HIP_CHECK(hipMemcpyAsync(d_dst, ctx->last_rec, ctx->last_n_rec * 2, hipMemcpyDeviceToDevice, ctx->stream));
        MGTA_HIP_CHECK(hipStreamSynchronize(ctx->stream));
        return MGTA_OK;
    });
}

int mgta_sdbg_build(mgta_ctx *ctx, const uint32_t *packed, uint64_t n_words, const uint64_t *start_idx, uint64_t n_reads,
                    uint64_t n_short_reads, int k, int min_count, int need_mercy, mgta_edge_sink sink, void *user,
                    mgta_build_stats *stats) {
    mgta_reads *rd = nullptr;
    int rc = mgta_reads_upload(ctx, packed, n_words, start_idx, n_reads, &rd);
    if (rc != MGTA_OK) return rc;
    rc = mgta_sdbg_build_resident(ctx, rd, n_short_reads, k, min_count, need_mercy, 0, MGTA_NUM_BUCKETS, sink, user, stats);
    mgta_reads_free(rd);
    return rc;
}

}
```

Before: 9.589.

## Fuse emitter run-head info computation into the final local sort pass

The last local-sort pass now writes back keys in sorted order through shared memory and computes a per-key info byte (head flags, edge labels) alongside them. A new compaction kernel builds run starts from these info bytes with 16-byte loads, so the separate emitter no longer has to re-read full multi-word keys and their neighbours. This adds an extra shared-memory scatter and syncs in the sort epilogue, plus an info buffer. An optional verification mode recomputes the result the old way and compares the two.

```diff
diff --git a/include/megagta_hip.h b/include/megagta_hip.h
--- a/include/megagta_hip.h
+++ b/include/megagta_hip.h
@@ -83,6 +83,7 @@
                              int need_mercy, int32_t bucket_begin, int32_t bucket_end ,
                              mgta_edge_sink sink, void *user, mgta_build_stats *stats);
 int mgta_sdbg_last_counting(mgta_ctx *, int64_t *hist );
+int mgta_sdbg_last_emit_fused(mgta_ctx *, int64_t *n_passes);
 int mgta_sdbg_export_records_device(mgta_ctx *, void *d_dst, uint64_t capacity_bytes, uint64_t *n_records);
 int mgta_sdbg_build(mgta_ctx *, const uint32_t *packed_seq, uint64_t n_words, const uint64_t *start_idx,
                     uint64_t n_reads, uint64_t n_short_reads, int k, int min_count, int need_mercy,
diff --git a/megagta_amd/_lib.py b/megagta_amd/_lib.py
--- a/megagta_amd/_lib.py
+++ b/megagta_amd/_lib.py
@@ -233,6 +233,7 @@
     "mgta_sdbg_build_resident": (C.c_int, [C.c_void_p, C.c_void_p, C.c_uint64, C.c_int, C.c_int, C.c_int, C.c_int32, C.c_int32,
                                           EDGE_SINK, C.c_void_p, C.POINTER(BuildStats)]),
     "mgta_sdbg_last_counting": (C.c_int, [C.c_void_p, C.c_void_p]),
+    "mgta_sdbg_last_emit_fused": (C.c_int, [C.c_void_p, C.POINTER(C.c_int64)]),
     "mgta_sdbg_export_records_device": (C.c_int, [C.c_void_p, C.c_void_p, C.c_uint64, C.POINTER(C.c_uint64)]),
     "mgta_sdbg_build": (C.c_int, [C.c_void_p, C.c_void_p, C.c_uint64, C.c_void_p, C.c_uint64, C.c_uint64, C.c_int, C.c_int,
                                  C.c_int, EDGE_SINK, C.c_void_p, C.POINTER(BuildStats)]),
diff --git a/megagta_amd/api.py b/megagta_amd/api.py
--- a/megagta_amd/api.py
+++ b/megagta_amd/api.py
@@ -346,9 +346,13 @@
                                                cb, None, C.byref(st)),
               "mgta_sdbg_build_resident")
         cat = lambda xs, dt: np.concatenate(xs) if xs else np.zeros(0, dt)
+        stats = st.as_dict()
+        fused = C.c_int64(0)
+        check(self._L.mgta_sdbg_last_emit_fused(self.h, C.byref(fused)), "mgta_sdbg_last_emit_fused")
+        stats["n_emit_fused"] = fused.value
         return EdgeStream(k=k, words_per_tip=wpt, bucket_items=counts[:, 0].copy(), records=cat(recs, np.uint16),
                           large=cat(large, np.uint16), tips=cat(tips, np.uint32), bucket_large=counts[:, 1].copy(),
-                          bucket_tips=counts[:, 2].copy(), stats=st.as_dict())
+                          bucket_tips=counts[:, 2].copy(), stats=stats)
 
 
 def export_records_to_torch(ctx: "Context"):
diff --git a/megagta_amd/csrc/common.hpp b/megagta_amd/csrc/common.hpp
--- a/megagta_amd/csrc/common.hpp
+++ b/megagta_amd/csrc/common.hpp
@@ -101,6 +101,7 @@
     uint64_t mem_limit = 0;
     int force_full_lsd = 0;
     int lsd_skip_left = 0;
+    int64_t emit_fused_passes = 0;
     int split_levels = 0;
     int astar_log_b0 = 0;
     uint64_t astar_pool_bytes = 0;
diff --git a/megagta_amd/csrc/sdbg_build.hip b/megagta_amd/csrc/sdbg_build.hip
--- a/megagta_amd/csrc/sdbg_build.hip
+++ b/megagta_amd/csrc/sdbg_build.hip
@@ -1163,6 +1163,49 @@
 template <int W>
 __device__ __forceinline__ uint32_t key_prefix(const Key<W> &key, int T) { return T == 0 ? 0u : (key.w[0] >> (32 - T)); }
 
+template <int W>
+__device__ __forceinline__ bool keys_equal(const Key<W> &x, const Key<W> &y) {
+    bool eq = true;
+#pragma unroll
+    for (int j = 0; j < W; ++j) eq = eq && (x.w[j] == y.w[j]);
+    return eq;
+}
+template <int W>
+__device__ __forceinline__ bool same_km1(const Key<W> &x, const Key<W> &y, int k) {
+    int full = (k - 1) >> 4, rem = (k - 1) & 15;
+    bool eq = true;
+#pragma unroll
+    for (int j = 0; j < W; ++j) {
+        if (j < full) eq = eq && (x.w[j] == y.w[j]);
+        else if (j == full && rem > 0) eq = eq && ((x.w[j] >> (16 - rem) * 2) == (y.w[j] >> (16 - rem) * 2));
+    }
+    return eq;
+}
+template <int W>
+__device__ __forceinline__ int key_a(const Key<W> &x, int k) {
+    if ((x.w[W - 1] >> 3) & 1u) {
+        int wi = (k - 1) >> 4, ci = (k - 1) & 15;
+        uint32_t word = 0;
+#pragma unroll
+        for (int j = 0; j < W; ++j) if (j == wi) word = x.w[j];
+        return (word >> (15 - ci) * 2) & 3;
+    }
+    return kDollar;
+}
+template <int W>
+__device__ __forceinline__ int key_b(const Key<W> &x) { return x.w[W - 1] & 7u; }
+
+template <int W>
+__device__ __forceinline__ uint8_t head_info(const Key<W> &cur, int k, bool ghead, bool bhead) {
+    return (uint8_t)(key_a<W>(cur, k) | (key_b<W>(cur) << 3) | ((int)ghead << 6) | ((int)bhead << 7));
+}
+template <int W>
+__device__ __forceinline__ uint8_t key_info(const Key<W> &cur, const Key<W> &prv, int k, bool &head) {
+    head = !keys_equal<W>(cur, prv);
+    return head_info<W>(cur, k, !same_km1<W>(cur, prv, k), (cur.w[0] >> 16) != (prv.w[0] >> 16));
+}
+constexpr uint8_t kInfoNoHead = 7;
+
 struct LocalPlan {
     const Digit *low_plan;
     int n_low;
@@ -1175,6 +1218,8 @@
     uint32_t *lsd_count;
     uint32_t lsd_cap;
     int debug;
+    uint8_t *info;
+    int emit_k;
 };
 
 constexpr uint32_t kMaxAvgRun = 40;
@@ -1308,9 +1353,9 @@
     return PW == 1 ? (uint64_t)k.w[0] : (((uint64_t)k.w[0] << 32) | (uint64_t)k.w[W > 1 ? 1 : 0]);
 }
 
-template <int W, int FIRST, bool MASKED, int PW>
+template <int W, int FIRST, bool MASKED, int PW, bool INFO = false>
 __device__ __forceinline__ bool finish_by_comparison(CompareShared<W> &sh, Key<W> *keys, uint64_t first, uint32_t nt, int run_bits, uint32_t m2,
-                                                     uint32_t m1, bool skip_compare) {
+                                                     uint32_t m1, bool skip_compare, uint8_t *info = nullptr, int emit_k = 0, int emit_T = 0) {
     const int run_shift = 32 * PW - run_bits;
     constexpr int kIpt = LocalCfg<W>::kIpt, kWindows = LocalCfg<W>::kTile / 64;
     const int lane = lane_id(), wv = wave_id();
@@ -1351,27 +1396,66 @@
     if (__ballot(over) && lane == 0) sh.flags[1] = 1;
     __syncthreads();
     if (wave_uniform(sh.flags[1])) return false;
-#pragma unroll
-    for (int it = 0; it < kIpt; ++it) {
-        const uint32_t j = ((uint32_t)it * kSortWaves + (uint32_t)wv) * 64 + (uint32_t)lane;
-        if (j < nt) {
-            const Key<W> mine = sh.keys[j];
-            const uint32_t rs = run[it] & 0xFFFFu, re = rs + (run[it] >> 16);
-            uint32_t r = j - rs;
-            if (!skip_compare) {
-                r = 0;
+    auto place = [&](uint32_t j, uint32_t rn, const Key<W> &mine) {
+        const uint32_t rs = rn & 0xFFFFu, re = rs + (rn >> 16);
+        uint32_t r = j - rs;
+        if (!skip_compare) {
+            r = 0;
 #pragma unroll 2
-                for (uint32_t t = rs; t < j; ++t) r += key_less<W, FIRST, MASKED>(mine, sh.keys[t], m2, m1) ? 0u : 1u;
+            for (uint32_t t = rs; t < j; ++t) r += key_less<W, FIRST, MASKED>(mine, sh.keys[t], m2, m1) ? 0u : 1u;
 #pragma unroll 2
-                for (uint32_t t = j + 1; t < re; ++t) r += key_less<W, FIRST, MASKED>(sh.keys[t], mine, m2, m1) ? 1u : 0u;
-            }
-            keys[first + rs + r] = mine;
+            for (uint32_t t = j + 1; t < re; ++t) r += key_less<W, FIRST, MASKED>(sh.keys[t], mine, m2, m1) ? 1u : 0u;
+        }
+        return rs + r;
+    };
+    if constexpr (!INFO) {
+#pragma unroll
+        for (int it = 0; it < kIpt; ++it) {
+            const uint32_t j = ((uint32_t)it * kSortWaves + (uint32_t)wv) * 64 + (uint32_t)lane;
+            if (j < nt) {
+                const Key<W> mine = sh.keys[j];
+                keys[first + place(j, run[it], mine)] = mine;
+            }
+        }
+    } else {
+        static_assert(!MASKED, "stage 1 emits no edges");
+        Key<W> mine[kIpt];
+#pragma unroll
+        for (int it = 0; it < kIpt; ++it) {
+            const uint32_t j = ((uint32_t)it * kSortWaves + (uint32_t)wv) * 64 + (uint32_t)lane;
+            if (j < nt) {
+                mine[it] = sh.keys[j];
+                run[it] = place(j, run[it], mine[it]);
+            }
+        }
+        __syncthreads();
+#pragma unroll
+        for (int it = 0; it < kIpt; ++it) {
+            const uint32_t j = ((uint32_t)it * kSortWaves + (uint32_t)wv) * 64 + (uint32_t)lane;
+            if (j < nt) sh.keys[run[it]] = mine[it];
+        }
+        __syncthreads();
+#pragma unroll
+        for (int it = 0; it < kIpt; ++it) {
+            const uint32_t j = ((uint32_t)it * kSortWaves + (uint32_t)wv) * 64 + (uint32_t)lane;
+            if (j < nt) {
+                const Key<W> cur = sh.keys[j];
+                bool head = true;
+                uint8_t byte;
+                if (j == 0) {
+                    const bool bhead = emit_T < 16 || first == 0 || (cur.w[0] >> 16) != (keys[first - 1].w[0] >> 16);
+                    byte = head_info<W>(cur, emit_k, true, bhead);
+                } else
+                    byte = key_info<W>(cur, sh.keys[j - 1], emit_k, head);
+                keys[first + j] = cur;
+                info[first + j] = head ? byte : kInfoNoHead;
+            }
         }
     }
     return true;
 }
 
-template <int W, bool WANT_KEYS>
+template <int W, bool WANT_KEYS, bool INFO = false>
 __global__ __launch_bounds__(kSortThreads, 8) void local_sort_kernel(Key<W> *keys, uint64_t n, LocalPlan lp, uint64_t *big, uint32_t *big_count,
                                                                      uint32_t big_cap) {
     constexpr int kTile = LocalCfg<W>::kTile, kIpt = LocalCfg<W>::kIpt, kChunk = LocalCfg<W>::kChunk, kWindows = kTile / 64;
@@ -1501,7 +1585,14 @@
     const bool skip = (lp.debug & 1) != 0;
     const bool masked = (lp.mask_last2 & lp.mask_last) != ~0u;
     bool done;
-    if (run_bits > 32 && W > 1)
+    if constexpr (INFO) {
+        if (run_bits > 32 && W > 1)
+            done = finish_by_comparison<W, (W > 1 ? 1 : 0), false, 2, true>(sh, keys, first, nt, run_bits, ~0u, ~0u, skip, lp.info, lp.emit_k, T);
+        else if (run_bits == 32 && W > 1)
+            done = finish_by_comparison<W, (W > 1 ? 1 : 0), false, 1, true>(sh, keys, first, nt, run_bits, ~0u, ~0u, skip, lp.info, lp.emit_k, T);
+        else
+            done = finish_by_comparison<W, 0, false, 1, true>(sh, keys, first, nt, run_bits, ~0u, ~0u, skip, lp.info, lp.emit_k, T);
+    } else if (run_bits > 32 && W > 1)
         done = masked ? finish_by_comparison<W, (W > 1 ? 1 : 0), true, 2>(sh, keys, first, nt, run_bits, lp.mask_last2, lp.mask_last, skip)
                       : finish_by_comparison<W, (W > 1 ? 1 : 0), false, 2>(sh, keys, first, nt, run_bits, lp.mask_last2, lp.mask_last, skip);
     else if (run_bits == 32 && W > 1)
@@ -1595,38 +1686,6 @@
 constexpr int kEmitPerThread = 16;
 constexpr int kEmitTile = kEmitThreads * kEmitPerThread;
 
-template <int W>
-__device__ __forceinline__ bool keys_equal(const Key<W> &x, const Key<W> &y) {
-    bool eq = true;
-#pragma unroll
-    for (int j = 0; j < W; ++j) eq = eq && (x.w[j] == y.w[j]);
-    return eq;
-}
-template <int W>
-__device__ __forceinline__ bool same_km1(const Key<W> &x, const Key<W> &y, int k) {
-    int full = (k - 1) >> 4, rem = (k - 1) & 15;
-    bool eq = true;
-#pragma unroll
-    for (int j = 0; j < W; ++j) {
-        if (j < full) eq = eq && (x.w[j] == y.w[j]);
-        else if (j == full && rem > 0) eq = eq && ((x.w[j] >> (16 - rem) * 2) == (y.w[j] >> (16 - rem) * 2));
-    }
-    return eq;
-}
-template <int W>
-__device__ __forceinline__ int key_a(const Key<W> &x, int k) {
-    if ((x.w[W - 1] >> 3) & 1u) {
-        int wi = (k - 1) >> 4, ci = (k - 1) & 15;
-        uint32_t word = 0;
-#pragma unroll
-        for (int j = 0; j < W; ++j) if (j == wi) word = x.w[j];
-        return (word >> (15 - ci) * 2) & 3;
-    }
-    return kDollar;
-}
-template <int W>
-__device__ __forceinline__ int key_b(const Key<W> &x) { return x.w[W - 1] & 7u; }
-
 constexpr int kRunBaseStepLog = 10;
 struct RunStarts {
     uint32_t *lo;
@@ -1667,15 +1726,11 @@
         info[it] = 0;
         if (idx < n) {
             Key<W> cur = keys[idx];
-            bool ghead = true, bhead = true;
-            if (idx == 0) head = true;
-            else {
-                Key<W> prv = keys[idx - 1];
-                head = !keys_equal<W>(cur, prv);
-                ghead = !same_km1<W>(cur, prv, k);
-                bhead = (cur.w[0] >> 16) != (prv.w[0] >> 16);
-            }
-            info[it] = (uint8_t)(key_a<W>(cur, k) | (key_b<W>(cur) << 3) | ((int)ghead << 6) | ((int)bhead << 7));
+            if (idx == 0) {
+                head = true;
+                info[it] = head_info<W>(cur, k, true, true);
+            } else
+                info[it] = key_info<W>(cur, keys[idx - 1], k, head);
         }
         uint64_t bal = __ballot(head);
         rank_in_wave[it] = (uint32_t)__popcll(bal & lanemask_lt());
@@ -1705,6 +1760,107 @@
             if ((s & ((1u << kRunBaseStepLog) - 1)) == 0) sub_start.base[s >> kRunBaseStepLog] = idx;
             sub_info[s] = info[it];
         }
+    }
+}
+
+constexpr int kInfoRounds = 8;
+constexpr int kInfoTile = kEmitTile * kInfoRounds;
+template <bool TICKET>
+__global__ __launch_bounds__(kEmitThreads) void emit_compact_info_kernel(const uint8_t *info_in, uint64_t n, EmitChain chain, uint32_t n_tiles,
+                                                                          RunStarts sub_start, uint8_t *sub_info) {
+    static_assert(kEmitPerThread == 16, "one 16-byte load per lane and round");
+    static_assert(kInfoRounds == 8 && kEmitTile <= 65535, "round counts are scanned as 2 x 4 fields of 16 bits");
+    __shared__ uint64_t s_scr[kEmitThreads / 64 + 1];
+    __shared__ uint32_t s_tile;
+    __shared__ unsigned long long s_base;
+    __shared__ uint16_t s_off[kEmitTile];
+    __shared__ uint8_t s_inf[kEmitTile];
+    const uint32_t tile = TICKET ? chain_ticket(chain.ticket, &s_tile) : blockIdx.x;
+    const uint64_t base = (uint64_t)tile * kInfoTile;
+    const uint32_t mine = threadIdx.x * kEmitPerThread;
+    uint4 v[kInfoRounds];
+#pragma unroll
+    for (int r = 0; r < kInfoRounds; ++r) {
+        const uint64_t idx0 = base + (uint64_t)r * kEmitTile + mine;
+        v[r] = make_uint4(0, 0, 0, 0);
+        if (idx0 < n) v[r] = *reinterpret_cast<const uint4 *>(info_in + idx0);
+    }
+    uint32_t headbits[kInfoRounds];
+    uint64_t packed[2] = {0, 0};
+#pragma unroll
+    for (int r = 0; r < kInfoRounds; ++r) {
+        const uint64_t idx0 = base + (uint64_t)r * kEmitTile + mine;
+        const uint32_t left = idx0 < n ? (uint32_t)(n - idx0 < (uint64_t)kEmitPerThread ? n - idx0 : (uint64_t)kEmitPerThread) : 0u;
+        const uint32_t wd[4] = {v[r].x, v[r].y, v[r].z, v[r].w};
+        uint32_t hb = 0;
+#pragma unroll
+        for (int b = 0; b < kEmitPerThread; ++b) hb |= (uint32_t)(((wd[b >> 2] >> (8 * (b & 3))) & 7u) != (uint32_t)kInfoNoHead) << b;
+        headbits[r] = hb & ((1u << left) - 1u);
+        packed[r >> 2] |= (uint64_t)__popc(headbits[r]) << (16 * (r & 3));
+    }
+    uint64_t ex[2], tot[2];
+    ex[0] = block_excl_scan64<kEmitThreads>(packed[0], s_scr, &tot[0]);
+    ex[1] = block_excl_scan64<kEmitThreads>(packed[1], s_scr, &tot[1]);
+    uint32_t round_total[kInfoRounds], round_first[kInfoRounds], tile_total = 0;
+#pragma unroll
+    for (int r = 0; r < kInfoRounds; ++r) {
+        round_total[r] = (uint32_t)(tot[r >> 2] >> (16 * (r & 3))) & 0xFFFFu;
+        round_first[r] = tile_total;
+        tile_total += round_total[r];
+    }
+    if (wave_id() == 0) {
+        const uint64_t before = chain_exclusive(chain.state, tile, tile_total, chain.error);
+        if (lane_id() == 0) {
+            s_base = before;
+            if (tile + 1 == n_tiles) *chain.total = before + tile_total;
+        }
+    }
+    uint64_t tb = 0;
+#pragma unroll
+    for (int r = 0; r < kInfoRounds; ++r) {
+        if (round_total[r] == 0) continue;
+        const uint32_t wd[4] = {v[r].x, v[r].y, v[r].z, v[r].w};
+        uint32_t q = (uint32_t)(ex[r >> 2] >> (16 * (r & 3))) & 0xFFFFu;
+#pragma unroll
+        for (int b = 0; b < kEmitPerThread; ++b) {
+            if ((headbits[r] >> b) & 1u) {
+                s_off[q] = (uint16_t)(mine + (uint32_t)b);
+                s_inf[q] = (uint8_t)((wd[b >> 2] >> (8 * (b & 3))) & 255u);
+                ++q;
+            }
+        }
+        __syncthreads();
+        tb = s_base;
+        const uint64_t out0 = tb + round_first[r], pos0 = base + (uint64_t)r * kEmitTile;
+        for (uint32_t i = threadIdx.x; i < round_total[r]; i += kEmitThreads) {
+            const uint64_t s = out0 + i, idx = pos0 + s_off[i];
+            sub_start.lo[s] = (uint32_t)idx;
+            if ((s & ((1u << kRunBaseStepLog) - 1)) == 0) sub_start.base[s >> kRunBaseStepLog] = idx;
+            sub_info[s] = s_inf[i];
+        }
+        __syncthreads();
+    }
+}
+
+__global__ __launch_bounds__(256) void emit_check_kernel(const uint32_t *lo, const uint8_t *info, const uint32_t *lo_ref, const uint8_t *info_ref, uint64_t m,
+                                                         uint32_t *bad) {
+    for (uint64_t s = (uint64_t)blockIdx.x * 256 + threadIdx.x; s < m; s += (uint64_t)gridDim.x * 256) {
+        if (lo[s] != lo_ref[s]) atomicAdd(&bad[0], 1u);
+        if (info[s] != info_ref[s]) atomicAdd(&bad[1], 1u);
+    }
+}
+
+template <int W>
+__global__ __launch_bounds__(256) void emit_info_range_kernel(const Key<W> *keys, uint64_t n, int k, const uint64_t *start, const uint64_t *end, int stride,
+                                                              uint8_t *key_info_out) {
+    const uint64_t first = start[(uint64_t)blockIdx.x * stride] & ~kSegInOther;
+    uint64_t last = end[(uint64_t)blockIdx.x * stride];
+    if (last > n) last = n;
+    for (uint64_t i = first + threadIdx.x; i < last; i += 256) {
+        const Key<W> cur = keys[i];
+        bool head = true;
+        const uint8_t info = i == 0 ? head_info<W>(cur, k, true, true) : key_info<W>(cur, keys[i - 1], k, head);
+        key_info_out[i] = head ? info : kInfoNoHead;
     }
 }
 
@@ -1863,10 +2019,11 @@
 }
 
 struct SortModes {
-    int bias = 1, side = 1, fused = 1, wide = 1;
+    int bias = 1, side = 1, fused = 1, wide = 1, emit_fused = 1;
     static SortModes from_env() {
         const char *bias = getenv("MGTA_SORT_BIAS"), *side = getenv("MGTA_SORT_SIDE"), *fused = getenv("MGTA_SORT_FUSED"), *wide = getenv("MGTA_SORT_WIDE");
-        return SortModes{bias ? atoi(bias) : 1, side ? atoi(side) : 1, fused ? atoi(fused) : 1, wide ? atoi(wide) : 1};
+        const char *emit_fused = getenv("MGTA_EMIT_FUSED");
+        return SortModes{bias ? atoi(bias) : 1, side ? atoi(side) : 1, fused ? atoi(fused) : 1, wide ? atoi(wide) : 1, emit_fused ? atoi(emit_fused) : 1};
     }
 };
 
@@ -1955,6 +2112,7 @@
     bool census_done = false;
     bool side_done = false;
     bool first_pass_done = false;
+    int emit_k = 0;
     bool uses_side() const { return side_mode > 0 && top.P >= 2 && kSideFits<WT>; }
     uint64_t side_bytes() const { return n * (top.max_width() > 8 ? 2u : 1u) + 64; }
     uint64_t hist_bytes() const { return std::max<uint64_t>(1, (n + kBlockTile - 1) / kBlockTile) * ((uint64_t)8 << top.max_width()); }
@@ -2087,7 +2245,7 @@
 }
 
 template <int WT>
-static Key<WT> *lds_finish(mgta_ctx *ctx, const SortJob<WT> &job, Key<WT> *src, Key<WT> *dst, SortLog *log) {
+static Key<WT> *lds_finish(mgta_ctx *ctx, const SortJob<WT> &job, Key<WT> *src, Key<WT> *dst, SortLog *log, const uint8_t **info_out = nullptr) {
     hipStream_t stream = ctx->stream;
     const uint64_t n_items = job.n;
     const int T = job.top.T();
@@ -2117,7 +2275,15 @@
     lp.mask_last2 = job.mask_last2; lp.mask_last = job.mask_last; lp.stride = stride;
     lp.lsd_list = d_lsd; lp.lsd_count = d_big_count + 1; lp.lsd_cap = (uint32_t)l_blocks;
     lp.debug = ctx->force_lsd_tiles >> 1;
-    if (ub > 0)
+    uint8_t *d_info = nullptr;
+    if (info_out) *info_out = nullptr;
+    if (info_out && job.emit_k > 0 && T <= 2 * (job.emit_k - 1) && (job.mask_last2 & job.mask_last) == ~0u && !lp.debug)
+        d_info = pool_get<uint8_t>(ctx, S_SIDE, job.uses_side() ? job.side_bytes() : n_items + 64);
+    lp.info = d_info; lp.emit_k = job.emit_k;
+    if (ub > 0 && d_info)
+        hipLaunchKernelGGL((local_sort_kernel<WT, true, true>), dim3((unsigned)l_blocks), dim3(kSortThreads), 0, stream, src, n_items, lp, d_big, d_big_count,
+                           big_cap);
+    else if (ub > 0)
         hipLaunchKernelGGL((local_sort_kernel<WT, true>), dim3((unsigned)l_blocks), dim3(kSortThreads), 0, stream, src, n_items, lp, d_big, d_big_count,
                            big_cap);
     else
@@ -2146,6 +2312,13 @@
             ctx->split_levels = std::max(ctx->split_levels, levels);
         }
     }
+    if (d_info) {
+        if (n_lsd_tiles > 0)
+            hipLaunchKernelGGL((emit_info_range_kernel<WT>), dim3(n_lsd_tiles), dim3(256), 0, stream, src, n_items, job.emit_k, d_lsd, d_lsd + 1, 2, d_info);
+        if (n_big > 0)
+            hipLaunchKernelGGL((emit_info_range_kernel<WT>), dim3(n_big), dim3(256), 0, stream, src, n_items, job.emit_k, d_big, d_big + big_cap, 1, d_info);
+        *info_out = d_info;
+    }
     t.end();
     MGTA_HIP_CHECK(hipEventSynchronize(t.b));
     const float ms = t.ms();
@@ -2154,9 +2327,9 @@
 }
 
 template <int WT>
-static Key<WT> *device_sort(mgta_ctx *ctx, const SortJob<WT> &job, SortLog *log = nullptr) {
+static Key<WT> *device_sort(mgta_ctx *ctx, const SortJob<WT> &job, SortLog *log = nullptr, const uint8_t **info_out = nullptr) {
     Key<WT> *src = global_passes(ctx, job, log);
-    return src ? lds_finish(ctx, job, src, src == job.a ? job.b : job.a, log) : nullptr;
+    return src ? lds_finish(ctx, job, src, src == job.a ? job.b : job.a, log, info_out) : nullptr;
 }
 
 template <int W>
@@ -2338,6 +2511,7 @@
     uint64_t wide_items = 0;
     uint32_t wide_nb = 0;
     bool fz_check_failed = false;
+    const uint8_t *sorted_info = nullptr;
     mgta_build_stats S{};
     Timer t_all{stream}, t_ph{stream};
     SortLog log{&S, {}};
@@ -2392,6 +2566,7 @@
         S.k = k; S.words_per_key = W; S.words_per_tip = words_per_tip; S.n_reads = (int64_t)rd->n_reads;
         ctx->peak_bytes = ctx->live_bytes;
         ctx->split_levels = 0;
+        ctx->emit_fused_passes = 0;
         size_t free_b = 0, total_b = 0;
         MGTA_HIP_CHECK(hipMemGetInfo(&free_b, &total_b));
         const uint64_t avail = (uint64_t)free_b + pool_bytes(ctx);
@@ -2537,6 +2712,7 @@
         SortJob<W> job{a, b, p.n_items, top_plan(p.n_items, p.b_lo, p.b_hi)};
         job.low = low_digit_plan(k, W, job.top.T());
         job.side_mode = modes.side;
+        job.emit_k = modes.emit_fused > 0 ? k : 0;
         job.census_done = p.closed_form && job.top.P >= 1 && p.n_tiles <= 0x7FFFFFFFull;
         job.side_done = !p.closed_form && job.uses_side();
         if (!p.closed_form && fz_table && multi_n && p.width == multi_width && p.b_lo >= multi_lo && (p.b_lo - multi_lo) % p.width == 0) {
@@ -2601,7 +2777,7 @@
 
     Key<W> *sort_keys(const SortJob<W> &job) {
         t_ph.start();
-        Key<W> *sorted = device_sort(ctx, job, &log);
+        Key<W> *sorted = device_sort(ctx, job, &log, &sorted_info);
         if (sorted) S.ms_sort += t_ph.stop();
         return sorted;
     }
@@ -2624,29 +2800,70 @@
         uint64_t *d_scan_tmp = pool_get<uint64_t>(ctx, S_SCAN_TMP, scan_tmp_elems(std::max<uint64_t>(std::max(n_blocks, e_tiles), n_items / kDecideTile + 1)) * 8);
         if (e_tiles > 0xFFFFFFFFull) { set_error("too many emit tiles"); return MGTA_EUNSUPPORTED; }
         unsigned long long *d_chain = pool_get<unsigned long long>(ctx, S_TILE_BASE, (e_tiles + 4) * 8);
-        EmitChain chain;
-        chain.state = d_chain; chain.total = d_chain + e_tiles;
-        chain.ticket = reinterpret_cast<uint32_t *>(d_chain + e_tiles + 1); chain.error = reinterpret_cast<uint32_t *>(d_chain + e_tiles + 2);
         RunStarts sub_start;
         sub_start.lo = reinterpret_cast<uint32_t *>(scratch);
         uint16_t *rec = reinterpret_cast<uint16_t *>(scratch + n_items * 4);
         uint8_t *info = reinterpret_cast<uint8_t *>(scratch + n_items * 6);
         sub_start.base = reinterpret_cast<uint64_t *>(scratch + ((n_items * 7 + 7) & ~7ull));
-        unsigned long long chain_out[3] = {0, 0, 0};
-        for (int attempt = 0; attempt < 2; ++attempt) {
-            MGTA_HIP_CHECK(hipMemsetAsync(d_chain, 0, (e_tiles + 4) * 8, stream));
-            if (attempt == 0 && !ctx->force_full_lsd)
-                hipLaunchKernelGGL((emit_compact_kernel<W, false>), dim3((unsigned)e_tiles), dim3(kEmitThreads), 0, stream, sorted, n_items, k, chain,
-                                   (uint32_t)e_tiles, sub_start, info);
-            else
-                hipLaunchKernelGGL((emit_compact_kernel<W, true>), dim3((unsigned)e_tiles), dim3(kEmitThreads), 0, stream, sorted, n_items, k, chain,
-                                   (uint32_t)e_tiles, sub_start, info);
-            MGTA_HIP_CHECK(hipMemcpyAsync(chain_out, d_chain + e_tiles, 24, hipMemcpyDeviceToHost, stream));
-            MGTA_HIP_CHECK(hipStreamSynchronize(stream));
-            if ((uint32_t)chain_out[2] == 0) break;
-        }
-        if ((uint32_t)chain_out[2] != 0) { set_error("internal: chained scan of the emitter timed out"); return MGTA_EINTERNAL; }
-        const uint64_t m = chain_out[0];
+        auto compact = [&](const uint8_t *key_info, RunStarts st, uint8_t *st_info, uint64_t *m_out) {
+            unsigned long long chain_out[3] = {0, 0, 0};
+            const uint64_t tiles = key_info ? (n_items + kInfoTile - 1) / kInfoTile : e_tiles;
+            EmitChain chain;
+            chain.state = d_chain; chain.total = d_chain + tiles;
+            chain.ticket = reinterpret_cast<uint32_t *>(d_chain + tiles + 1); chain.error = reinterpret_cast<uint32_t *>(d_chain + tiles + 2);
+            for (int attempt = 0; attempt < 2; ++attempt) {
+                MGTA_HIP_CHECK(hipMemsetAsync(d_chain, 0, (tiles + 4) * 8, stream));
+                const bool ticket = !(attempt == 0 && !ctx->force_full_lsd);
+                const dim3 grid((unsigned)tiles), block(kEmitThreads);
+                if (key_info && !ticket)
+                    hipLaunchKernelGGL((emit_compact_info_kernel<false>), grid, block, 0, stream, key_info, n_items, chain, (uint32_t)tiles, st, st_info);
+                else if (key_info)
+                    hipLaunchKernelGGL((emit_compact_info_kernel<true>), grid, block, 0, stream, key_info, n_items, chain, (uint32_t)tiles, st, st_info);
+                else if (!ticket)
+                    hipLaunchKernelGGL((emit_compact_kernel<W, false>), grid, block, 0, stream, sorted, n_items, k, chain, (uint32_t)tiles, st, st_info);
+                else
+                    hipLaunchKernelGGL((emit_compact_kernel<W, true>), grid, block, 0, stream, sorted, n_items, k, chain, (uint32_t)tiles, st, st_info);
+                MGTA_HIP_CHECK(hipMemcpyAsync(chain_out, d_chain + tiles, 24, hipMemcpyDeviceToHost, stream));
+                MGTA_HIP_CHECK(hipStreamSynchronize(stream));
+                if ((uint32_t)chain_out[2] == 0) break;
+            }
+            if ((uint32_t)chain_out[2] != 0) { set_error("internal: chained scan of the emitter timed out"); return MGTA_EINTERNAL; }
+            *m_out = chain_out[0];
+            return MGTA_OK;
+        };
+        uint64_t m = 0;
+        if (int rc = compact(sorted_info, sub_start, info, &m)) return rc;
+        if (sorted_info) {
+            ctx->emit_fused_passes++;
+            if (modes.emit_fused >= 2) {
+                RunStarts ref;
+                uint8_t *ref_info = reinterpret_cast<uint8_t *>(rec);
+                char *behind = reinterpret_cast<char *>(sub_start.base + (n_items >> kRunBaseStepLog) + 1);
+                ref.lo = reinterpret_cast<uint32_t *>(behind);
+                ref.base = reinterpret_cast<uint64_t *>(behind + ((n_items * 4 + 7) & ~7ull));
+                if ((uint64_t)(reinterpret_cast<char *>(ref.base + (n_items >> kRunBaseStepLog) + 1) - scratch) > p.key_b) {
+                    set_error("internal: no room to check the emitter's info bytes");
+                    return MGTA_EINTERNAL;
+                }
+                uint64_t m_ref = 0;
+                if (int rc = compact(nullptr, ref, ref_info, &m_ref)) return rc;
+                uint32_t *d_bad = reinterpret_cast<uint32_t *>(pool_get<uint64_t>(ctx, S_SMALL, 4096) + 320);
+                uint32_t bad[2] = {0, 0};
+                MGTA_HIP_CHECK(hipMemsetAsync(d_bad, 0, 8, stream));
+                const uint64_t m_min = std::min(m, m_ref);
+                if (m_min > 0) {
+                    const unsigned grid = (unsigned)std::min<uint64_t>((m_min + 255) / 256, (uint64_t)ctx->num_cus * 16);
+                    hipLaunchKernelGGL(emit_check_kernel, dim3(grid), dim3(256), 0, stream, sub_start.lo, info, ref.lo, ref_info, m_min, d_bad);
+                }
+                MGTA_HIP_CHECK(hipMemcpyAsync(bad, d_bad, 8, hipMemcpyDeviceToHost, stream));
+                MGTA_HIP_CHECK(hipStreamSynchronize(stream));
+                if (m != m_ref || bad[0] || bad[1]) {
+                    set_error("internal: the info bytes of the sort give %llu runs, the keys %llu; %u starts and %u info bytes differ",
+                              (unsigned long long)m, (unsigned long long)m_ref, bad[0], bad[1]);
+                    return MGTA_EINTERNAL;
+                }
+            }
+        }
         uint64_t d_tiles = (m + kDecideTile - 1) / kDecideTile;
         uint32_t *ce = pool_get<uint32_t>(ctx, S_CNT, d_tiles * 4 * 3), *cl = ce + d_tiles, *ct = cl + d_tiles;
         uint64_t *be = pool_get<uint64_t>(ctx, S_BASE, d_tiles * 8 * 3), *bl = be + d_tiles, *bt = bl + d_tiles;
@@ -2826,6 +3043,12 @@
     return MGTA_OK;
 }
 
+int mgta_sdbg_last_emit_fused(mgta_ctx *ctx, int64_t *n_passes) {
+    if (!ctx || !n_passes) { set_error("mgta_sdbg_last_emit_fused: null argument"); return MGTA_EINVAL; }
+    *n_passes = ctx->emit_fused_passes;
+    return MGTA_OK;
+}
+
 int mgta_sort_plan(uint64_t n_items, int words_per_key, uint32_t bucket_begin, uint32_t bucket_end, int *n_passes, int *skip_bits) {
     if (!n_passes || !skip_bits || words_per_key < 2 || bucket_end > (uint32_t)MGTA_NUM_BUCKETS || bucket_begin >= bucket_end) {
         set_error("mgta_sort_plan: bad argument");
```

After: 10.04, median of 6. +4.7%, better.
